# amidos2006/gym-pcgrl

Measured on AMD Instinct MI355X. Metric: env-steps/sec (whole node), binary-narrow 14x14 @ 65536 envs, higher is better.
Workload: dtype u8; 1 GPU; binary-narrow-v0 14x14, 65536 envs/GPU; envs_per_gpu=65536, width=14, height=14, max_changes=39, actions=uniform random, device-generated before the timed region, parallelism=env-axis shard x1, no collective on the step path

## Files before the change

gym_pcgrl_amd/_lib.py:

```python
import ctypes as C
import os
import subprocess

PKG = os.path.dirname(os.path.abspath(__file__))
ROOT = os.path.dirname(PKG)
CSRC = os.path.join(PKG, "csrc")
LIBDIR = os.path.join(PKG, "lib")
SO = os.path.join(LIBDIR, "libpcgrl_hip.so")
SOURCES = [os.path.join(CSRC, "pcgrl_abi.hip")]
HIPCC_FLAGS = ["--offload-arch=gfx950", "-O3", "-std=c++17", "-ffp-contract=off", "-fPIC", "-shared", "-mllvm", "-amdgpu-sched-strategy=max-ilp"]

PCGRL_OK, PCGRL_EINVAL, PCGRL_EHIP, PCGRL_ESTATE = 0, -1, -2, -3


class Config(C.Structure):
    _fields_ = [(n, C.c_int32) for n in (
        "prob", "rep", "num_envs", "width", "height", "prob_width", "prob_height", "max_changes", "max_iterations",
        "random_start", "random_tile", "warp", "random_probs", "auto_reset", "target_path",
        "max_enemies", "target_enemy_dist", "max_crates", "target_solution", "solver_power", "max_potions",
        "max_treasures", "max_diamonds", "min_spikes", "target_jumps", "min_empty", "min_enemies", "min_jumps")] + [
        ("target_col_enemies", C.c_double), ("tile_probs", C.c_double * 8), ("rewards", C.c_double * 12)]


class Layout(C.Structure):
    _fields_ = [(n, C.c_int32) for n in ("group", "mask_bytes", "nplanes", "nstats")] + [
        (n, C.c_size_t) for n in ("map", "old_map", "heatmap", "pos", "planes", "counters", "stats", "start_stats",
                                  "info", "reward", "done", "tile_p", "rng_rep", "rng_prob", "rng_cursor", "scratch")]


TUNING_FIELDS = ("no_fused", "fused_zelda", "step_epb", "no_inc", "inline_reset", "pair_min", "no_wide", "wide_waves", "wide_grid",
                 "wide_pairs", "wide_few", "sok_generic", "sok_hard_cap", "sok_spawn", "md_only_agent", "smb_lds_heap", "full_per_wave", "inc_per_wave", "wide_spin", "step_prio", "no_touch", "touch_tight", "step_pair", "async_split", "big_team", "obs_at_end", "touch_resume",
                 "changes_grid", "changes_chunk")


class Tuning(C.Structure):
    _fields_ = [(n, C.c_int32) for n in TUNING_FIELDS]


TUNING_OVERRIDES = {}


def make_tuning(overrides=None):
    t = Tuning(*([-1] * len(TUNING_FIELDS)))
    for k, v in list(TUNING_OVERRIDES.items()) + list((overrides or {}).items()):
        if k not in TUNING_FIELDS:
            raise KeyError("unknown tuning switch %r (known: %s)" % (k, ", ".join(TUNING_FIELDS)))
        setattr(t, k, int(v))
    return t


BUFFER_NAMES = ("map", "old_map", "heatmap", "pos", "planes", "counters", "stats", "start_stats", "info", "reward",
                "done", "tile_p", "rng_rep", "rng_prob", "rng_cursor", "scratch")


class Buffers(C.Structure):
    _fields_ = [(n, C.c_void_p) for n in BUFFER_NAMES]


ROW_FIELDS = ("actions_out", "reward", "done", "start_in", "start_out", "ep_return", "ep_length", "took", "fresh")


class Row(C.Structure):
    _fields_ = [(n, C.c_void_p) for n in ROW_FIELDS] + [("actions_i64", C.c_int32)]


class RenderDesc(C.Structure):
    _fields_ = [("indices", C.c_void_p), ("count", C.c_int32), ("tiles", C.c_void_p), ("tile_size", C.c_int32),
                ("border_x", C.c_int32), ("border_y", C.c_int32), ("border_tile", C.c_int32), ("cursor", C.c_int32),
                ("grid_rows", C.c_int32), ("grid_cols", C.c_int32), ("out", C.c_void_p)]


ABI_VERSION = 15
EXPORTS = ("pcgrl_abi_version", "pcgrl_error_string", "pcgrl_last_hip_error", "pcgrl_query_layout", "pcgrl_create",
           "pcgrl_destroy", "pcgrl_bind", "pcgrl_configure", "pcgrl_seed", "pcgrl_set_tile_probs", "pcgrl_reset",
           "pcgrl_step", "pcgrl_set_maps", "pcgrl_observe", "pcgrl_action_map", "pcgrl_status", "pcgrl_profile",
           "pcgrl_profile_read", "pcgrl_bind_episode_stats", "pcgrl_seed_words", "pcgrl_rollout", "pcgrl_bind_observation", "pcgrl_selftest_heap",
           "pcgrl_tuning_defaults", "pcgrl_set_tuning", "pcgrl_clear_status", "pcgrl_step_flat",
           "pcgrl_async_bytes", "pcgrl_bind_async", "pcgrl_step_async", "pcgrl_async_flush", "pcgrl_step_multi", "pcgrl_selftest_step_pool", "pcgrl_step_threads", "pcgrl_selftest_range_reward",
           "pcgrl_bind_row", "pcgrl_render", "pcgrl_get_stats_bytes", "pcgrl_get_stats", "pcgrl_get_reward",
           "pcgrl_get_solution_bytes", "pcgrl_get_solution", "pcgrl_get_playthrough_bytes", "pcgrl_get_playthrough",
           "pcgrl_get_smb_play_bytes", "pcgrl_get_smb_play", "pcgrl_get_paths_legs", "pcgrl_get_paths_bytes", "pcgrl_get_paths",
           "pcgrl_get_changes_bytes", "pcgrl_get_changes")
NPHASE = 6
PHASES = ("update", "stats", "reset_or_idle", "solver_or_reset", "reset2", "solver2")


def sources_newer_than_lib():
    if not os.path.exists(SO):
        return True
    t = os.path.getmtime(SO)
    deps = [os.path.join(CSRC, f) for f in os.listdir(CSRC)] + [os.path.join(ROOT, "include", "pcgrl_hip.h")]
    return any(os.path.getmtime(d) > t for d in deps)


def source_hash():
    import hashlib
    h = hashlib.sha256()
    files = sorted(os.path.join(CSRC, f) for f in os.listdir(CSRC)) + [os.path.join(ROOT, "include", "pcgrl_hip.h")]
    h.update(" ".join(HIPCC_FLAGS).encode() + b"\0")
    for f in files:
        h.update(os.path.basename(f).encode() + b"\0")
        with open(f, "rb") as fh:
            h.update(fh.read())
    return h.hexdigest()[:16]


NPARTS = 8


def build(force=False, verbose=False, jobs=None):
    if not force and not sources_newer_than_lib():
        return SO
    os.makedirs(LIBDIR, exist_ok=True)
    objdir = os.path.join(LIBDIR, "obj")
    os.makedirs(objdir, exist_ok=True)
    hipcc = os.environ.get("HIPCC", "hipcc")
    flags = [f for f in HIPCC_FLAGS if f != "-shared"]
    jobs = jobs or int(os.environ.get("PCGRL_BUILD_JOBS", "0")) or min(NPARTS, os.cpu_count() or 1)
    objs = [os.path.join(objdir, "part%d.o" % k) for k in range(NPARTS)]
    cmds = [[hipcc] + flags + ["-DPCGRL_PART=%d" % k, "-c", SOURCES[0], "-o", objs[k]] for k in range(NPARTS)]
    running, todo, failed = [], list(range(NPARTS)), []
    while todo or running:
        while todo and len(running) < jobs:
            k = todo.pop(0)
            if verbose:
                print(" ".join(cmds[k]), flush=True)
            running.append((k, subprocess.Popen(cmds[k])))
        k, p = running.pop(0)
        if p.wait() != 0:
            failed.append(k)
    if failed:
        raise subprocess.CalledProcessError(1, cmds[failed[0]])
    link = [hipcc, "--offload-arch=gfx950", "-shared", "-fPIC"] + objs + ["-o", SO]
    if verbose:
        print(" ".join(link), flush=True)
    subprocess.check_call(link)
    return SO


_lib = None


def load():
    global _lib, SO
    if _lib is not None:
        return _lib
    SO = os.environ.get("PCGRL_HIP_SO", SO)
    if not os.path.exists(SO):
        raise RuntimeError(
            "gym_pcgrl_amd: HIP library %s is missing. Build it with `python -c 'import __graft_entry__ as g; g.build()'` "
            "(hipcc --offload-arch=gfx950). There is no CPU fallback for the batched environment." % SO)
    import torch
    L = C.CDLL(SO)
    for name in EXPORTS:
        if not hasattr(L, name):
            raise RuntimeError("gym_pcgrl_amd: %s does not export %s (stale build?)" % (SO, name))
    L.pcgrl_abi_version.restype = C.c_int
    if L.pcgrl_abi_version() != ABI_VERSION:
        raise RuntimeError("gym_pcgrl_amd: %s has ABI version %d, this package needs %d (stale build?)" % (SO, L.pcgrl_abi_version(), ABI_VERSION))
    L.pcgrl_error_string.restype = C.c_char_p
    L.pcgrl_error_string.argtypes = [C.c_int]
    L.pcgrl_last_hip_error.restype = C.c_int
    L.pcgrl_query_layout.argtypes = [C.POINTER(Config), C.POINTER(Layout)]
    L.pcgrl_create.argtypes = [C.POINTER(Config), C.POINTER(C.c_void_p)]
    L.pcgrl_destroy.argtypes = [C.c_void_p]
    L.pcgrl_tuning_defaults.argtypes = [C.POINTER(Tuning)]
    L.pcgrl_tuning_defaults.restype = None
    L.pcgrl_set_tuning.argtypes = [C.c_void_p, C.POINTER(Tuning)]
    L.pcgrl_bind.argtypes = [C.c_void_p, C.POINTER(Buffers), C.c_void_p]
    L.pcgrl_configure.argtypes = [C.c_void_p, C.POINTER(Config)]
    L.pcgrl_seed.argtypes = [C.c_void_p, C.c_void_p, C.c_int32, C.c_int32, C.c_void_p]
    L.pcgrl_seed_words.argtypes = [C.c_void_p, C.c_void_p, C.c_int32, C.c_int32, C.c_void_p]
    L.pcgrl_set_tile_probs.argtypes = [C.c_void_p, C.c_void_p]
    L.pcgrl_reset.argtypes = [C.c_void_p, C.c_void_p]
    L.pcgrl_step.argtypes = [C.c_void_p, C.c_void_p, C.c_void_p]
    L.pcgrl_rollout.argtypes = [C.c_void_p, C.c_void_p, C.c_int32, C.c_void_p, C.c_void_p, C.c_void_p, C.c_void_p]
    L.pcgrl_set_maps.argtypes = [C.c_void_p, C.c_void_p, C.c_void_p]
    L.pcgrl_observe.argtypes = [C.c_void_p, C.c_void_p, C.c_int32, C.c_int32, C.c_int32, C.c_int32, C.c_int32, C.c_void_p]
    L.pcgrl_bind_observation.argtypes = [C.c_void_p, C.c_void_p, C.c_int32, C.c_int32, C.c_int32, C.c_int32, C.c_int32, C.c_int32]
    L.pcgrl_bind_row.argtypes = [C.c_void_p, C.POINTER(Row)]
    L.pcgrl_render.argtypes = [C.c_void_p, C.POINTER(RenderDesc), C.c_void_p]
    L.pcgrl_get_stats_bytes.argtypes = [C.POINTER(Config), C.c_int32]
    L.pcgrl_get_stats_bytes.restype = C.c_size_t
    L.pcgrl_get_stats.argtypes = [C.c_void_p, C.c_void_p, C.c_int32, C.c_void_p, C.c_void_p, C.c_size_t, C.c_void_p]
    L.pcgrl_get_reward.argtypes = [C.c_void_p, C.c_void_p, C.c_void_p, C.c_int32, C.c_void_p, C.c_void_p, C.c_void_p]
    moves_args = (C.c_void_p, C.c_void_p, C.c_int32, C.c_int32, C.c_void_p, C.c_void_p, C.c_void_p, C.c_void_p, C.c_void_p, C.c_size_t, C.c_void_p)
    for name in ("pcgrl_get_solution", "pcgrl_get_playthrough", "pcgrl_get_smb_play"):
        getattr(L, name + "_bytes").argtypes = [C.POINTER(Config), C.c_int32, C.c_int32]
        getattr(L, name + "_bytes").restype = C.c_size_t
        getattr(L, name).argtypes = list(moves_args)
    L.pcgrl_get_paths_legs.argtypes = [C.POINTER(Config)]
    L.pcgrl_get_paths_legs.restype = C.c_int32
    L.pcgrl_get_paths_bytes.argtypes = [C.POINTER(Config), C.c_int32, C.c_int32]
    L.pcgrl_get_paths_bytes.restype = C.c_size_t
    L.pcgrl_get_paths.argtypes = [C.c_void_p, C.c_void_p, C.c_int32, C.c_int32, C.c_void_p, C.c_void_p, C.c_void_p, C.c_void_p, C.c_size_t, C.c_void_p]
    L.pcgrl_get_changes_bytes.argtypes = [C.POINTER(Config), C.c_int32, C.c_int32]
    L.pcgrl_get_changes_bytes.restype = C.c_size_t
    L.pcgrl_get_changes.argtypes = [C.c_void_p, C.c_void_p, C.c_int32, C.c_void_p, C.c_int32, C.c_void_p, C.c_void_p, C.c_void_p, C.c_void_p, C.c_void_p,
                                    C.c_void_p, C.c_size_t, C.c_void_p]
    L.pcgrl_action_map.argtypes = [C.c_void_p, C.c_void_p, C.c_void_p, C.c_void_p]
    L.pcgrl_step_flat.argtypes = [C.c_void_p, C.c_void_p, C.c_void_p, C.c_void_p]
    L.pcgrl_selftest_heap.argtypes = [C.c_void_p, C.c_int32, C.c_void_p, C.c_void_p, C.c_void_p, C.c_void_p]
    L.pcgrl_selftest_step_pool.argtypes = [C.c_int32, C.c_int32, C.c_int32, C.c_void_p]
    L.pcgrl_selftest_range_reward.argtypes = [C.c_void_p, C.c_int32, C.c_void_p, C.c_void_p]
    L.pcgrl_step_threads.argtypes = [C.c_int32]
    L.pcgrl_step_threads.restype = C.c_int32
    L.pcgrl_status.argtypes = [C.c_void_p, C.c_void_p, C.POINTER(C.c_int32)]
    L.pcgrl_clear_status.argtypes = [C.c_void_p, C.c_void_p]
    L.pcgrl_profile.argtypes = [C.c_void_p, C.c_int]
    L.pcgrl_bind_episode_stats.argtypes = [C.c_void_p, C.c_void_p, C.c_void_p, C.c_void_p, C.c_void_p, C.c_void_p]
    L.pcgrl_profile_read.argtypes = [C.c_void_p, C.POINTER(C.c_double), C.POINTER(C.c_int32)]
    L.pcgrl_async_bytes.argtypes = [C.POINTER(Config), C.c_int32]
    L.pcgrl_async_bytes.restype = C.c_size_t
    L.pcgrl_bind_async.argtypes = [C.c_void_p, C.c_void_p, C.c_size_t, C.c_int32, C.c_void_p]
    L.pcgrl_step_async.argtypes = [C.c_void_p, C.c_void_p, C.c_int32, C.c_void_p]
    L.pcgrl_async_flush.argtypes = [C.c_void_p, C.c_void_p]
    L.pcgrl_step_multi.argtypes = [C.POINTER(C.c_void_p), C.POINTER(C.c_void_p), C.POINTER(C.c_void_p), C.c_int32]
    _lib = L
    return L


def check(rc, what):
    if rc != 0:
        L = load()
        msg = L.pcgrl_error_string(rc).decode()
        extra = " (hipError %d)" % L.pcgrl_last_hip_error() if rc == PCGRL_EHIP else ""
        raise RuntimeError("gym_pcgrl_amd: %s failed: %s%s" % (what, msg, extra))
```

gym_pcgrl_amd/csrc/kernels_stats.h:

```cpp
#pragma once
template <class MaskT>
__device__ __forceinline__ MaskT row_valid(int lane, int W, int H) {
    MaskT full = (W >= (int)(8 * sizeof(MaskT))) ? ~(MaskT)0 : (((MaskT)1 << W) - 1);
    return lane < H ? full : (MaskT)0;
}

template <int PROB = -1>
__device__ __forceinline__ bool finalize_item(const PcgrlParams& P, const DevBufs& B, int e, const int32_t* s,
                                              int mode, int parity, int shard, bool push_reset = true, int rst_list = WL_RST,
                                              const int2* pre = nullptr, const double* reward_pre = nullptr) {
    const int prob = PROB >= 0 ? PROB : P.prob;
    int32_t* st = B.stats + (size_t)e * 8;
    int32_t* start = B.start_stats + (size_t)e * 8;
    if (mode == MODE_STEP) {
        int32_t old[PCGRL_MAX_STATS], sv[PCGRL_MAX_STATS];
        for (int k = 0; k < 8; k++) { old[k] = st[k]; sv[k] = start[k]; }
        const int2 c = pre ? *pre : reinterpret_cast<const int2*>(B.counters)[e];
        const double r = reward_pre ? *reward_pre : compute_reward(P, s, old, prob);
        const bool d = episode_over(P, s, sv, prob) || c.y >= P.max_changes || c.x >= P.max_iterations;
        B.reward[e] = r;
        B.done[e] = d ? 1 : 0;
        episode_account(B, e, r, d);
        int32_t* inf = B.info + (size_t)e * 10;
#pragma unroll
        for (int k = 0; k < 8; k++) {
            st[k] = s[k];
            inf[k] = (prob == PCGRL_PROB_BINARY && k == 2) ? s[1] - sv[1] : ((prob == PCGRL_PROB_BINARY && k == 3) ? 0 : s[k]);
        }
        inf[8] = c.x; inf[9] = c.y;
        if (d && P.auto_reset && push_reset) wl_push(B, parity, rst_list, shard, e);
        return d && P.auto_reset;
    } else {
        for (int k = 0; k < 8; k++) st[k] = s[k];
        if (mode == MODE_START)
            for (int k = 0; k < 8; k++) start[k] = s[k];
    }
    return false;
}

template <int PROB, class G, class MaskT>
__device__ __forceinline__ bool compute_item_stats(G& g, const PcgrlParams& P, MaskT b0, MaskT b1, MaskT b2, MaskT valid, int32_t* s,
                                                   int32_t* status, MaskT& champ, bool tight = true) {
    champ = 0;
    if (PROB == PCGRL_PROB_BINARY) {
        int regions, path;
        if (G::kGroup == 16) {
            int ub2;
            regions_and_longest_path(g, (MaskT)(~b0 & valid), regions, path, champ, ub2, tight);
            s[3] = ub2 + 1;
        } else {
            regions_and_longest_path(g, (MaskT)(~b0 & valid), regions, path, champ);
        }
        s[0] = regions; s[1] = path; s[2] = g.any(champ) ? 1 : 0;
        return false;
    }
    if (PROB == PCGRL_PROB_ZELDA) { zelda_stats(g, P, b0, b1, b2, valid, s); return false; }
    if (PROB == PCGRL_PROB_MDUNGEON) return mdungeon_stats(g, P, b0, b1, b2, valid, s);
    if (PROB == PCGRL_PROB_DDAVE) {
        bool overflow = false;
        const bool ns = ddave_stats(g, P, b0, b1, b2, valid, s, &overflow);
        if (overflow && g.lane == 0) atomicOr(status, PCGRL_STATUS_TOO_MANY_CRATES);
        return ns;
    }
    if (PROB == PCGRL_PROB_SMB) return true;
    return sokoban_stats(g, P, b0, b1, b2, valid, s);
}
template <int PROB, class G, class MaskT>
__device__ __forceinline__ bool compute_item_stats(G& g, const PcgrlParams& P, MaskT b0, MaskT b1, MaskT b2, MaskT valid, int32_t* s, int32_t* status) {
    MaskT champ;
    return compute_item_stats<PROB>(g, P, b0, b1, b2, valid, s, status, champ);
}

template <int PROB = -1>
__device__ __forceinline__ bool finish_or_park(const PcgrlParams& P, const DevBufs& B, int e, const int32_t* s, bool need_solver,
                                               int mode, int parity, int shard, bool push_reset = true, int park_list = -1,
                                               const double* reward_pre = nullptr) {
    if (need_solver) {
        int32_t* park = (mode == MODE_STEP) ? B.info + (size_t)e * 10 : B.stats + (size_t)e * 8;
        for (int k = 0; k < 8; k++) park[k] = s[k];
        wl_push(B, parity, park_list >= 0 ? park_list : (mode == MODE_STEP ? WL_SOL : WL_SOL2), shard, e);
        return false;
    }
    return finalize_item<PROB>(P, B, e, s, mode, parity, shard, push_reset, WL_RST, nullptr, reward_pre);
}

template <int J>
__device__ __forceinline__ double dpp_down(double v) {
    const long long b = __double_as_longlong(v);
    const int lo = __builtin_amdgcn_update_dpp(0, (int)b, 0x100 + J, 0xF, 0xF, true), hi = __builtin_amdgcn_update_dpp(0, (int)(b >> 32), 0x100 + J, 0xF, 0xF, true);
    return __longlong_as_double(((long long)hi << 32) | (unsigned)lo);
}
__device__ __forceinline__ void zelda_reward_tab(const PcgrlParams& P, ZeldaRewardTab* T) {
    T->w[0] = P.rewards[0]; T->w[1] = P.rewards[1]; T->w[2] = P.rewards[2]; T->w[3] = P.rewards[4]; T->w[4] = P.rewards[3];
    T->w[5] = P.rewards[5]; T->w[6] = P.rewards[6]; T->w[7] = 0.0;
    T->lo[0] = 1; T->lo[1] = 1; T->lo[2] = 1; T->lo[3] = 2; T->lo[4] = 1; T->lo[5] = P.target_enemy_dist; T->lo[6] = PCGRL_IPOS; T->lo[7] = 0;
    T->hi[0] = 1; T->hi[1] = 1; T->hi[2] = 1; T->hi[3] = P.max_enemies; T->hi[4] = 1; T->hi[5] = PCGRL_IPOS; T->hi[6] = PCGRL_IPOS; T->hi[7] = 0;
}
__device__ __forceinline__ double zelda_reward_lanes(const ZeldaRewardTab* T, const int32_t* old, const int32_t* s, int k) {
    const int s0 = s[0], s1 = s[1], s2 = s[2], s3 = s[3], s4 = s[4], s5 = s[5], s6 = s[6];
    int n = s6;
    n = k == 5 ? s5 : n; n = k == 4 ? s4 : n; n = k == 3 ? s3 : n; n = k == 2 ? s2 : n; n = k == 1 ? s1 : n; n = k == 0 ? s0 : n;
    const int kk = k & 7;
    const int o = old[kk];
    const double t = k < 7 ? (double)range_reward_i(n, o, T->lo[kk], T->hi[kk]) * T->w[kk] : 0.0;
    double r = t;
    r = r + dpp_down<1>(t); r = r + dpp_down<2>(t); r = r + dpp_down<3>(t);
    r = r + dpp_down<4>(t); r = r + dpp_down<5>(t); r = r + dpp_down<6>(t);
    return r;
}

template <int PROB, int G, class MaskT, bool FUSED = false>
__device__ __forceinline__ void stats_wave_task(const PcgrlParams& P, const DevBufs& B, DevGroup<G, MaskT>& g, int lane64, int gw, bool lone,
                                                bool inc, bool pair, bool zinc, bool have, int raw, int shard, int mode, int parity,
                                                int inline_reset, int gen_map, uint32_t* mt, uint8_t* tiles, MaskT rowmask,
                                                StepLocal* SL = nullptr, bool step_obs = false) {
    constexpr bool kCanReset = PROB == PCGRL_PROB_BINARY || PROB == PCGRL_PROB_ZELDA;
    if (!kCanReset) inline_reset = 0;
    constexpr int GPW = 64 / G;
    constexpr bool kInc = PROB == PCGRL_PROB_BINARY;
    constexpr bool kZinc = PROB == PCGRL_PROB_ZELDA && G == 16 && sizeof(MaskT) == 4;
    constexpr int NPL = (PROB == PCGRL_PROB_BINARY) ? 1 : 3;
    MaskT* champ_base = reinterpret_cast<MaskT*>(B.champ);
    const bool tch = kInc && G == 16 && !inc && !lone && have && raw < 0;
    const bool packed = inc || (kZinc && zinc && !lone) || tch;
    const bool reset_only = have && !packed && (raw & WL_RESET_ONLY) != 0;
    const bool compute = have && !reset_only && !(lone && (gw & 1));
    const int e = packed ? wl_inc_env<G>(raw) : (raw & ~WL_RESET_ONLY);
    MaskT* planes_e = reinterpret_cast<MaskT*>(B.planes) + (size_t)e * NPL * G;
    MaskT b0 = 0, b1 = 0, b2 = 0;
    if (compute) {
        b0 = planes_e[g.lane * NPL];
        if (NPL > 1) { b1 = planes_e[g.lane * NPL + 1]; b2 = planes_e[g.lane * NPL + 2]; }
    }
    if (GPW >= 2 && lone && inline_reset) {
        const int role = gw & 1;
        int2 pre = make_int2(0, 0);
        if (g.lane == 0 && role == 0 && have) pre = reinterpret_cast<const int2*>(B.counters)[e];
        asm volatile("s_waitcnt vmcnt(0)" ::: "memory");
#pragma unroll
        for (int k = 0; k < GPW / 2; k++) {
            if (k > 0 && !pair) break;
            if (!__builtin_amdgcn_readlane((int)have, 2 * k * G)) continue;
            const int ek = __builtin_amdgcn_readlane(e, 2 * k * G);
            const int step_draws = (SL && P.rep == PCGRL_REP_NARROW && P.random_tile) ? 1 : 0;
            if (SL && lane64 == 0) SL->dirty[ek - SL->e0] = 1;
            ResetRows rr;
            wave_reset_env<PROB, !FUSED, FUSED>(P, B, ek, gen_map, mt, (uint8_t*)nullptr, lane64, step_draws, gw == 2 * k + 1 ? g.lane : -1, &rr);
            MaskT t0, t1, t2;
            reset_rows_to_planes<MaskT>(P, reinterpret_cast<MaskT*>(B.planes) + (size_t)ek * NPL * G, gw == 2 * k + 1 ? g.lane : -1, rr.m0, rr.m1, rr.m2, t0, t1, t2);
            if (gw == 2 * k + 1) { b0 = t0; b1 = t1; b2 = t2; }
            __builtin_amdgcn_wave_barrier();
        }
        TL(9);
        const bool act = have && (role == 1 || !reset_only);
        int32_t sl[PCGRL_MAX_STATS] = {0, 0, 0, 0, 0, 0, 0, 0};
        MaskT champ_l = 0;
        bool ns = false;
        if (act) ns = compute_item_stats<PROB>(g, P, b0, b1, b2, rowmask, sl, B.status, champ_l, (B.step_tight & 2) != 0);
        TL(10);
        constexpr bool kLaneReward = PROB == PCGRL_PROB_ZELDA && G == 16;
        double rpre = 0.0;
        if (kLaneReward && SL && role == 0 && act) rpre = zelda_reward_lanes(&SL->zr, B.stats + (size_t)e * 8, sl, g.lane);
        if (g.lane == 0 && role == 0 && act) finalize_item<PROB>(P, B, e, sl, MODE_STEP, parity, shard, false, WL_RST, &pre, (kLaneReward && SL) ? &rpre : nullptr);
        __builtin_amdgcn_wave_barrier();
        if (role == 1 && have) {
            if (kInc && champ_base) champ_base[(size_t)e * G + g.lane] = champ_l;
            if (g.lane == 0) finish_or_park<PROB>(P, B, e, sl, ns, MODE_START, parity, shard);
        }
        if (FUSED && step_obs) {
#pragma unroll
            for (int k = 0; k < GPW / 2; k++) {
                if (k > 0 && !pair) break;
                if (!__builtin_amdgcn_readlane((int)have, 2 * k * G)) continue;
                const ObsPlanes<MaskT, NPL> src = {reinterpret_cast<const MaskT*>(B.planes), G};
                obs_write_env_lean(src, obs_view_from_lds(&SL->obs_v), B.pos, __builtin_amdgcn_readlane(e, 2 * k * G), lane64);
            }
        }
        return;
    }
    int32_t s[PCGRL_MAX_STATS] = {0, 0, 0, 0, 0, 0, 0, 0};
    bool need_solver = false;
    MaskT champ = 0;
    if (kInc && inc) {
        if (compute) {
            const MaskT cbit = (g.lane == wl_inc_row<G>(raw)) ? (MaskT)1 << wl_inc_col<G>(raw) : (MaskT)0;
            const MaskT champ_old = champ_base[(size_t)e * G + g.lane];
            const int4 old = *reinterpret_cast<const int4*>(B.stats + (size_t)e * 8);
            int regions, path, ub2;
            binary_incremental(g, (MaskT)(~b0 & rowmask), cbit, wl_inc_code<G>(raw) != 0, old.x, old.y, champ_old, old.w - 1, regions, path, champ, ub2);
            s[0] = regions; s[1] = path; s[2] = 1; s[3] = ub2 + 1;
        }
    } else if (kZinc && packed) {
        if (compute) {
            const MaskT cbit = (g.lane == wl_inc_row<G>(raw)) ? (MaskT)1 << wl_inc_col<G>(raw) : (MaskT)0;
            zelda_stats(g, P, b0, b1, b2, rowmask, s, (int)wl_inc_code<G>(raw), cbit, B.stats[(size_t)e * 8 + 4]);
        }
    } else {
        bool full = compute;
        if (kInc && G == 16) {
            const bool t = compute && tch;
            TouchMemo<MaskT> memo = touch_memo_empty(g, b0);
            if (t) {
                const MaskT cbit = (g.lane == wl_inc_row<G>(raw)) ? (MaskT)1 << wl_inc_col<G>(raw) : (MaskT)0;
                const MaskT champ_old = champ_base[(size_t)e * G + g.lane];
                const int4 old = *reinterpret_cast<const int4*>(B.stats + (size_t)e * 8);
                int regions, path, ub2;
                if (binary_touch(g, (MaskT)(~b0 & rowmask), cbit, (wl_inc_code<G>(raw) & 1u) != 0, old.x, champ_old, old.w - 1, regions, path, champ, ub2, memo)) {
                    s[0] = regions; s[1] = path; s[2] = 1; s[3] = ub2 + 1;
                    full = false;
                }
            }
#ifdef PCGRL_TIMELINE
            {
                const uint64_t gu = __ballot(t && full && g.lane == 0), pl = __ballot(compute && !tch && g.lane == 0);
                TL(32 + __popcll(gu) + 8 * __popcll(pl));
            }
#endif
            constexpr bool kResume = FUSED && sizeof(MaskT) == 4;
            if (kResume && B.touch_resume) {
                if (full) {
                    int regions, path, ub2;
                    rlp_resume(g, (MaskT)(~b0 & rowmask), memo, regions, path, champ, ub2, (B.step_tight & 1) != 0);
                    s[0] = regions; s[1] = path; s[2] = g.any(champ) ? 1 : 0; s[3] = ub2 + 1;
                }
                full = false;
            }
        }
        if (full) need_solver = compute_item_stats<PROB>(g, P, b0, b1, b2, rowmask, s, B.status, champ, (B.step_tight & 1) != 0);
    }
    if (kInc && compute && champ_base) champ_base[(size_t)e * G + g.lane] = champ;
    TL(10);
    int want_reset = 0;
    constexpr bool kLaneReward = PROB == PCGRL_PROB_ZELDA && G == 16;
    double rpre = 0.0;
    const bool lane_reward = kLaneReward && SL != nullptr && mode == MODE_STEP;
    if (lane_reward && have && !reset_only) rpre = zelda_reward_lanes(&SL->zr, B.stats + (size_t)e * 8, s, g.lane);
    if (g.lane == 0 && have) {
        if (reset_only) want_reset = 1;
        else want_reset = finish_or_park<PROB>(P, B, e, s, need_solver, mode, parity, shard, !inline_reset, -1, lane_reward ? &rpre : nullptr) ? 1 : 0;
    }
    if (inline_reset) {
        const uint64_t want = __ballot(want_reset != 0);
        TL(11);
        if (want) {
            TL(12);
            if (SL) { while (__hip_atomic_load(&SL->refill_done[SL->par], __ATOMIC_ACQUIRE, __HIP_MEMORY_SCOPE_WORKGROUP) < SL->need) __builtin_amdgcn_s_sleep(2); }
            bool mine = false;
#pragma unroll
            for (int k = 0; k < GPW; k++) {
                if ((want >> (k * G)) & 1ull) {
                    const int ek = __builtin_amdgcn_readlane(e, k * G);
                    if (SL && lane64 == 0) { SL->dirty[ek - SL->e0] = 1; SL->late[ek - SL->e0] = 1; SL->n_late = 1; }
                    int pend = 0;
                    if (SL) {
                        if (lane64 == 0) {
                            pend = atomicExch(&SL->pend[ek - SL->e0], 0);
                            if (pend < 0) {
                                while (__hip_atomic_load(&SL->late_done[(ek - SL->e0) >> 6], __ATOMIC_ACQUIRE, __HIP_MEMORY_SCOPE_WORKGROUP) == 0) __builtin_amdgcn_s_sleep(2);
                                pend = 0;
                            }
                        }
                        pend = __builtin_amdgcn_readfirstlane(pend);
                    }
                    ResetRows rr;
                    wave_reset_env<PROB, !FUSED, FUSED>(P, B, ek, gen_map, mt, (uint8_t*)nullptr, lane64, 0, gw == k ? g.lane : -1, &rr, pend);
                    MaskT t0, t1, t2;
                    reset_rows_to_planes<MaskT>(P, reinterpret_cast<MaskT*>(B.planes) + (size_t)ek * NPL * G, gw == k ? g.lane : -1, rr.m0, rr.m1, rr.m2, t0, t1, t2);
                    if (gw == k) { b0 = t0; b1 = t1; b2 = t2; mine = true; }
                    __builtin_amdgcn_wave_barrier();
                }
            }
            if (mine) {
                int32_t st[PCGRL_MAX_STATS] = {0, 0, 0, 0, 0, 0, 0, 0};
                const bool ns = compute_item_stats<PROB>(g, P, b0, b1, b2, rowmask, st, B.status, champ, (B.step_tight & 2) != 0);
                if (kInc && champ_base) champ_base[(size_t)e * G + g.lane] = champ;
                if (g.lane == 0) finish_or_park<PROB>(P, B, e, st, ns, MODE_START, parity, shard);
            }
        }
    }
}

template <int PROB, int G, class MaskT>
__global__ __launch_bounds__(PCGRL_BLOCK) __attribute__((amdgpu_waves_per_eu(4, 8))) void k_stats(PcgrlParams P, DevBufs B, int list, int parity, int mode, int clear_parity,
                                                        int inline_reset, int gen_map, int lone0) {
    extern __shared__ __attribute__((aligned(16))) uint8_t smem[];
    __shared__ int s_pref[WL_NSHARD + 1], s_pref_inc[WL_NSHARD + 1], s_pref_rst[WL_NSHARD + 1];
    if (clear_parity >= 0 && blockIdx.x == 0) wl_clear(B, clear_parity);
    DevGroup<G, MaskT> g;
    constexpr int GPB = PCGRL_BLOCK / G, GPW = 64 / G;
    constexpr bool kInc = PROB == PCGRL_PROB_BINARY;
    constexpr bool kZinc = PROB == PCGRL_PROB_ZELDA && G == 16 && sizeof(MaskT) == 4;
    const bool zinc = kZinc && mode == MODE_STEP && B.zelda_inc;
    const bool with_inc = (kInc && mode == MODE_STEP && B.champ != nullptr) || zinc;
    int n_inc = 0, n_rst = 0;
    const int n_full = (with_inc || lone0 == 2 || list < 0) ? wl_load_prefix3(B, parity, list, with_inc ? WL_INC : -1, lone0 == 2 ? WL_RST : -1,
                                                                              s_pref, s_pref_inc, s_pref_rst, &n_inc, &n_rst)
                                                             : wl_load_prefix(B, parity, list, s_pref);
    const int n0 = lone0 == 1 ? s_pref[1] : (lone0 == 2 ? n_rst : 0);
    const int f0 = lone0 == 1 ? n0 : 0;
    const int w_full = (n_full - f0 + GPW - 1) / GPW;
    const bool pair = GPW >= 4 && n0 >= B.pair_min;
    const int w_lone = pair ? (n0 + 1) >> 1 : n0;
    const int w_total = w_lone + w_full + (n_inc + GPW - 1) / GPW;
    MaskT* champ_base = reinterpret_cast<MaskT*>(B.champ);
    const int lane64 = threadIdx.x & 63, wv = threadIdx.x >> 6, gw = lane64 / G;
    const int NPL = (PROB == PCGRL_PROB_BINARY) ? 1 : 3;
    const int W = P.width, H = P.height;
    uint32_t* mt = reinterpret_cast<uint32_t*>(smem + (size_t)wv * reset_stage_bytes(W * H));
    uint8_t* tiles = reinterpret_cast<uint8_t*>(mt + PCGRL_MT_N);
    const MaskT rowmask = row_valid<MaskT>(g.lane, W, H);
    for (int wid = blockIdx.x * (PCGRL_BLOCK / 64) + wv; wid < w_total; wid += gridDim.x * (PCGRL_BLOCK / 64)) {
        const bool lone = wid < w_lone;
        const bool inc = wid >= w_lone + w_full;
        const int item = lone ? (pair ? 2 * wid + (gw >> 1) : wid) : (inc ? (wid - w_lone - w_full) * GPW + gw : f0 + (wid - w_lone) * GPW + gw);
        const bool have = lone ? (item < n0 && (pair || gw < 2)) : item < (inc ? n_inc : n_full);
        const bool from_rst = lone && lone0 == 2;
        const int raw = !have ? 0 : (inc ? wl_get(B, WL_INC, s_pref_inc, item) : (from_rst ? wl_get(B, WL_RST, s_pref_rst, item) : wl_get(B, list, s_pref, item)));
        const int shard = (item >> 4) & (WL_NSHARD - 1);
        stats_wave_task<PROB, G, MaskT>(P, B, g, lane64, gw, lone, inc, pair, zinc, have, raw, shard, mode, parity, inline_reset, gen_map, mt, tiles, rowmask);
    }
}

template <class MaskT>
struct LdsShared {
    MaskT* rest; int* bestp; int lane;
    __device__ __forceinline__ MaskT load_rest() const { return *reinterpret_cast<volatile MaskT*>(rest + lane); }
    template <class G>
    __device__ __forceinline__ bool retire(G& g, MaskT comp) const {
        const MaskT fb = g.first_bit(comp);
        MaskT old = 0;
        if (fb) old = atomicAnd(rest + lane, ~fb);
        const bool won = __ballot((old & fb) != 0) != 0;
        if (comp) atomicAnd(rest + lane, ~comp);
        return won;
    }
    __device__ __forceinline__ int best() const { return *reinterpret_cast<volatile int*>(bestp); }
    __device__ __forceinline__ void raise(int v) const { if (lane == 0 && v > 0) atomicMax(bestp, v); }
};
template <class MaskT>
__device__ __forceinline__ void block_regions_and_path(DevGroup<64, MaskT>& g, MaskT pass, int tw, int ts, int lane, int H,
                                                       MaskT* s_rest, int* s_regions, int* s_best, int* s_owner, MaskT* champ_e) {
    const int bh = (H + ts - 1) / ts;
    const int row_lo = tw * bh, row_hi = (row_lo + bh < H) ? row_lo + bh : H;
    int tiny_regions, tiny_path;
    TL(20);
    const MaskT nontiny = rlp_prepare(g, pass, tiny_regions, tiny_path);
    TL(21);
    if (tw == 0) {
        s_rest[lane] = nontiny;
        if (lane == 0) { *s_regions = tiny_regions; *s_best = tiny_path; *s_owner = -1; }
    }
    __syncthreads();
    LdsShared<MaskT> sh = {s_rest, s_best, lane};
    int regions = 0, my_best = 0;
    MaskT my_champ = 0;
    MaskT rest = sh.load_rest();
    if (g.any(rest)) {
        const PcgFillCtx<DevGroup<64, MaskT>> ctx = pcg_fill_ctx(g, pass);
        do {
            rlp_process_seed(g, rlp_choose_seed(g, rest, row_lo, row_hi), ctx, sh, regions, my_best, my_champ);
            rest = sh.load_rest();
        } while (g.any(rest));
    }
    TL(22);
    if (lane == 0 && regions) atomicAdd(s_regions, regions);
    __syncthreads();
    TL(23);
    if (lane == 0 && my_best > tiny_path && my_best == *s_best) atomicCAS(s_owner, -1, tw);
    __syncthreads();
    if (champ_e) {
        const int owner = *s_owner;
        if (tw == (owner < 0 ? 0 : owner)) champ_e[lane] = owner < 0 ? (MaskT)0 : my_champ;
    }
}

template <class MaskT>
__device__ __forceinline__ void wave_incremental_item(const PcgrlParams& P, const DevBufs& B, DevGroup<64, MaskT>& g, int raw, int parity,
                                                      int inline_reset, int gen_map, uint32_t* mt, uint8_t* tiles, int lane, MaskT rowmask) {
    const int e = wl_inc_env<64>(raw);
    MaskT* planes_e = reinterpret_cast<MaskT*>(B.planes) + (size_t)e * 64;
    MaskT* champ_e = reinterpret_cast<MaskT*>(B.champ) + (size_t)e * 64;
    const MaskT b0 = planes_e[lane];
    const MaskT champ_old = champ_e[lane];
    const int2 old = *reinterpret_cast<const int2*>(B.stats + (size_t)e * 8);
    const MaskT cbit = (lane == wl_inc_row<64>(raw)) ? (MaskT)1 << wl_inc_col<64>(raw) : (MaskT)0;
    int regions, path;
    MaskT champ;
    binary_incremental(g, (MaskT)(~b0 & rowmask), cbit, wl_inc_code<64>(raw) != 0, old.x, old.y, champ_old, regions, path, champ);
    champ_e[lane] = champ;
    int want = 0;
    if (lane == 0) {
        int32_t s[PCGRL_MAX_STATS] = {regions, path, 1, 0, 0, 0, 0, 0};
        want = finalize_item<PCGRL_PROB_BINARY>(P, B, e, s, MODE_STEP, parity, e & (WL_NSHARD - 1), !inline_reset) ? 1 : 0;
    }
    want = __builtin_amdgcn_readfirstlane(want);
    if (inline_reset && want) {
        ResetRows rr;
        wave_reset_env<PCGRL_PROB_BINARY>(P, B, e, gen_map, mt, (uint8_t*)nullptr, lane, 0, lane, &rr);
        MaskT n0, n1, n2;
        reset_rows_to_planes<MaskT>(P, planes_e, lane, rr.m0, rr.m1, rr.m2, n0, n1, n2);
        int32_t st[PCGRL_MAX_STATS] = {0, 0, 0, 0, 0, 0, 0, 0};
        compute_item_stats<PCGRL_PROB_BINARY>(g, P, n0, n1, n2, rowmask, st, B.status, champ);
        champ_e[lane] = champ;
        if (lane == 0) finalize_item<PCGRL_PROB_BINARY>(P, B, e, st, MODE_START, parity, e & (WL_NSHARD - 1));
    }
}

#define WIDE_SPIN_LIMIT 400
__device__ __forceinline__ int wide_claim(int32_t* word, int epoch, int who) {
    int cur = __hip_atomic_load(word, __ATOMIC_RELAXED, __HIP_MEMORY_SCOPE_AGENT);
    for (;;) {
        if ((cur >> 1) == epoch) return 0;
        const int seen = atomicCAS(word, cur, (epoch << 1) | who);
        if (seen == cur) return 1;
        cur = seen;
    }
}

template <class MaskT, int NWAVES>
__global__ __launch_bounds__(NWAVES * 64) void k_stats_wide(PcgrlParams P, DevBufs B, int list, int parity, int mode, int clear_parity,
                                                             int inline_reset, int gen_map, int pair_few) {
    extern __shared__ __attribute__((aligned(16))) uint8_t smem[];
    __shared__ int s_pref[WL_NSHARD + 1], s_pref_rst[WL_NSHARD + 1], s_pref_inc[WL_NSHARD + 1];
    __shared__ MaskT s_rest[2][64];
    __shared__ int s_regions[2], s_best[2], s_owner[2], s_flag, s_flag2[2], s_cur, s_claim;
    __shared__ int2 s_pre;
    if (clear_parity >= 0 && blockIdx.x == 0) wl_clear(B, clear_parity);
    TL_INIT(); TL(1);
    WTL(0, wall_clock64());
    DevGroup<64, MaskT> g;
    const bool with_inc = mode == MODE_STEP && B.champ != nullptr;
    int n_rst = 0, n_inc = 0;
    const int n_chg = wl_load_prefix3(B, parity, list, with_inc ? WL_INC : -1, inline_reset ? WL_RST : -1, s_pref, s_pref_inc, s_pref_rst, &n_inc, &n_rst);
    const int n = n_rst + n_chg;
    const int lane = threadIdx.x & 63, wv = threadIdx.x >> 6;
    const int W = P.width, H = P.height;
    const int wave_lds = reset_stage_bytes(W * H);
    uint32_t* mt = reinterpret_cast<uint32_t*>(smem);
    uint8_t* tiles = reinterpret_cast<uint8_t*>(mt + PCGRL_MT_N);
    uint32_t* rst_raw = reinterpret_cast<uint32_t*>(smem + wave_lds);
    uint64_t* rst_bits = reinterpret_cast<uint64_t*>(smem + wave_lds + (size_t)8 * W * H);
    const MaskT rowmask = row_valid<MaskT>(lane, W, H);
    const int n_many = pair_few ? s_pref[WL_NSHARD / 2] : n_chg;
    const int n_items = 2 * n_rst + n_many + (n_chg - n_many + 1) / 2;
    const int epoch = B.wide_epoch;
    WTL(1, wall_clock64());
    WTL(5, (unsigned long long)n_items | ((unsigned long long)n_rst << 16) | ((unsigned long long)n_many << 32) | ((unsigned long long)n_inc << 48));
    for (int item = blockIdx.x; item < n_items; item += gridDim.x) {
        const bool lone = item < 2 * n_rst;
        const bool old_half = lone && (item & 1) == 0;
        WTL(2, (old_half ? 1 : (lone ? 2 : (item >= 2 * n_rst + n_many ? 4 : 3))) | (item << 8));
        if (item >= 2 * n_rst + n_many) {
            constexpr int TS = NWAVES / 2;
            const int team = wv / TS, tw = wv % TS;
            const int idx0 = n_many + 2 * (item - 2 * n_rst - n_many);
            const int e0 = wl_get(B, list, s_pref, idx0) & ~WL_RESET_ONLY;
            const int e1 = idx0 + 1 < n_chg ? (wl_get(B, list, s_pref, idx0 + 1) & ~WL_RESET_ONLY) : -1;
            const int et = team ? e1 : e0;
            const int shard = (item >> 4) & (WL_NSHARD - 1);
            MaskT pass = 0;
            if (et >= 0) pass = (MaskT)(~(reinterpret_cast<const MaskT*>(B.planes) + (size_t)et * 64)[lane] & rowmask);
            if (threadIdx.x < 2) s_flag2[threadIdx.x] = 0;
            block_regions_and_path(g, pass, tw, TS, lane, H, s_rest[team], &s_regions[team], &s_best[team], &s_owner[team],
                                   (et >= 0 && B.champ) ? reinterpret_cast<MaskT*>(B.champ) + (size_t)et * 64 : (MaskT*)nullptr);
            if (tw == 0 && lane == 0 && et >= 0) {
                int32_t s[PCGRL_MAX_STATS] = {s_regions[team], s_best[team], s_owner[team] >= 0 ? 1 : 0, 0, 0, 0, 0, 0};
                const bool want = finalize_item<PCGRL_PROB_BINARY>(P, B, et, s, mode, parity, shard, !inline_reset);
                s_flag2[team] = (want && inline_reset) ? 1 : 0;
            }
            __syncthreads();
            for (int t = 0; t < 2; t++) {
                if (!(inline_reset && s_flag2[t])) continue;
                const int er = t ? e1 : e0;
                MaskT* planes_r = reinterpret_cast<MaskT*>(B.planes) + (size_t)er * 64;
                const MaskT b0 = block_reset_env<PCGRL_PROB_BINARY, NWAVES * 64, MaskT>(P, B, er, gen_map, mt, tiles, rst_raw, rst_bits, &s_cur);
                if (wv == 0) planes_r[lane] = b0;
                block_regions_and_path(g, (MaskT)(~b0 & rowmask), wv, NWAVES, lane, H, s_rest[0], &s_regions[0], &s_best[0], &s_owner[0],
                                       B.champ ? reinterpret_cast<MaskT*>(B.champ) + (size_t)er * 64 : (MaskT*)nullptr);
                if (threadIdx.x == 0) {
                    int32_t s[PCGRL_MAX_STATS] = {s_regions[0], s_best[0], s_owner[0] >= 0 ? 1 : 0, 0, 0, 0, 0, 0};
                    finalize_item<PCGRL_PROB_BINARY>(P, B, er, s, MODE_START, parity, shard);
                }
                __syncthreads();
            }
            continue;
        }
        const int raw = lone ? wl_get(B, WL_RST, s_pref_rst, item >> 1) : wl_get(B, list, s_pref, item - 2 * n_rst);
        const bool reset_only = (raw & WL_RESET_ONLY) != 0;
        const int e = raw & ~WL_RESET_ONLY;
        const int shard = (item >> 4) & (WL_NSHARD - 1);
        MaskT* planes_e = reinterpret_cast<MaskT*>(B.planes) + (size_t)e * 64;
        MaskT* champ_e = B.champ ? reinterpret_cast<MaskT*>(B.champ) + (size_t)e * 64 : nullptr;
        int32_t* sync_e = B.wide_sync + (size_t)e * 4;
        if (old_half) {
            if (reset_only) continue;
            if (threadIdx.x == 0) s_claim = wide_claim(sync_e + 3, epoch, 0);
            __syncthreads();
            if (!s_claim) { __syncthreads(); continue; }
            const MaskT b_old = planes_e[lane];
            asm volatile("s_waitcnt vmcnt(0)" ::: "memory");
            __syncthreads();
            if (threadIdx.x == 0) __hip_atomic_store(sync_e + 0, epoch, __ATOMIC_RELEASE, __HIP_MEMORY_SCOPE_AGENT);
            block_regions_and_path(g, (MaskT)(~b_old & rowmask), wv, NWAVES, lane, H, s_rest[0], &s_regions[0], &s_best[0], &s_owner[0], (MaskT*)nullptr);
            if (threadIdx.x == 0) {
                sync_e[2] = s_regions[0] | (s_best[0] << 16);
                __hip_atomic_store(sync_e + 1, epoch, __ATOMIC_RELEASE, __HIP_MEMORY_SCOPE_AGENT);
            }
            __syncthreads();
            continue;
        }
        if (lone) {
            __builtin_amdgcn_s_setprio(1);
            if (threadIdx.x == 0) s_pre = reinterpret_cast<const int2*>(B.counters)[e];
            asm volatile("s_waitcnt vmcnt(0)" ::: "memory");
            __syncthreads();
            TL(24);
            const MaskT n0 = block_reset_env<PCGRL_PROB_BINARY, NWAVES * 64, MaskT>(P, B, e, gen_map, mt, tiles, rst_raw, rst_bits, &s_cur);
            int own_old = 0;
            if (!reset_only) {
                if (threadIdx.x == 0) {
                    int spins = 0, mine = 0;
                    while (__hip_atomic_load(sync_e + 0, __ATOMIC_ACQUIRE, __HIP_MEMORY_SCOPE_AGENT) != epoch) {
                        __builtin_amdgcn_s_sleep(4);
                        if (++spins == B.wide_spin && wide_claim(sync_e + 3, epoch, 1)) { mine = 1; break; }
                    }
                    s_claim = mine;
                }
                __syncthreads();
                own_old = s_claim;
                if (own_old) {
                    const MaskT b_old = planes_e[lane];
                    asm volatile("s_waitcnt vmcnt(0)" ::: "memory");
                    block_regions_and_path(g, (MaskT)(~b_old & rowmask), wv, NWAVES, lane, H, s_rest[1], &s_regions[1], &s_best[1], &s_owner[1], (MaskT*)nullptr);
                }
                __syncthreads();
            }
            if (wv == 0) planes_e[lane] = n0;
            TL(26);
            block_regions_and_path(g, (MaskT)(~n0 & rowmask), wv, NWAVES, lane, H, s_rest[0], &s_regions[0], &s_best[0], &s_owner[0], champ_e);
            if (threadIdx.x == 0) {
                if (!reset_only) {
                    int32_t s[PCGRL_MAX_STATS] = {s_regions[1], s_best[1], 0, 0, 0, 0, 0, 0};
// ... 52 lines not shown
```

gym_pcgrl_amd/csrc/kernels_step.h:

```cpp
#pragma once

struct StepLds { int planes, champ, stats, start, cnt, cur, fifo, tag, pos, act, flat, in_total, info, rew, done, total; };
__host__ __device__ constexpr StepLds step_lds_layout(int plane_row_bytes, int champ_row_bytes, bool fifo, int action_width, int epb) {
    StepLds L = {};
    int o = 0;
    L.planes = o; o += epb * plane_row_bytes;
    L.champ = o; o += epb * champ_row_bytes;
    L.stats = o; o += epb * 32;
    L.start = o; o += epb * 32;
    L.cnt = o; o += epb * 8;
    L.cur = o; o += epb * 8;
    L.fifo = o; o += fifo ? epb * PCGRL_FIFO_N * 4 : 0;
    L.tag = o; o += fifo ? epb * 4 : 0;
    L.pos = o; o += epb * 2;
    L.act = o; o += epb * 4 * action_width;
    L.flat = o; o += action_width == 3 ? epb * 4 : 0;
    L.in_total = o;
    L.info = o; o += epb * 40;
    L.rew = o; o += epb * 8;
    L.done = o; o += epb;
    L.total = (o + 15) & ~15;
    return L;
}

template <int TPB>
__device__ __forceinline__ void blk_copy(uint8_t* dst, const uint8_t* src, int bytes) {
    const int nv = bytes >> 4;
    for (int i = threadIdx.x; i < nv; i += TPB) reinterpret_cast<uint4*>(dst)[i] = reinterpret_cast<const uint4*>(src)[i];
    for (int i = (nv << 4) + threadIdx.x; i < bytes; i += TPB) dst[i] = src[i];
}
template <int TPB>
__device__ __forceinline__ void blk_copy_rows(uint8_t* dst, const uint8_t* src, int rows, int row, const uint8_t* flag) {
    const int per = row >> 4;
    for (int i = threadIdx.x; i < rows * per; i += TPB)
        if (flag[i / per]) reinterpret_cast<uint4*>(dst)[i] = reinterpret_cast<const uint4*>(src)[i];
}

template <int TPB, int C, int SLOT0, int NV>
__device__ __forceinline__ void seg_load_c(uint4& rc, const void* g, bool on, int tid) {
    if (C * TPB + TPB - 1 < SLOT0 || C * TPB >= SLOT0 + NV) return;
    const int slot = C * TPB + tid;
    if (on && slot >= SLOT0 && slot < SLOT0 + NV) rc = reinterpret_cast<const uint4*>(g)[slot - SLOT0];
}
#define PCGRL_SEG_LOAD(SLOT0, NV, G, ON) do { const void* g_ = (G); const bool on_ = (ON); \
    seg_load_c<TPB, 0, SLOT0, NV>(r0, g_, on_, tid0); seg_load_c<TPB, 1, SLOT0, NV>(r1, g_, on_, tid0); seg_load_c<TPB, 2, SLOT0, NV>(r2, g_, on_, tid0); \
    seg_load_c<TPB, 3, SLOT0, NV>(r3, g_, on_, tid0); seg_load_c<TPB, 4, SLOT0, NV>(r4, g_, on_, tid0); seg_load_c<TPB, 5, SLOT0, NV>(r5, g_, on_, tid0); \
    seg_load_c<TPB, 6, SLOT0, NV>(r6, g_, on_, tid0); seg_load_c<TPB, 7, SLOT0, NV>(r7, g_, on_, tid0); seg_load_c<TPB, 8, SLOT0, NV>(r8, g_, on_, tid0); } while (0)
template <int TPB, int C, int TOTAL>
__device__ __forceinline__ void seg_store_c(uint8_t* smem, const uint4& rc, int tid) {
    if (C * TPB >= TOTAL) return;
    const int slot = C * TPB + tid;
    if (slot < TOTAL) reinterpret_cast<uint4*>(smem)[slot] = rc;
}

__device__ __forceinline__ void fifo_refill(const DevBufs& B, int e, int k, int cur0) {
    uint32_t* ring = B.rng_rep + (size_t)e * PCGRL_MT_N;
    uint32_t* fl = B.fifo + (size_t)e * PCGRL_FIFO_N;
    const int base = mt_wrap(cur0 + PCGRL_FIFO_N), basem = mt_wrap(base + PCGRL_MT_M);
    uint32_t a[PCGRL_FIFO_N + 1], m[PCGRL_FIFO_N];
#pragma unroll
    for (int i = 0; i <= PCGRL_FIFO_N; i++) a[i] = (i <= k) ? ring[mt_wrap(base + i)] : 0u;
#pragma unroll
    for (int i = 0; i < PCGRL_FIFO_N; i++) m[i] = (i < k) ? ring[mt_wrap(basem + i)] : 0u;
#pragma unroll
    for (int i = 0; i < PCGRL_FIFO_N; i++) if (i < k) ring[mt_wrap(cur0 + i)] = fl[i];
#pragma unroll
    for (int j = 0; j < PCGRL_FIFO_N; j++) if (j + k < PCGRL_FIFO_N) fl[j] = fl[j + k];
#pragma unroll
    for (int i = 0; i < PCGRL_FIFO_N; i++) if (i < k) fl[PCGRL_FIFO_N - k + i] = mt_twist(a[i], a[i + 1], m[i]);
    B.fifo_tag[e] = mt_wrap(cur0 + k);
}

__device__ __forceinline__ void step_set_prio(int p) {
    if (p == 0) __builtin_amdgcn_s_setprio(0);
    else if (p == 1) __builtin_amdgcn_s_setprio(1);
    else if (p == 2) __builtin_amdgcn_s_setprio(2);
    else __builtin_amdgcn_s_setprio(3);
}

template <int PROB, int REP, class MaskT, bool MULTI, int EPB, bool OBS = false, bool ROW = false>
__global__ __launch_bounds__(EPB * 4) __attribute__((amdgpu_waves_per_eu(4, 8))) void k_step(PcgrlParams P, DevBufs Bg, const int32_t* __restrict__ actions, int parity, int gen_map,
                                                                                                     int steps, size_t action_stride, double* reward_out, uint8_t* done_out, int32_t* info_out) {
    extern __shared__ __attribute__((aligned(16))) uint8_t smem[];
    constexpr int TPB = EPB * 4, NUPD = EPB / 64;
    __shared__ int s_items[3][EPB];
    __shared__ int s_n[2][4];
    __shared__ StepLocal s_loc;
    __shared__ int s_obs_ticket;
    static_assert(!(OBS && MULTI), "the tape form writes its images at the end");
    static_assert(!(ROW && MULTI), "the tape form has its own outputs (pcgrl_rollout ignores the row binding)");
    constexpr int G = 16, GPW = 4;
    constexpr int NPL = (PROB == PCGRL_PROB_BINARY) ? 1 : 3;
    constexpr int kPlaneRow = G * NPL * (int)sizeof(MaskT);
    const int W = P.width, H = P.height;
    TL_INIT(); TL(1);
    const int e0 = blockIdx.x * EPB;
    const int ne = (P.num_envs - e0) < EPB ? (P.num_envs - e0) : EPB;
    const bool has_champ = PROB == PCGRL_PROB_BINARY && Bg.champ != nullptr;
    const bool has_fifo = REP == PCGRL_REP_NARROW && Bg.fifo != nullptr;
    constexpr int kChampRow = PROB == PCGRL_PROB_BINARY ? G * (int)sizeof(MaskT) : 0;
    constexpr int AW = REP == PCGRL_REP_WIDE ? 3 : 1;
    constexpr StepLds L = step_lds_layout(kPlaneRow, kChampRow, REP == PCGRL_REP_NARROW, AW, EPB);
    const int champ_row = kChampRow;
    DevBufs B = Bg;
    const size_t cells_ = (size_t)W * H;
    B.map = Bg.map + (size_t)e0 * cells_;
    B.old_map = Bg.old_map + (size_t)e0 * cells_;
    B.heat = Bg.heat + (size_t)e0 * cells_;
    B.tile_p = Bg.tile_p + (size_t)e0 * 2;
    B.rng_rep = Bg.rng_rep + (size_t)e0 * PCGRL_MT_N;
    if (Bg.rng_prob) B.rng_prob = Bg.rng_prob + (size_t)e0 * PCGRL_MT_N;
    if (Bg.ep_return) { B.ep_return = Bg.ep_return + e0; B.ep_length = Bg.ep_length + e0; B.last_return = Bg.last_return + e0; B.last_length = Bg.last_length + e0; }
    B.planes = smem + L.planes;
    if (has_champ) B.champ = smem + L.champ;
    B.stats = reinterpret_cast<int32_t*>(smem + L.stats);
    B.start_stats = reinterpret_cast<int32_t*>(smem + L.start);
    B.info = reinterpret_cast<int32_t*>(smem + L.info);
    B.reward = reinterpret_cast<double*>(smem + L.rew);
    B.counters = reinterpret_cast<int32_t*>(smem + L.cnt);
    B.rng_cur = reinterpret_cast<int32_t*>(smem + L.cur);
    if (has_fifo) {
        B.fifo = reinterpret_cast<uint32_t*>(smem + L.fifo);
        B.fifo_tag = reinterpret_cast<int32_t*>(smem + L.tag);
    } else {
        B.fifo = nullptr; B.fifo_tag = nullptr;
    }
    B.pos = smem + L.pos;
    B.done = smem + L.done;
    const int32_t* act_lds = reinterpret_cast<const int32_t*>(smem + L.act);
    const uint8_t* g_planes = reinterpret_cast<const uint8_t*>(Bg.planes) + (size_t)e0 * kPlaneRow;
    const uint8_t* g_champ = has_champ ? reinterpret_cast<const uint8_t*>(Bg.champ) + (size_t)e0 * champ_row : nullptr;
    const bool row_fl = ROW && AW == 3 && Bg.flat;
    const int row_per = row_fl ? 1 : AW;
    const size_t row_a0 = (size_t)e0 * row_per + threadIdx.x;
    const bool row_have = ROW && (int)threadIdx.x < ne * row_per;
    int64_t row_act = 0;
    static_assert(AW <= 4, "one action value per thread");
    if (row_have) {
        const int32_t* src = row_fl ? Bg.flat : actions;
        row_act = Bg.act_i64 ? reinterpret_cast<const int64_t*>(src)[row_a0] : (int64_t)src[row_a0];
    }
    if (ne == EPB) {
        static_assert(L.in_total / 16 <= 9 * TPB, "nine 16-byte slots per thread");
        uint4 r0 = {}, r1 = {}, r2 = {}, r3 = {}, r4 = {}, r5 = {}, r6 = {}, r7 = {}, r8 = {};
        const int tid0 = (int)threadIdx.x;
        PCGRL_SEG_LOAD(L.planes / 16, EPB * kPlaneRow / 16, g_planes, true);
        if (kChampRow) PCGRL_SEG_LOAD(L.champ / 16, (kChampRow ? EPB * kChampRow / 16 : 1), g_champ, has_champ);
        PCGRL_SEG_LOAD(L.stats / 16, EPB * 2, Bg.stats + (size_t)e0 * 8, true);
        PCGRL_SEG_LOAD(L.start / 16, EPB * 2, Bg.start_stats + (size_t)e0 * 8, true);
        PCGRL_SEG_LOAD(L.cnt / 16, EPB / 2, Bg.counters + (size_t)e0 * 2, true);
        PCGRL_SEG_LOAD(L.cur / 16, EPB / 2, Bg.rng_cur + (size_t)e0 * 2, true);
        if (REP == PCGRL_REP_NARROW) {
            PCGRL_SEG_LOAD(L.fifo / 16, EPB * PCGRL_FIFO_N * 4 / 16, has_fifo ? Bg.fifo + (size_t)e0 * PCGRL_FIFO_N : nullptr, has_fifo);
            PCGRL_SEG_LOAD(L.tag / 16, EPB / 4, has_fifo ? Bg.fifo_tag + e0 : nullptr, has_fifo);
        }
        PCGRL_SEG_LOAD(L.pos / 16, EPB / 8, Bg.pos + (size_t)e0 * 2, true);
        if (!ROW) PCGRL_SEG_LOAD(L.act / 16, EPB / 4 * AW, actions + (size_t)e0 * AW, !(AW == 3 && Bg.flat));
        if (!ROW && AW == 3) PCGRL_SEG_LOAD(L.flat / 16, (AW == 3 ? EPB / 4 : 1), Bg.flat ? Bg.flat + e0 : nullptr, Bg.flat != nullptr);
        asm volatile("" ::: "memory");
        static_assert(L.act % 16 == 0, "the prefetch ends on a slot boundary in front of the actions");
        constexpr int TOT = (ROW ? L.act : L.in_total) / 16;
        seg_store_c<TPB, 0, TOT>(smem, r0, tid0); seg_store_c<TPB, 1, TOT>(smem, r1, tid0); seg_store_c<TPB, 2, TOT>(smem, r2, tid0);
        seg_store_c<TPB, 3, TOT>(smem, r3, tid0); seg_store_c<TPB, 4, TOT>(smem, r4, tid0); seg_store_c<TPB, 5, TOT>(smem, r5, tid0);
        seg_store_c<TPB, 6, TOT>(smem, r6, tid0); seg_store_c<TPB, 7, TOT>(smem, r7, tid0); seg_store_c<TPB, 8, TOT>(smem, r8, tid0);
    } else {
        blk_copy<TPB>(smem + L.planes, g_planes, ne * kPlaneRow);
        if (has_champ) blk_copy<TPB>(smem + L.champ, g_champ, ne * champ_row);
        blk_copy<TPB>(smem + L.stats, reinterpret_cast<const uint8_t*>(Bg.stats + (size_t)e0 * 8), ne * 32);
        blk_copy<TPB>(smem + L.start, reinterpret_cast<const uint8_t*>(Bg.start_stats + (size_t)e0 * 8), ne * 32);
        blk_copy<TPB>(smem + L.cnt, reinterpret_cast<const uint8_t*>(Bg.counters + (size_t)e0 * 2), ne * 8);
        blk_copy<TPB>(smem + L.cur, reinterpret_cast<const uint8_t*>(Bg.rng_cur + (size_t)e0 * 2), ne * 8);
        blk_copy<TPB>(smem + L.pos, Bg.pos + (size_t)e0 * 2, ne * 2);
        if (has_fifo) {
            blk_copy<TPB>(smem + L.fifo, reinterpret_cast<const uint8_t*>(Bg.fifo + (size_t)e0 * PCGRL_FIFO_N), ne * PCGRL_FIFO_N * 4);
            blk_copy<TPB>(smem + L.tag, reinterpret_cast<const uint8_t*>(Bg.fifo_tag + e0), ne * 4);
        }
        if (ROW) {}
        else if (AW == 3 && Bg.flat) blk_copy<TPB>(smem + L.flat, reinterpret_cast<const uint8_t*>(Bg.flat + e0), ne * 4);
        else blk_copy<TPB>(smem + L.act, reinterpret_cast<const uint8_t*>(actions + (size_t)e0 * AW), ne * 4 * AW);
    }
    if (row_have) {
        reinterpret_cast<int32_t*>(smem + (row_fl ? L.flat : L.act))[threadIdx.x] = (int32_t)row_act;
        if (Bg.row.actions_out) Bg.row.actions_out[row_a0] = row_act;
    }
    if (threadIdx.x < EPB) { s_loc.dirty[threadIdx.x] = 0; if (OBS) { s_loc.obs_skip[threadIdx.x] = 0; s_loc.late[threadIdx.x] = 0; } }
    if (threadIdx.x < 8) s_n[threadIdx.x >> 2][threadIdx.x & 3] = 0;
    if (threadIdx.x == 0) { s_loc.e0 = 0; s_loc.need = NUPD; s_loc.refill_done[0] = 0; s_loc.refill_done[1] = 0; s_loc.n_late = 0; s_obs_ticket = 0; }
    constexpr int OBS_PER_TASK = 8;
    const bool obs_delta = OBS && REP == PCGRL_REP_WIDE && NPL == 3 && Bg.obs.delta;
    const int n_obs = (OBS && !obs_delta) ? (ne + OBS_PER_TASK - 1) / OBS_PER_TASK : 0;
    const ObsPlanes<MaskT, NPL> obs_src = {reinterpret_cast<const MaskT*>(smem + L.planes), G};
    if (OBS && threadIdx.x == 0) s_loc.obs_v = obs_view(P, Bg.obs, e0);
    if (PROB == PCGRL_PROB_ZELDA && threadIdx.x == 64) zelda_reward_tab(P, &s_loc.zr);
    uint8_t* reset_scratch = smem + L.total;
#pragma clang loop unroll(disable)
  for (int t = 0; t < (MULTI ? steps : 1); t++) {
    int tid = (int)threadIdx.x;
    if (MULTI) asm volatile("" : "+v"(tid));
    const int lane64 = tid & 63, wv = tid >> 6, gw = lane64 / G;
    const int sp = t & 1;
    DevGroup<G, MaskT> g(lane64);
    if (MULTI && t > 0) {
        const int32_t* row = actions + (size_t)t * action_stride + (size_t)e0 * AW;
        for (int i = tid; i < ne * AW; i += TPB) reinterpret_cast<int32_t*>(smem + L.act)[i] = row[i];
    }
    __syncthreads();
    TL(17);
    const int prio = B.step_prio, prio_nfull = (prio >> 8) & 15;
    int prio_now = 0;
    if (wv < NUPD) {
        if ((prio >> 6) & 3) { prio_now = (prio >> 6) & 3; step_set_prio(prio_now); }
        const int e = wv * 64 + lane64;
        UpdateOut u = {};
        UpdateMid mid = {};
        if (REP == PCGRL_REP_WIDE && !MULTI && Bg.flat && e < ne) {
            const int dim = P.ntiles, total = W * H * dim;
            int a = reinterpret_cast<const int32_t*>(smem + L.flat)[e];
            if (a < 0 || a >= total) atomicOr(B.status, PCGRL_STATUS_BAD_ACTION);
            a = a < 0 ? 0 : (a >= total ? total - 1 : a);
            int32_t* t3 = reinterpret_cast<int32_t*>(smem + L.act) + 3 * e;
            const int q = a / dim;
            t3[0] = q % W; t3[1] = q / W; t3[2] = a - q * dim;
        }
        if (e < ne) u = update_env<REP, MaskT, true, true, true>(P, B, act_lds, e, &mid);
        TL(2);
        const bool first = u.rst || u.sure_done;
        const bool packed_full = PROB == PCGRL_PROB_ZELDA && B.zelda_inc;
        int dest = -1, v = e;
        if (first) { dest = 0; v = u.rst ? (e | WL_RESET_ONLY) : e; }
        else if (u.chg) { dest = u.cheap ? 2 : 1; v = (u.cheap || packed_full) ? u.inc_item : ((u.touch && B.step_touch) ? (u.inc_item | (int)0x80000000) : e); }
        if (u.chg) s_loc.dirty[e] = 1;
        if (OBS && first && e < EPB) s_loc.obs_skip[e] = 1;
        const uint64_t m0 = __ballot(dest == 0), m1 = __ballot(dest == 1), m2 = __ballot(dest == 2);
        const uint64_t below = (1ull << lane64) - 1ull;
        int b0 = 0, b1 = 0, b2 = 0;
        if (lane64 == 0) {
            b0 = m0 ? atomicAdd(&s_n[sp][0], __popcll(m0)) : 0;
            b1 = m1 ? atomicAdd(&s_n[sp][1], __popcll(m1)) : 0;
            b2 = m2 ? atomicAdd(&s_n[sp][2], __popcll(m2)) : 0;
            if (wv == 0) { s_n[sp ^ 1][0] = 0; s_n[sp ^ 1][1] = 0; s_n[sp ^ 1][2] = 0; s_n[sp ^ 1][3] = 0; s_loc.refill_done[sp ^ 1] = 0; s_loc.par = sp; }
        }
        b0 = __builtin_amdgcn_readfirstlane(b0); b1 = __builtin_amdgcn_readfirstlane(b1); b2 = __builtin_amdgcn_readfirstlane(b2);
        if (dest == 0) s_items[0][b0 + __popcll(m0 & below)] = v;
        if (dest == 2) s_items[2][b2 + __popcll(m2 & below)] = v;
        {
            const int lvl = (u.bucket >> 3) & 7;
            int pos1 = 0;
#pragma unroll
            for (int b = 0; b < 8; b++) {
                const uint64_t mb = __ballot(dest == 1 && lvl == b);
                pos1 += b > lvl ? __popcll(mb) : (b == lvl ? __popcll(mb & below) : 0);
            }
            if (dest == 1) s_items[1][b1 + pos1] = v;
        }
        asm volatile("s_waitcnt lgkmcnt(0)" ::: "memory");
        __builtin_amdgcn_s_barrier();
        int k_used = 0, cur0 = 0;
        if (lane64 == 0) s_loc.late_done[wv] = 0;
        if (e < ne && !first) update_env_cursor<REP, MaskT>(P, B, e, mid, k_used, cur0);
        if (OBS && REP == PCGRL_REP_WIDE && NPL == 3 && obs_delta && e < ne && !first && u.chg) obs_write_delta_piece(obs_src, obs_view_from_lds(&s_loc.obs_v), e, act_lds[3 * e], act_lds[3 * e + 1]);
        if (e < EPB) s_loc.pend[e] = (has_fifo && e < ne && !first) ? k_used : 0;
        asm volatile("s_waitcnt vmcnt(0) lgkmcnt(0)" ::: "memory");
        if (lane64 == 0) __hip_atomic_fetch_add(&s_loc.refill_done[sp], 1, __ATOMIC_RELEASE, __HIP_MEMORY_SCOPE_WORKGROUP);
    }
    int n0 = 0, n1 = 0, n2 = 0, w_full = 0, w_total = 0, w_lone = 0;
    bool stats_left = true, obs_left = OBS;
    bool pair = false;
    const int fpw = B.step_fpw, ipw = B.step_ipw;
    const int tiles_bytes = (W * H + 15) & ~15;
    uint32_t* mt = reinterpret_cast<uint32_t*>(reset_scratch + (size_t)wv * (PCGRL_MT_N * 4 + tiles_bytes));
    uint8_t* tiles = reinterpret_cast<uint8_t*>(mt + PCGRL_MT_N);
    const MaskT rowmask = row_valid<MaskT>(g.lane, W, H);
    const bool zinc = PROB == PCGRL_PROB_ZELDA && sizeof(MaskT) == 4 && B.zelda_inc;
    for (bool first_round = true;; first_round = false) {
        if (first_round) {
            if (wv >= NUPD) {
                asm volatile("s_waitcnt lgkmcnt(0)" ::: "memory");
                __builtin_amdgcn_s_barrier();
                asm volatile("" ::: "memory");
            }
            TL(3);
            n0 = s_n[sp][0]; n1 = s_n[sp][1]; n2 = s_n[sp][2];
            w_full = (n1 + fpw - 1) / fpw;
            pair = PROB == PCGRL_PROB_ZELDA && B.step_pair > 0 && n0 >= B.step_pair;
            w_lone = pair ? (n0 + 1) >> 1 : n0;
            w_total = w_lone + w_full + (n2 + ipw - 1) / ipw;
        }
        if (OBS && !first_round && obs_left) {
            int oid = 0;
            if (lane64 == 0) oid = atomicAdd(&s_obs_ticket, 1);
            oid = __builtin_amdgcn_readfirstlane(oid);
            if (oid >= n_obs) obs_left = false;
            else {
                if (prio_now) { prio_now = 0; step_set_prio(0); }
                while (__hip_atomic_load(&s_loc.refill_done[sp], __ATOMIC_ACQUIRE, __HIP_MEMORY_SCOPE_WORKGROUP) < NUPD) __builtin_amdgcn_s_sleep(2);
                const int o0 = oid * OBS_PER_TASK;
                const ObsView V = obs_view_from_lds(&s_loc.obs_v);
#pragma clang loop unroll(disable)
                for (int j = 0; j < OBS_PER_TASK; j++) {
                    const int eo = o0 + j;
                    if (eo < ne && !s_loc.obs_skip[eo]) obs_write_env_lean(obs_src, V, smem + L.pos, eo, lane64);
                }
            }
        }
        if (!stats_left) { if (!OBS || !obs_left) break; continue; }
        int wid = 0;
        if (lane64 == 0) wid = atomicAdd(&s_n[sp][3], 1);
        wid = __builtin_amdgcn_readfirstlane(wid);
        TL(18);
        if (wid >= w_total) { stats_left = false; if (!OBS || !obs_left) break; continue; }
        const bool lone = wid < w_lone, inc = wid >= w_lone + w_full;
        const int item = lone ? (pair ? 2 * wid + (gw >> 1) : wid) : (inc ? (wid - w_lone - w_full) * ipw + gw : (wid - w_lone) * fpw + gw);
        const bool have = lone ? (item < n0 && (pair || gw < 2)) : (gw < (inc ? ipw : fpw) && item < (inc ? n2 : n1));
        const int raw = have ? s_items[lone ? 0 : (inc ? 2 : 1)][item] : 0;
        TL(lone ? 4 : (inc ? 6 : 5));
        if (prio) {
            const int want = lone ? (prio & 3) : (inc ? ((prio >> 4) & 3) : ((prio_nfull == 0 || wid - w_lone < prio_nfull) ? ((prio >> 2) & 3) : 0));
            if (want != prio_now) { prio_now = want; step_set_prio(want); }
        }
        stats_wave_task<PROB, G, MaskT, true>(P, B, g, lane64, gw, lone, inc, PROB == PCGRL_PROB_ZELDA && pair, zinc, have, raw, lane64, MODE_STEP, parity, 1, gen_map, mt, tiles, rowmask, &s_loc, OBS);
        TL(7);
    }
    if (prio_now) { prio_now = 0; step_set_prio(0); }
    if (has_fifo && wv < NUPD) {
        const int e = wv * 64 + lane64;
        int k = 0;
        if (e < ne) k = atomicExch(&s_loc.pend[e], -1);
        if (k > 0) {
            int c0 = B.rng_cur[2 * e] - k;
            c0 = c0 < 0 ? c0 + PCGRL_MT_N : c0;
            fifo_refill(B, e, k, c0);
        }
        asm volatile("s_waitcnt vmcnt(0) lgkmcnt(0)" ::: "memory");
        if (lane64 == 0) __hip_atomic_store(&s_loc.late_done[wv], 1, __ATOMIC_RELEASE, __HIP_MEMORY_SCOPE_WORKGROUP);
    }
    TL(8);
    if (MULTI && (reward_out || done_out || info_out)) {
        __syncthreads();
        const size_t row = (size_t)t * P.num_envs + e0;
        if (reward_out && tid < ne) reward_out[row + tid] = reinterpret_cast<const double*>(smem + L.rew)[tid];
        if (done_out && tid >= TPB / 2 && tid - TPB / 2 < ne) done_out[row + tid - TPB / 2] = smem[L.done + tid - TPB / 2];
        if (info_out) for (int i = tid; i < ne * 10; i += TPB) info_out[row * 10 + i] = reinterpret_cast<const int32_t*>(smem + L.info)[i];
    }
  }
    __syncthreads();
    blk_copy<TPB>(reinterpret_cast<uint8_t*>(Bg.stats + (size_t)e0 * 8), smem + L.stats, ne * 32);
    blk_copy<TPB>(reinterpret_cast<uint8_t*>(Bg.info + (size_t)e0 * 10), smem + L.info, ne * 40);
    blk_copy<TPB>(reinterpret_cast<uint8_t*>(Bg.reward + e0), smem + L.rew, ne * 8);
    blk_copy<TPB>(reinterpret_cast<uint8_t*>(Bg.counters + (size_t)e0 * 2), smem + L.cnt, ne * 8);
    blk_copy<TPB>(reinterpret_cast<uint8_t*>(Bg.rng_cur + (size_t)e0 * 2), smem + L.cur, ne * 8);
    blk_copy<TPB>(Bg.pos + (size_t)e0 * 2, smem + L.pos, ne * 2);
    blk_copy<TPB>(Bg.done + e0, smem + L.done, ne);
    if (has_fifo) {
        blk_copy<TPB>(reinterpret_cast<uint8_t*>(Bg.fifo + (size_t)e0 * PCGRL_FIFO_N), smem + L.fifo, ne * PCGRL_FIFO_N * 4);
        blk_copy<TPB>(reinterpret_cast<uint8_t*>(Bg.fifo_tag + e0), smem + L.tag, ne * 4);
    }
    blk_copy_rows<TPB>(reinterpret_cast<uint8_t*>(Bg.planes) + (size_t)e0 * kPlaneRow, smem + L.planes, ne, kPlaneRow, s_loc.dirty);
    if (has_champ) blk_copy_rows<TPB>(reinterpret_cast<uint8_t*>(Bg.champ) + (size_t)e0 * champ_row, smem + L.champ, ne, champ_row, s_loc.dirty);
    blk_copy_rows<TPB>(reinterpret_cast<uint8_t*>(Bg.start_stats + (size_t)e0 * 8), smem + L.start, ne, 32, s_loc.dirty);
    if (ROW) {
        const RowBind& R = Bg.row;
        const int q = (int)threadIdx.x / EPB, i = (int)threadIdx.x % EPB;
        if (i < ne) {
            const uint8_t d = smem[L.done + i] ? 1 : 0;
            if (q == 0) { if (R.reward) R.reward[e0 + i] = reinterpret_cast<const double*>(smem + L.rew)[i]; }
            else if (q == 1) {
                if (R.done) R.done[e0 + i] = d;
                if (R.start_out) R.start_out[e0 + i] = d;
                if (R.took) R.took[e0 + i] = 1;
                if (R.fresh) R.fresh[e0 + i] = 1;
            }
            else if (q == 2) { if (R.ep_return) R.ep_return[e0 + i] = d ? Bg.last_return[e0 + i] : __longlong_as_double(0x7FF8000000000000ll); }
            else if (R.ep_length) R.ep_length[e0 + i] = d ? Bg.last_length[e0 + i] : 0;
        }
    }
    if (!OBS && Bg.obs.out && Bg.obs.fused) {
        const ObsPlanes<MaskT, NPL> src = {reinterpret_cast<const MaskT*>(smem + L.planes), G};
        obs_write_block_lean(src, obs_view(P, Bg.obs, e0), smem + L.pos, ne, REP == PCGRL_REP_WIDE && !MULTI && Bg.obs.delta, act_lds, s_loc.dirty,
                             smem + L.done, (int)threadIdx.x, TPB);
    }
    if (OBS && s_loc.n_late) {
        asm volatile("s_waitcnt vmcnt(0)" ::: "memory");
        __syncthreads();
        const ObsView V = obs_view_from_lds(&s_loc.obs_v);
        for (int eo = __builtin_amdgcn_readfirstlane((int)threadIdx.x >> 6); eo < ne; eo += TPB >> 6)
            if (s_loc.late[eo]) obs_write_env_lean(obs_src, V, smem + L.pos, eo, (int)threadIdx.x & 63);
    }
}
```

gym_pcgrl_amd/csrc/kernels_update.h:

```cpp
#pragma once
#define PCGRL_SPEC_DRAWS 6
struct UpdateOut {
    bool chg;
    bool rst;
    bool cheap;
    bool touch;
    bool sure_done;
    int bucket;
    int inc_item;
    int k, cur0;
};
struct UpdateMid { int x, y, hx, hy, cur; bool chg, dead; };
template <int REP, class MaskT, bool FIFO = false, bool SPLIT = false, bool AR_ONLY = false>
__device__ __forceinline__ UpdateOut update_env(const PcgrlParams& P, const DevBufs& B, const int32_t* __restrict__ actions, int e, UpdateMid* mid = nullptr, const int ash = 0) {
    bool chg = false, rst = false, cheap = false, sure_done = false, touch_item = false;
    int bucket = 0, inc_item = 0, k_used = 0, cur0 = 0;
    uint32_t fw[PCGRL_FIFO_N];
#pragma unroll
    for (int i = 0; i < PCGRL_FIFO_N; i++) fw[i] = 0;
    {
        const int W = P.width, H = P.height, G = P.group, NPL = P.nplanes;
        const int2 c = reinterpret_cast<const int2*>(B.counters)[e];
        int a0_ = 0, a1_ = 0, a2_ = 0;
        if (REP == PCGRL_REP_WIDE) { a0_ = actions[(size_t)(3 * e + 0) << ash]; a1_ = actions[(size_t)(3 * e + 1) << ash]; a2_ = actions[(size_t)(3 * e + 2) << ash]; }
        else a0_ = actions[(size_t)e << ash];
        uchar2 p0 = make_uchar2(0, 0);
        if (REP != PCGRL_REP_WIDE) p0 = reinterpret_cast<const uchar2*>(B.pos)[e];
        const bool draws = REP == PCGRL_REP_NARROW && P.random_tile;
        int cur = 0;
        if (draws) cur = B.rng_cur[2 * e];
        const int4* sp = reinterpret_cast<const int4*>(B.stats + (size_t)e * 8);
        const int4* tp = reinterpret_cast<const int4*>(B.start_stats + (size_t)e * 8);
        const int4 s0 = sp[0], s1 = sp[1], t0 = tp[0], t1 = tp[1];

        bucket = difficulty_bucket(P, s0, s1, B.wide_few);
        const int iter = c.x + 1;
        int changes = c.y;
        int x = p0.x, y = p0.y;
        int tile = -1, wx = 0, wy = 0, hx = 0, hy = 0;
        bool bad = false;
        if (REP == PCGRL_REP_NARROW) {
            const int a = clampi(a0_, 0, P.ntiles);
            bad = a != a0_;
            if (a > 0) tile = a - 1;
            wx = x; wy = y;
        } else if (REP == PCGRL_REP_WIDE) {
            wx = clampi(a0_, 0, W - 1);
            wy = clampi(a1_, 0, H - 1);
            tile = clampi(a2_, 0, P.ntiles - 1);
            bad = wx != a0_ || wy != a1_ || tile != a2_;
            hx = wx; hy = wy;
        } else {
            const int a = clampi(a0_, 0, P.ntiles + 3);
            bad = a != a0_;
            if (a < 4) {
                const int dx = (a == 0) ? -1 : (a == 1 ? 1 : 0), dy = (a == 2) ? -1 : (a == 3 ? 1 : 0);
                x += dx;
                if (x < 0) x = P.warp ? x + W : 0;
                if (x >= W) x = P.warp ? x - W : W - 1;
                y += dy;
                if (y < 0) y = P.warp ? y + H : 0;
                if (y >= H) y = P.warp ? y - H : H - 1;
            } else {
                tile = a - 4;
            }
            wx = x; wy = y; hx = x; hy = y;
        }
        uint8_t* cell = B.map + ((size_t)e * H + wy) * W + wx;
        MaskT* pl = reinterpret_cast<MaskT*>(B.planes) + ((size_t)e * G + wy) * NPL;
        const bool writes = tile >= 0;
        const bool inc_on = P.prob == PCGRL_PROB_BINARY && B.champ != nullptr;
        MaskT ch0 = 0, chu = 0, chd = 0;
        bool big_touch = false;
        if (inc_on && writes && P.big) {
            const int KW = (W + 63) >> 6;
            const uint64_t* ch = reinterpret_cast<const uint64_t*>(B.champ) + (size_t)e * H * KW;
            const int xs[5] = {wx, wx - 1, wx + 1, wx, wx}, ys[5] = {wy, wy, wy, wy - 1, wy + 1};
#pragma unroll
            for (int q = 0; q < 5; q++) {
                const int xx = xs[q], yy = ys[q];
                if (xx >= 0 && xx < W && yy >= 0 && yy < H) big_touch = big_touch || ((ch[yy * KW + (xx >> 6)] >> (xx & 63)) & 1ull) != 0ull;
            }
        } else if (inc_on && writes) {
            const MaskT* ch = reinterpret_cast<const MaskT*>(B.champ) + (size_t)e * G;
            ch0 = ch[wy];
            chu = ch[wy > 0 ? wy - 1 : wy];
            chd = ch[wy < G - 1 ? wy + 1 : wy];
        }
        MaskT m0 = 0, m1 = 0, m2 = 0;
        int old_byte = 0;
        if (writes) {
            if (NPL == 0) old_byte = (int)*cell;
            else {
                m0 = pl[0];
                if (NPL > 1) { m1 = pl[1]; m2 = pl[2]; }
            }
        }
        const int old = NPL == 0 ? old_byte : ((int)((m0 >> wx) & 1) | ((NPL > 1) ? (int)(((m1 >> wx) & 1) << 1) | (int)(((m2 >> wx) & 1) << 2) : 0));
        uint32_t* ring = B.rng_rep + (size_t)e * PCGRL_MT_N;
        uint32_t xa[PCGRL_SPEC_DRAWS + 1], xb[PCGRL_SPEC_DRAWS];
        cur0 = cur;
        if (draws && FIFO && !SPLIT) {
            const int tag = B.fifo_tag[e];
            const uint4* fp = reinterpret_cast<const uint4*>(B.fifo + (size_t)e * PCGRL_FIFO_N);
            const uint4 fa = fp[0], fb = fp[1];
            fw[0] = fa.x; fw[1] = fa.y; fw[2] = fa.z; fw[3] = fa.w; fw[4] = fb.x; fw[5] = fb.y; fw[6] = fb.z; fw[7] = fb.w;
            if (tag != cur) {
#pragma unroll
                for (int i = 0; i < PCGRL_FIFO_N; i++) {
                    fw[i] = mt_twist(ring[mt_wrap(cur + i)], ring[mt_wrap(cur + i + 1)], ring[mt_wrap(mt_wrap(cur + PCGRL_MT_M) + i)]);
                    B.fifo[(size_t)e * PCGRL_FIFO_N + i] = fw[i];
                }
            }
        }
        if (draws && !FIFO) {
#pragma unroll
            for (int i = 0; i <= PCGRL_SPEC_DRAWS; i++) xa[i] = ring[mt_wrap(cur + i)];
#pragma unroll
            for (int i = 0; i < PCGRL_SPEC_DRAWS; i++) xb[i] = ring[mt_wrap(mt_wrap(cur + PCGRL_MT_M) + i)];
        }
        if (tile >= 0 && old != tile) {
            chg = true;
            if (inc_on && s0.z != 0 && P.big) {
                cheap = !big_touch;
                inc_item = wl_incbig_pack(e, wx, wy, tile == 0);
            } else if (inc_on && s0.z != 0) {
                const MaskT bit = (MaskT)1 << wx;
                const MaskT touch = ((ch0 | chu | chd) & bit) | (ch0 & ((bit << 1) | (bit >> 1)));
                cheap = touch == 0;
                touch_item = touch != 0 && s0.w != 0;
                inc_item = wl_inc_pack(G, e, wy, wx, tile == 0 ? 1u : 0u);
            }
            if (P.prob == PCGRL_PROB_SMB && B.champ != nullptr) {
                const bool so = (0x5Au >> old) & 1u, sn = (0x5Au >> tile) & 1u;
                const uint32_t seen = reinterpret_cast<const uint32_t*>(B.champ)[(size_t)e * W + wx];
                cheap = (so == sn || ((seen >> wy) & 1u) == 0u) && B.sok_cnt[e] != SMB_REPLAY;
                inc_item = e | SMB_KEEP_PLAY;
            }
            if (B.zelda_inc) {
                const bool po = old != 1 && old != 4, pn = tile != 1 && tile != 4;
                inc_item = wl_inc_pack(16, e, wy, wx, po == pn ? 0u : (pn ? 1u : 2u));
                cheap = po == pn;
            }
            const bool dead_writes = FIFO && P.auto_reset && B.inline_reset && (c.y + 1 >= P.max_changes || iter >= P.max_iterations);
            if (!dead_writes) *cell = (uint8_t)tile;
            const MaskT bit = (MaskT)1 << wx;
            if (NPL > 0) pl[0] = (tile & 1) ? (m0 | bit) : (m0 & ~bit);
            if (NPL > 1) {
                pl[1] = (tile & 2) ? (m1 | bit) : (m1 & ~bit);
                pl[2] = (tile & 4) ? (m2 | bit) : (m2 & ~bit);
            }
        }
        if (REP == PCGRL_REP_NARROW && !SPLIT) {
            if (draws && FIFO) {
                const uint32_t rx = (uint32_t)(W - 1), ry = (uint32_t)(H - 1);
                uint32_t mx = rx, my = ry;
                mx |= mx >> 1; mx |= mx >> 2; mx |= mx >> 4; mx |= mx >> 8; mx |= mx >> 16;
                my |= my >> 1; my |= my >> 2; my |= my >> 4; my |= my >> 8; my |= my >> 16;
                int stage = 0, used = 0;
                if (rx == 0) { x = 0; stage = 1; }
                if (stage == 1 && ry == 0) { y = 0; stage = 2; }
#pragma unroll
                for (int i = 0; i < PCGRL_FIFO_N; i++) {
                    if (stage < 2) {
                        used = i + 1;
                        const uint32_t v = mt_temper(fw[i]);
                        if (stage == 0) {
                            if ((v & mx) <= rx) { x = (int)(v & mx); stage = 1; if (ry == 0) { y = 0; stage = 2; } }
                        } else {
                            if ((v & my) <= ry) { y = (int)(v & my); stage = 2; }
                        }
                    }
                }
                if (stage < 2) {
#pragma unroll
                    for (int i = 0; i < PCGRL_FIFO_N; i++) ring[mt_wrap(cur + i)] = fw[i];
                    cur = mt_wrap(cur + PCGRL_FIFO_N);
                    if (stage == 0) { x = mt_randint(ring, cur, W); y = mt_randint(ring, cur, H); }
                    else y = mt_randint(ring, cur, H);
                    B.fifo_tag[e] = -1;
                    asm volatile("s_waitcnt vmcnt(0)" ::: "memory");
                    __threadfence_block();
                    cur0 = cur;
                } else {
                    cur = mt_wrap(cur + used);
                    k_used = used;
                }
                B.rng_cur[2 * e] = cur;
            } else if (draws) {
                if (B.fifo_tag) B.fifo_tag[e] = -1;
                const uint32_t rx = (uint32_t)(W - 1), ry = (uint32_t)(H - 1);
                uint32_t mx = rx, my = ry;
                mx |= mx >> 1; mx |= mx >> 2; mx |= mx >> 4; mx |= mx >> 8; mx |= mx >> 16;
                my |= my >> 1; my |= my >> 2; my |= my >> 4; my |= my >> 8; my |= my >> 16;
                int stage = 0, used = 0;
                if (rx == 0) { x = 0; stage = 1; }
                if (stage == 1 && ry == 0) { y = 0; stage = 2; }
#pragma unroll
                for (int i = 0; i < PCGRL_SPEC_DRAWS; i++) {
                    if (stage < 2) {
                        const uint32_t yv = mt_twist(xa[i], xa[i + 1], xb[i]);
                        ring[mt_wrap(cur + i)] = yv;
                        used = i + 1;
                        const uint32_t v = mt_temper(yv);
                        if (stage == 0) {
                            if ((v & mx) <= rx) { x = (int)(v & mx); stage = 1; if (ry == 0) { y = 0; stage = 2; } }
                        } else {
                            if ((v & my) <= ry) { y = (int)(v & my); stage = 2; }
                        }
                    }
                }
                cur = mt_wrap(cur + used);
                if (stage < 2) {
                    if (stage == 0) { x = mt_randint(ring, cur, W); y = mt_randint(ring, cur, H); }
                    else y = mt_randint(ring, cur, H);
                }
                B.rng_cur[2 * e] = cur;
            } else {
                x += 1;
                if (x >= W) { x = 0; y += 1; if (y >= H) y = 0; }
            }
            hx = x; hy = y;
        }
        bool dead_heat = false;
        if (chg) {
            changes += 1;
            const bool dead_writes = FIFO && P.auto_reset && B.inline_reset && (changes >= P.max_changes || iter >= P.max_iterations);
            dead_heat = dead_writes;
            if (!dead_writes && !(SPLIT && REP == PCGRL_REP_NARROW)) heat_increment<AR_ONLY>(B, ((size_t)e * H + hy) * W + hx);
        }
        reinterpret_cast<int2*>(B.counters)[e] = make_int2(iter, changes);
        if (bad) atomicOr(B.status, PCGRL_STATUS_BAD_ACTION);
        if (REP != PCGRL_REP_WIDE && !(SPLIT && REP == PCGRL_REP_NARROW)) reinterpret_cast<uchar2*>(B.pos)[e] = make_uchar2((unsigned char)x, (unsigned char)y);
        if (SPLIT && mid) { mid->x = x; mid->y = y; mid->hx = hx; mid->hy = hy; mid->cur = cur; mid->chg = chg; mid->dead = dead_heat; }
        sure_done = chg && P.auto_reset && B.inline_reset && (changes >= P.max_changes || iter >= P.max_iterations);
        if (sure_done) { cheap = false; touch_item = false; }
        if (!chg) {
            int32_t s[PCGRL_MAX_STATS], st[PCGRL_MAX_STATS];
            s[0] = s0.x; s[1] = s0.y; s[2] = s0.z; s[3] = s0.w; s[4] = s1.x; s[5] = s1.y; s[6] = s1.z; s[7] = s1.w;
            st[0] = t0.x; st[1] = t0.y; st[2] = t0.z; st[3] = t0.w; st[4] = t1.x; st[5] = t1.y; st[6] = t1.z; st[7] = t1.w;
            const bool d = episode_over(P, s, st) || changes >= P.max_changes || iter >= P.max_iterations;
            B.reward[e] = 0.0;
            B.done[e] = d ? 1 : 0;
            episode_account(B, e, 0.0, d);
            int32_t* inf = B.info + (size_t)e * 10;
            inf[0] = s0.x; inf[1] = s0.y; inf[2] = s0.z; inf[3] = s0.w;
            inf[4] = s1.x; inf[5] = s1.y; inf[6] = s1.z; inf[7] = s1.w;
            if (P.prob == PCGRL_PROB_BINARY) { inf[2] = s0.y - t0.y; inf[3] = 0; }
            inf[8] = iter; inf[9] = changes;
            rst = d && P.auto_reset;
        }
    }
    UpdateOut o;
    o.chg = chg; o.rst = rst; o.cheap = cheap; o.touch = touch_item; o.sure_done = sure_done; o.bucket = bucket; o.inc_item = inc_item;
    o.k = k_used; o.cur0 = cur0;
    return o;
}

template <int REP, class MaskT>
__device__ __forceinline__ void update_env_cursor(const PcgrlParams& P, const DevBufs& B, int e, const UpdateMid& mid, int& k_used, int& cur0) {
    const int W = P.width, H = P.height;
    int x = mid.x, y = mid.y, cur = mid.cur;
    k_used = 0; cur0 = cur;
    if (REP != PCGRL_REP_NARROW) return;
    if (P.random_tile) {
        uint32_t* ring = B.rng_rep + (size_t)e * PCGRL_MT_N;
        uint32_t fw[PCGRL_FIFO_N];
        const int tag = B.fifo_tag[e];
        const uint4* fp = reinterpret_cast<const uint4*>(B.fifo + (size_t)e * PCGRL_FIFO_N);
        const uint4 fa = fp[0], fb = fp[1];
        fw[0] = fa.x; fw[1] = fa.y; fw[2] = fa.z; fw[3] = fa.w; fw[4] = fb.x; fw[5] = fb.y; fw[6] = fb.z; fw[7] = fb.w;
        if (tag != cur) {
#pragma unroll
            for (int i = 0; i < PCGRL_FIFO_N; i++) {
                fw[i] = mt_twist(ring[mt_wrap(cur + i)], ring[mt_wrap(cur + i + 1)], ring[mt_wrap(mt_wrap(cur + PCGRL_MT_M) + i)]);
                B.fifo[(size_t)e * PCGRL_FIFO_N + i] = fw[i];
            }
        }
        const uint32_t rx = (uint32_t)(W - 1), ry = (uint32_t)(H - 1);
        uint32_t mx = rx, my = ry;
        mx |= mx >> 1; mx |= mx >> 2; mx |= mx >> 4; mx |= mx >> 8; mx |= mx >> 16;
        my |= my >> 1; my |= my >> 2; my |= my >> 4; my |= my >> 8; my |= my >> 16;
        int stage = 0, used = 0;
        if (rx == 0) { x = 0; stage = 1; }
        if (stage == 1 && ry == 0) { y = 0; stage = 2; }
#pragma unroll
        for (int i = 0; i < PCGRL_FIFO_N; i++) {
            if (stage < 2) {
                used = i + 1;
                const uint32_t v = mt_temper(fw[i]);
                if (stage == 0) {
                    if ((v & mx) <= rx) { x = (int)(v & mx); stage = 1; if (ry == 0) { y = 0; stage = 2; } }
                } else {
                    if ((v & my) <= ry) { y = (int)(v & my); stage = 2; }
                }
            }
        }
        if (stage < 2) {
#pragma unroll
            for (int i = 0; i < PCGRL_FIFO_N; i++) ring[mt_wrap(cur + i)] = fw[i];
            cur = mt_wrap(cur + PCGRL_FIFO_N);
            if (stage == 0) { x = mt_randint(ring, cur, W); y = mt_randint(ring, cur, H); }
            else y = mt_randint(ring, cur, H);
            B.fifo_tag[e] = -1;
            asm volatile("s_waitcnt vmcnt(0)" ::: "memory");
            __threadfence_block();
            cur0 = cur;
        } else {
            cur = mt_wrap(cur + used);
            k_used = used;
        }
        B.rng_cur[2 * e] = cur;
    } else {
        x += 1;
        if (x >= W) { x = 0; y += 1; if (y >= H) y = 0; }
    }
    if (mid.chg && !mid.dead) heat_increment<true>(B, ((size_t)e * H + y) * W + x);
    reinterpret_cast<uchar2*>(B.pos)[e] = make_uchar2((unsigned char)x, (unsigned char)y);
}

template <int REP, class MaskT>
__global__ __launch_bounds__(PCGRL_BLOCK) void k_update(PcgrlParams P, DevBufs B, const int32_t* __restrict__ actions, int parity) {
    __shared__ int s_cnt[3][4];
    __shared__ int s_base[3];
    __shared__ int s_hist[WL_NSHARD + 1], s_gbase[WL_NSHARD + 1];
    const int e = blockIdx.x * PCGRL_BLOCK + threadIdx.x;
    UpdateOut u = {};
    bool live = e < P.num_envs;
    if (B.pending) {
        const int pv = live ? (int)B.pending[e] : 1;
        live = pv == 0;
        const int cnt = __popcll(__ballot(live));
        if ((threadIdx.x & 63) == 0 && cnt) atomicAdd(B.async_stats + 8 + 8 * (blockIdx.x & 15), (unsigned long long)cnt);
        if (pv == 2) { u.rst = true; B.pending[e] = 0; }
        if (B.row.took && e < P.num_envs) B.row.took[e] = live ? 1 : 0;
        async_list_runnable(B, e);
    }
    if (live) u = update_env<REP, MaskT>(P, B, actions, e, nullptr, B.act_i64);
    const bool chg = u.chg, rst = u.rst, cheap = u.cheap, sure_done = u.sure_done;
    int bucket = u.bucket;
    const int inc_item = u.inc_item;
    const bool inl = rst && B.inline_reset;
    const int val = inl ? (e | WL_RESET_ONLY) : e;
    if (P.prob == PCGRL_PROB_BINARY && P.group == 16 && !P.big) {
        bucket = (inl || sure_done) ? 0 : (bucket < 1 ? 1 : bucket);
        block_append_bucketed((chg && !cheap) || inl, bucket, val, B, parity, WL_CHG, s_hist, s_gbase, cheap, inc_item, B.champ != nullptr ? WL_INC : -1);
        if (!B.inline_reset) block_append(rst, e, B, parity, WL_RST, s_cnt[1], &s_base[1]);
    } else {
        const bool first = B.inline_reset ? (inl || sure_done) : rst;
        int dest = -1, v = e;
        if (first) { dest = 2; v = val; }
        else if (chg) { dest = cheap ? 1 : 0; v = (cheap || B.zelda_inc) ? inc_item : e; }
        if (P.prob == PCGRL_PROB_BINARY && P.group == 64 && !P.big) {
            block_append_bucketed(dest == 0, bucket, v, B, parity, WL_CHG, s_hist, s_gbase, dest == 1, v, WL_INC);
            block_append(dest == 2, v, B, parity, WL_RST, s_cnt[1], &s_base[1]);
            return;
        }
        if (P.prob == PCGRL_PROB_SMB && dest == 1) dest = 0;
        else if (P.prob == PCGRL_PROB_SMB && dest == 0 && B.sok_cnt[e] >= SMB_LONG_POPS) dest = 1;
        block_append3(dest, v, B, parity, s_cnt, s_base);
    }
}

template <int REP, class MaskT>
__global__ __launch_bounds__(PCGRL_BLOCK) void k_update_block(PcgrlParams P, DevBufs B, const int32_t* __restrict__ actions, int parity) {
    __shared__ int s_cnt[2][4];
    __shared__ int s_base[2];
    const int e = blockIdx.x * PCGRL_BLOCK + threadIdx.x;
    bool act = e < P.num_envs;
    bool chg = false, rst = false, sure_done = false;
    if (B.pending) {
        const int pv = act ? (int)B.pending[e] : 1;
        act = pv == 0;
        const int cnt = __popcll(__ballot(act));
        if ((threadIdx.x & 63) == 0 && cnt) atomicAdd(B.async_stats + 8 + 8 * (blockIdx.x & 15), (unsigned long long)cnt);
        if (pv == 2) { rst = true; B.pending[e] = 0; }
        if (B.row.took && e < P.num_envs) B.row.took[e] = act ? 1 : 0;
        async_list_runnable(B, e);
    }
    const int ash = B.act_i64;
    if (act) {
        const int W = P.width, H = P.height, G = P.group, NPL = P.nplanes, NT = P.ntiles;
        const int2 c = reinterpret_cast<const int2*>(B.counters)[e];
        const uchar2 p0 = reinterpret_cast<const uchar2*>(B.pos)[e];
        const int iter = c.x + 1;
        int changes = c.y, x = p0.x, y = p0.y;
        int vals[9];
#pragma unroll
        for (int i = 0; i < 9; i++) vals[i] = -1;
        bool bad = false;
        if (REP == PCGRL_REP_NARROW_MULTI) {
#pragma unroll
            for (int i = 0; i < 9; i++) { const int raw = actions[(size_t)(9 * e + i) << ash], a = clampi(raw, 0, NT); bad = bad || a != raw; vals[i] = a - 1; }
        } else {
            const int type = actions[(size_t)(2 * e) << ash], raw_value = actions[(size_t)(2 * e + 1) << ash], value = clampi(raw_value, 0, NT - 1);
            bad = value != raw_value || type < 0 || type > (REP == PCGRL_REP_NARROW_CAST ? 2 : 5);
            if (REP == PCGRL_REP_NARROW_CAST) {
                const int t = clampi(type, 0, 2);
                if (t == 1) vals[4] = value;
                if (t == 2) { for (int i = 0; i < 9; i++) vals[i] = value; }
            } else {
                const int t = clampi(type, 0, 5);
                if (t < 4) {
                    const int dx = (t == 0) ? -1 : (t == 1 ? 1 : 0), dy = (t == 2) ? -1 : (t == 3 ? 1 : 0);
                    x += dx;
                    if (x < 0) x = P.warp ? x + W : 0;
                    if (x >= W) x = P.warp ? x - W : W - 1;
                    y += dy;
                    if (y < 0) y = P.warp ? y + H : 0;
                    if (y >= H) y = P.warp ? y - H : H - 1;
                }
                if (t == 4) vals[4] = value;
                if (t == 5) { for (int i = 0; i < 9; i++) vals[i] = value; }
            }
        }
        int change = 0;
        uint8_t* map_e = B.map + (size_t)e * H * W;
        MaskT* pl_e = reinterpret_cast<MaskT*>(B.planes) + (size_t)e * NPL * G;
#pragma unroll
        for (int dy = -1; dy <= 1; dy++) {
            const int yy = y + dy;
            if (yy < 0 || yy >= H) continue;
            if (vals[(dy + 1) * 3] < 0 && vals[(dy + 1) * 3 + 1] < 0 && vals[(dy + 1) * 3 + 2] < 0) continue;
            MaskT m0 = NPL > 0 ? pl_e[yy * NPL] : (MaskT)0, m1 = NPL > 1 ? pl_e[yy * NPL + 1] : (MaskT)0, m2 = NPL > 1 ? pl_e[yy * NPL + 2] : (MaskT)0;
            bool touched = false;
#pragma unroll
            for (int dx = -1; dx <= 1; dx++) {
                const int xx = x + dx, v = vals[(dy + 1) * 3 + dx + 1];
                if (xx < 0 || xx >= W || v < 0) continue;
                uint8_t* cell = map_e + yy * W + xx;
                if (*cell != v) {
                    change++;
                    touched = true;
                    *cell = (uint8_t)v;
                    const MaskT bit = (MaskT)1 << xx;
                    m0 = (v & 1) ? (m0 | bit) : (m0 & ~bit);
                    m1 = (v & 2) ? (m1 | bit) : (m1 & ~bit);
                    m2 = (v & 4) ? (m2 | bit) : (m2 & ~bit);
                }
            }
            if (touched && NPL > 0) { pl_e[yy * NPL] = m0; if (NPL > 1) { pl_e[yy * NPL + 1] = m1; pl_e[yy * NPL + 2] = m2; } }
        }
        if (REP != PCGRL_REP_TURTLE_CAST) {
            if (P.random_tile) {
                uint32_t* ring = B.rng_rep + (size_t)e * PCGRL_MT_N;
                int cur = B.rng_cur[2 * e];
                x = mt_randint(ring, cur, W);
                y = mt_randint(ring, cur, H);
                B.rng_cur[2 * e] = cur;
            } else {
                x += 1;
                if (x >= W) { x = 0; y += 1; if (y >= H) y = 0; }
            }
        }
        if (change > 0) {
            chg = true;
            changes += change;
            heat_increment(B, ((size_t)e * H + y) * W + x);
        }
        reinterpret_cast<int2*>(B.counters)[e] = make_int2(iter, changes);
        reinterpret_cast<uchar2*>(B.pos)[e] = make_uchar2((unsigned char)x, (unsigned char)y);
        if (bad) atomicOr(B.status, PCGRL_STATUS_BAD_ACTION);
        if (!chg) {
            int32_t s[PCGRL_MAX_STATS], st[PCGRL_MAX_STATS];
            int32_t* inf = B.info + (size_t)e * 10;
            for (int k = 0; k < 8; k++) { s[k] = B.stats[(size_t)e * 8 + k]; st[k] = B.start_stats[(size_t)e * 8 + k]; inf[k] = s[k]; }
            const bool d = episode_over(P, s, st) || changes >= P.max_changes || iter >= P.max_iterations;
            B.reward[e] = 0.0;
            B.done[e] = d ? 1 : 0;
            episode_account(B, e, 0.0, d);
            if (P.prob == PCGRL_PROB_BINARY) inf[2] = s[1] - st[1];
            inf[8] = iter; inf[9] = changes;
            rst = d && P.auto_reset;
        }
    }
    const bool inl = rst && B.inline_reset;
    if (B.inline_reset) {
        const bool first = inl || sure_done;
        block_append2(chg && !first, e, WL_CHG, first, inl ? (e | WL_RESET_ONLY) : e, WL_RST, B, parity, s_cnt, s_base);
    } else {
        block_append2(chg, e, WL_CHG, rst, e, WL_RST, B, parity, s_cnt, s_base);
    }
}
```

gym_pcgrl_amd/csrc/pcgrl_abi.hip:

```cpp
#include <hip/hip_runtime.h>
#include <stdio.h>
#include <stdlib.h>
#include <string.h>

#include <type_traits>
#include <vector>

#include "../../include/pcgrl_hip.h"

#ifdef PCGRL_PART
#define PCGRL_IN_PART(k) (PCGRL_PART == (k))
#else
#define PCGRL_IN_PART(k) 1
#endif
#define PCGRL_LOCAL __attribute__((visibility("hidden")))
#define PART_CORE 0
#define PART_STATS 1
#define PART_UPDATE 2
#define PART_STEP_BINARY 3
#define PART_STEP_ZELDA 4
#define PART_SEARCH 5
#define PART_SMB 6
#define PART_STEP_SOLVER 7

#include "lanegroup_dev.h"
#include "mt19937.h"
#include "pcgrl_algos.h"
#include "path_trace.h"
#include "sokoban_solver.h"
#include "sokoban_fast.h"
#include "mdungeon_solver.h"
#include "mdungeon_fast.h"
#include "ddave_solver.h"
#include "ddave_fast.h"
#include "level_build_wave.h"

#include "worklist.h"
#include "kernels_update.h"
#include "kernels_obs.h"
#include "reset_env.h"
#include "kernels_stats.h"
#include "kernels_reset.h"
#include "bigmap.h"
#include "bigmap_team.h"
#include "kernels_big.h"
#include "kernels_step.h"
#include "search_game.h"
#include "kernels_sokoban.h"
#include "kernels_agents4.h"
#include "kernels_smb.h"
#include "kernels_step_solver.h"
#include "kernels_search_async.h"
#include "kernels_evaluate.h"
#include "kernels_changes.h"
#include "kernels_paths.h"
#include "kernels_moves.h"
#include "kernels_smb_play.h"
#include "search_big.h"
#include "kernels_search_big.h"
#if PCGRL_IN_PART(PART_CORE)
#include "kernels_misc.h"
#include "kernels_render.h"
#endif

#if PCGRL_IN_PART(PART_CORE)
PCGRL_LOCAL thread_local int g_last_hip = 0;
#else
extern PCGRL_LOCAL thread_local int g_last_hip;
#endif
#if PCGRL_IN_PART(PART_CORE)
#include "step_pool.h"
#endif
struct BigArenaDims { int nblocks, nodes_cap, tsize, stride; size_t heap_off, table_off, block_bytes; };
struct pcgrl_env {
    BigArenaDims big_dims;
    pcgrl_config cfg;
    PcgrlParams P;
    pcgrl_layout L;
    DevBufs B;
    int bound;
    int has_old;
    int was_reset;
    int parity;
    int device;
    int alloc_solver_power;
    int smb_replay;
    pcgrl_tuning tun;
    int no_wide, wide_waves, wide_grid, wide_pairs, fused_zelda, no_fused, step_epb, smb_heap, obs_at_end, no_inc;
    int profiling;
    int obs_incremental;
    const uint8_t* obs_synced;
    int obs_hold;
    RowBind row; int row_on, row_i64, row_live;
    AsyncCtl async;
    int async_on, async_dirty, async_split;
    int big_team_waves;
    std::vector<hipEvent_t> events;
    size_t ev_used;
    int prof_steps;
};
static int gen_flag(const pcgrl_env* h) { return (h->P.random_start || !h->has_old) ? 1 : 0; }
#define PCGRL_NPHASE 6
static int prof_mark(pcgrl_env* h, hipStream_t st) {
    if (!h->profiling) return PCGRL_OK;
    if (h->ev_used == h->events.size()) {
        hipEvent_t e;
        if (hipEventCreate(&e) != hipSuccess) return PCGRL_EHIP;
        h->events.push_back(e);
    }
    if (hipEventRecord(h->events[h->ev_used++], st) != hipSuccess) return PCGRL_EHIP;
    return PCGRL_OK;
}

#define HIPCHK(expr) do { hipError_t err_ = (expr); if (err_ != hipSuccess) { g_last_hip = (int)err_; return PCGRL_EHIP; } } while (0)

static size_t align_up(size_t v, size_t a) { return (v + a - 1) / a * a; }
static int tun_or(int v, int dflt) { return v < 0 ? dflt : v; }

struct DeviceGuard {
    int prev, dev;
    explicit DeviceGuard(int d) : prev(-1), dev(d) {
        if (hipGetDevice(&prev) != hipSuccess) prev = -1;
        if (prev != dev) (void)hipSetDevice(dev);
    }
    ~DeviceGuard() { if (prev >= 0 && prev != dev) (void)hipSetDevice(prev); }
};

static bool solver_prob(int prob) { return prob == PCGRL_SOKOBAN || prob == PCGRL_MDUNGEON || prob == PCGRL_DDAVE || prob == PCGRL_SMB; }
#define PCGRL_MAX_DIM 255
#define PCGRL_MAX_DIM_WIDE 4096
#define PCGRL_BIG_LDS_BUDGET ((size_t)150 * 1024)
#define PCGRL_MAX_LEVEL_CELLS 16384
#define PCGRL_MAX_SOLVER_POWER 1000000
static bool big_map(const pcgrl_config* c) { return c->prob != PCGRL_SMB && (c->width > 64 || c->height > 64); }
static bool big_search(const pcgrl_config* c) {
    return solver_prob(c->prob) && c->prob != PCGRL_SMB && ((c->width + 2) * (c->height + 2) > 256 || c->solver_power > 16383);
}
static int validate_config(const pcgrl_config* c) {
    if (!c) return PCGRL_EINVAL;
    if (c->prob < 0 || c->prob > 5 || c->rep < 0 || c->rep > 5) return PCGRL_EINVAL;
    if (c->num_envs < 1) return PCGRL_EINVAL;
    if (c->prob == PCGRL_SMB) {
        if (c->width < 1 || c->width > 250 || c->height < 3 || c->height > SMB_MAX_H) return PCGRL_EINVAL;
    } else {
        const int max_dim = c->rep == PCGRL_REP_WIDE ? PCGRL_MAX_DIM_WIDE : PCGRL_MAX_DIM;
        if (c->width < 1 || c->width > max_dim || c->height < 1 || c->height > max_dim) return PCGRL_EINVAL;
        if (big_map(c)) {
            const int kw = (c->width + 63) >> 6;
            if (big_wave_lds(c->width, c->height) > PCGRL_BIG_LDS_BUDGET || (long long)big_words(c->width, c->height) * kw >= 65536) return PCGRL_EINVAL;
        }
    }
    if (c->max_changes < 1 || c->max_iterations < 1) return PCGRL_EINVAL;
    if (c->auto_reset && c->max_changes > 65535) return PCGRL_EINVAL;
    if (solver_prob(c->prob)) {
        if (c->prob != PCGRL_SMB && (c->width + 2) * (c->height + 2) > PCGRL_MAX_LEVEL_CELLS) return PCGRL_EINVAL;
        if (c->solver_power < 1 || c->solver_power > (c->prob == PCGRL_SMB ? 16383 : PCGRL_MAX_SOLVER_POWER)) return PCGRL_EINVAL;
    }
    return PCGRL_OK;
}
static int ntiles_of(int prob) { return prob == PCGRL_BINARY ? 2 : (prob == PCGRL_SOKOBAN ? 5 : ((prob == PCGRL_DDAVE || prob == PCGRL_SMB) ? 7 : 8)); }

static void fill_params(const pcgrl_config* c, PcgrlParams* P) {
    memset(P, 0, sizeof(*P));
    P->prob = c->prob; P->rep = c->rep; P->num_envs = c->num_envs;
    P->width = c->width; P->height = c->height;
    P->prob_width = c->prob_width > 0 ? c->prob_width : c->width;
    P->prob_height = c->prob_height > 0 ? c->prob_height : c->height;
    P->ntiles = ntiles_of(c->prob);
    P->big = big_map(c) ? 1 : 0;
    P->big_search = big_search(c) ? 1 : 0;
    P->nplanes = (c->prob == PCGRL_SMB || P->big) ? 0 : (c->prob == PCGRL_BINARY ? 1 : 3);
    P->group = c->height <= 16 ? 16 : 64;
    P->mask_bytes = c->width <= 32 ? 4 : 8;
    P->max_changes = c->max_changes; P->max_iterations = c->max_iterations;
    P->random_start = c->random_start; P->random_tile = c->random_tile; P->warp = c->warp;
    P->random_probs = c->random_probs; P->auto_reset = c->auto_reset;
    P->target_path = c->target_path; P->max_enemies = c->max_enemies; P->target_enemy_dist = c->target_enemy_dist;
    P->max_crates = c->max_crates; P->target_solution = c->target_solution; P->solver_power = c->solver_power;
    P->max_potions = c->max_potions; P->max_treasures = c->max_treasures; P->target_col_enemies = c->target_col_enemies;
    P->max_diamonds = c->max_diamonds; P->min_spikes = c->min_spikes; P->target_jumps = c->target_jumps;
    P->min_empty = c->min_empty; P->min_enemies = c->min_enemies; P->min_jumps = c->min_jumps;
    for (int i = 0; i < PCGRL_MAX_REWARDS; i++) P->rewards[i] = c->rewards[i];
    pcgrl_build_cdf(c->tile_probs, P->ntiles, P->cdf);
}

static const size_t WL_CNT_BYTES = 2 * WL_NLIST * WL_NSHARD * WL_CSTRIDE * sizeof(int32_t);
static int wl_capacity(int num_envs, int list) {
    return list == WL_CHG ? num_envs : 2 * ((num_envs + WL_NSHARD - 1) / WL_NSHARD + 256);
}
static size_t wl_list_bytes(int num_envs, int list) { return align_up((size_t)WL_NSHARD * wl_capacity(num_envs, list) * 4, 256); }
#define SOK_BLOCKS 256
enum { SOK_RES_WORDS = 16, SOK_CNT_WORDS = 1, SOK_STOP_WORDS = 1 };
static int sok_table_size(int power) { int t = 1024; while (t < 2 * power) t <<= 1; return t; }
static bool sok_in_lds(const pcgrl_config* c) { return c->solver_power <= SOK_LDS_POWER || c->prob == PCGRL_SMB; }
static size_t sok_heap_bytes(int power) { return align_up((4 * (size_t)power + 4) * 4, 256); }
static size_t sok_pool_bytes(const pcgrl_config* c) {
    const size_t full = 4 * (size_t)c->solver_power + 4, small = (size_t)SS_SEARCH_WAVES * SS_SMALL_NODES;
    size_t nodes = full > small ? full : small;
    if (c->prob == PCGRL_SMB)
        nodes = (SMB_MAX_WAVES * smb_wave_arena_bytes(c->solver_power) + sizeof(SokNode) - 1) / sizeof(SokNode);
    return align_up(nodes * sizeof(SokNode), 256);
}
static int play_trace_words(const pcgrl_config* c) { return (int)(align_up(sok_pool_bytes(c) / sizeof(SokNode) * 4, 256) / 4); }
static_assert(SS_SMALL_NODES >= 4 * SS_SMALL_POPS + 4, "a small-tier search pushes up to four nodes per pop");
static size_t champ_bytes(const pcgrl_config* c) {
    if (c->prob == PCGRL_SMB) return (c->rep <= PCGRL_REP_TURTLE && c->num_envs < SMB_KEEP_PLAY) ? align_up((size_t)c->num_envs * c->width * 4, 256) : 0;
    if (c->prob != PCGRL_BINARY) return 0;
    if (big_map(c))
        return (c->rep <= PCGRL_REP_TURTLE && c->width <= 256 && c->height <= 256 && c->num_envs <= WL_INCBIG_ENV_MASK + 1)
                   ? align_up((size_t)c->num_envs * big_words(c->width, c->height) * 8, 256) : 0;
    if (c->height <= 16) return (c->width <= 32 && c->num_envs <= WL_INC_ENV_MASK) ? align_up((size_t)c->num_envs * 64, 256) : 0;
    return c->num_envs <= WL_INC64_ENV_MASK ? align_up((size_t)c->num_envs * 64 * (c->width > 32 ? 8 : 4), 256) : 0;
}
static BigArenaDims big_arena_of(const pcgrl_config* c) {
    BigArenaDims A;
    const int cells = (c->width + 2) * (c->height + 2), nwb = (cells + 63) / 64, inner = c->width * c->height;
    A.nodes_cap = 4 * c->solver_power + 4;
    A.tsize = sok_table_size(c->solver_power);
    while (align_up((size_t)A.nodes_cap * 8, 256) + (size_t)A.tsize * 4 < (size_t)2 * cells) A.tsize <<= 1;
    A.stride = c->prob == PCGRL_SOKOBAN ? sokb_stride(inner < SOKB_MAXC ? inner : SOKB_MAXC) : mdb_stride(nwb);
    A.heap_off = align_up((size_t)A.nodes_cap * A.stride, 256);
    A.table_off = A.heap_off + align_up((size_t)A.nodes_cap * 8, 256);
    A.block_bytes = A.table_off + align_up((size_t)A.tsize * 4, 256);
    const size_t budget = (size_t)6 << 30;
    size_t nb = budget / A.block_bytes;
    nb = nb > SOK_BLOCKS ? SOK_BLOCKS : (nb < 4 ? 4 : nb);
    if (nb > (size_t)c->num_envs) nb = (size_t)c->num_envs;
    A.nblocks = (int)nb;
    return A;
}
struct Region { size_t off, bytes; };
struct Bump { size_t off; Region take(size_t bytes) { const Region r = {off, bytes}; off += bytes; return r; } };
template <class T> static T* at(uint8_t* base, Region r) { return r.bytes ? reinterpret_cast<T*>(base + r.off) : nullptr; }
struct ScratchPlan {
    Region wl_cnt, status, wl_items[WL_NLIST];
    Region arena;
    Region sok_env, sok_sync;
    Region sok_heap, sok_table;
    Region champ, fifo, fifo_tag, wide_sync;
    size_t total;
    BigArenaDims big;
};
static ScratchPlan scratch_plan(const pcgrl_config* c) {
    ScratchPlan S = {};
    Bump b = {0};
    S.wl_cnt = b.take(WL_CNT_BYTES);
    S.status = b.take(256);
    for (int k = 0; k < WL_NLIST; k++) S.wl_items[k] = b.take(wl_list_bytes(c->num_envs, k));
    if (solver_prob(c->prob)) {
        const bool big = big_search(c);
        if (big) S.big = big_arena_of(c);
        S.arena = b.take(big ? (size_t)S.big.nblocks * S.big.block_bytes : SOK_BLOCKS * sok_pool_bytes(c));
        S.sok_env = b.take(align_up((size_t)c->num_envs * (SOK_RES_WORDS + SOK_CNT_WORDS + SOK_STOP_WORDS) * 4, 256));
        S.sok_sync = b.take(align_up(2 * (size_t)(SOK_SY_WORDS + SOK_HARD_CAP) * 4, 256));
        if (!big && !sok_in_lds(c)) {
            S.sok_heap = b.take(SOK_BLOCKS * sok_heap_bytes(c->solver_power));
            S.sok_table = b.take(SOK_BLOCKS * (size_t)sok_table_size(c->solver_power) * 4);
        }
    }
    S.champ = b.take(champ_bytes(c));
    const size_t n = (size_t)c->num_envs;
    S.fifo = b.take(c->rep == PCGRL_NARROW ? align_up(n * PCGRL_FIFO_N * 4, 256) : 0);
    S.fifo_tag = b.take(c->rep == PCGRL_NARROW ? align_up(n * 4, 256) : 0);
    S.wide_sync = b.take((c->prob == PCGRL_BINARY && c->height > 16 && !big_map(c)) ? align_up(n * 16, 256) : 0);
    S.total = b.off;
    return S;
}

PCGRL_LOCAL int search_device_setup(pcgrl_env* h);
PCGRL_LOCAL int smb_device_setup(pcgrl_env* h);
#if PCGRL_IN_PART(PART_CORE)
static int device_setup(pcgrl_env* h) {
    {
        uint32_t tab[PCGRL_MT_N];
        tab[0] = 19650218u;
        for (int i = 1; i < PCGRL_MT_N; i++) tab[i] = 1812433253u * (tab[i - 1] ^ (tab[i - 1] >> 30)) + (uint32_t)i;
        HIPCHK(hipMemcpyToSymbol(HIP_SYMBOL(g_mt_genrand), tab, sizeof(tab)));
    }
    if (h->cfg.prob == PCGRL_SMB) return smb_device_setup(h);
    if (solver_prob(h->cfg.prob) && !big_search(&h->cfg)) return search_device_setup(h);
    return PCGRL_OK;
}

static void resolve_tuning(pcgrl_env* h) {
    const pcgrl_tuning& T = h->tun;
    DevBufs& B = h->B;
    h->no_wide = tun_or(T.no_wide, 0) ? 1 : 0;
    h->wide_waves = tun_or(T.wide_waves, 8);
    h->wide_pairs = tun_or(T.wide_pairs, 1);
    h->wide_grid = tun_or(T.wide_grid, 2048);
    if (h->wide_grid < 1) h->wide_grid = 2048;
    h->fused_zelda = tun_or(T.fused_zelda, 1) ? 1 : 0;
    h->no_fused = tun_or(T.no_fused, 0) ? 1 : 0;
    h->obs_at_end = tun_or(T.obs_at_end, 0) ? 1 : 0;
    h->async_split = tun_or(T.async_split, h->cfg.prob == PCGRL_SOKOBAN ? 1 : 0) ? 1 : 0;
    const int n_ = h->cfg.num_envs;
    h->step_epb = T.step_epb > 0 ? T.step_epb : ((n_ >= 192 * 256 && n_ <= 256 * 256) ? 256 : (n_ >= 192 * 128 ? 128 : 64));
    if (h->step_epb != 128 && h->step_epb != 256) h->step_epb = 64;
    h->smb_heap = T.smb_lds_heap > 0 ? T.smb_lds_heap : SMB_LDS_HEAP;
    if (h->smb_heap < 256 || h->smb_heap > 4096) h->smb_heap = SMB_LDS_HEAP;
    const int f = tun_or(T.full_per_wave, 4), i = tun_or(T.inc_per_wave, 4);
    B.step_fpw = (f == 1 || f == 2) ? f : 4;
    B.step_prio = tun_or(T.step_prio, h->cfg.prob == PCGRL_BINARY ? (h->cfg.rep == PCGRL_NARROW ? (15 | (3 << 6)) : 15) : 0) & 0xFFF;
    B.step_ipw = (i == 1 || i == 2) ? i : 4;
    B.step_touch = tun_or(T.no_touch, 0) ? 0 : 1;
    B.touch_resume = tun_or(T.touch_resume, 1) ? 1 : 0;
    B.step_pair = tun_or(T.step_pair, 6);
    B.step_tight = B.step_touch ? tun_or(T.touch_tight, 1) : 0;
    h->no_inc = tun_or(T.no_inc, 0) != 0;
    B.zelda_inc = (h->cfg.prob == PCGRL_ZELDA && h->cfg.rep <= PCGRL_REP_TURTLE && h->cfg.height <= 16 && h->cfg.width <= 32 &&
                   h->cfg.num_envs <= WL_INC_ENV_MASK && !h->no_inc) ? 1 : 0;
    B.pair_min = tun_or(T.pair_min, 2048);
    B.big_team = tun_or(T.big_team, 1) ? 1 : 0;
    h->big_team_waves = tun_or(T.big_team, 1) >= 2 ? (tun_or(T.big_team, 1) > BIG_TEAM_MAX_WAVES ? BIG_TEAM_MAX_WAVES : tun_or(T.big_team, 1)) : 4;
    B.wide_few = tun_or(T.wide_few, WL_WIDE_FEW_REGIONS);
    B.wide_spin = T.wide_spin > 0 ? T.wide_spin : WIDE_SPIN_LIMIT;
    B.inline_reset = (!solver_prob(h->cfg.prob) && tun_or(T.inline_reset, 1) != 0) ? 1 : 0;
    if (big_search(&h->cfg)) {
        B.sok_fast_maxc = -1; B.md_only_agent = -1; B.sok_hard_cap = 0; B.sok_spawn_iters = SOK_SPAWN_ITERS;
    } else if (solver_prob(h->cfg.prob)) {
        B.sok_fast_maxc = tun_or(T.sok_generic, 0) ? -1 : SOKF_MAXC;
        B.md_only_agent = T.md_only_agent;
        B.sok_hard_cap = tun_or(T.sok_hard_cap, SOK_HARD_CAP);
        B.sok_spawn_iters = T.sok_spawn > 0 ? T.sok_spawn : SOK_SPAWN_ITERS;
        if (B.sok_hard_cap > SOK_HARD_CAP) B.sok_hard_cap = SOK_HARD_CAP;
    }
}
static int bind_buffers(pcgrl_env* h, const pcgrl_buffers* b, hipStream_t st) {
    const pcgrl_config& c = h->cfg;
    DevBufs& B = h->B;
    B.map = (uint8_t*)b->map; B.old_map = (uint8_t*)b->old_map; B.heat = (uint16_t*)b->heatmap; B.pos = (uint8_t*)b->pos;
    B.heat_end = B.heat + (size_t)c.num_envs * c.width * c.height;
    B.heat32 = c.auto_reset ? 0 : 1;
    B.ep_return = nullptr; B.ep_length = nullptr; B.last_return = nullptr; B.last_length = nullptr;
    B.planes = b->planes; B.counters = (int32_t*)b->counters; B.stats = (int32_t*)b->stats;
    B.start_stats = (int32_t*)b->start_stats; B.info = (int32_t*)b->info; B.reward = (double*)b->reward;
    B.done = (uint8_t*)b->done; B.tile_p = (double*)b->tile_p; B.rng_rep = (uint32_t*)b->rng_rep;
    B.rng_prob = (uint32_t*)b->rng_prob; B.rng_cur = (int32_t*)b->rng_cursor;
    B.obs = ObsSpec{nullptr, 0, 0, 0, 0, 0, 0, 0};
    B.local = nullptr; B.flat = nullptr;
    const ScratchPlan S = scratch_plan(&c);
    uint8_t* s = (uint8_t*)b->scratch;
    B.wl_cnt = at<int32_t>(s, S.wl_cnt); B.status = at<int32_t>(s, S.status);
    for (int k = 0; k < WL_NLIST; k++) { B.wl_cap[k] = wl_capacity(c.num_envs, k); B.wl_items[k] = at<int32_t>(s, S.wl_items[k]); }
    HIPCHK(hipMemsetAsync(B.wl_cnt, 0, S.wl_cnt.bytes + S.status.bytes, st));
    B.champ = h->no_inc ? nullptr : at<uint8_t>(s, S.champ);
    if (B.champ) HIPCHK(hipMemsetAsync(B.champ, c.prob == PCGRL_SMB ? 0xFF : 0, S.champ.bytes, st));
    B.fifo = at<uint32_t>(s, S.fifo); B.fifo_tag = at<int32_t>(s, S.fifo_tag);
    if (B.fifo_tag) HIPCHK(hipMemsetAsync(B.fifo_tag, 0xFF, S.fifo_tag.bytes, st));
    B.wide_sync = at<int32_t>(s, S.wide_sync); B.wide_epoch = 0;
    if (B.wide_sync) HIPCHK(hipMemsetAsync(B.wide_sync, 0, S.wide_sync.bytes, st));
    const bool big = big_search(&c);
    B.big_arena = big ? at<uint8_t>(s, S.arena) : nullptr;
    B.sok_pool = big ? nullptr : at<SokNode>(s, S.arena);
    B.sok_heap = at<uint32_t>(s, S.sok_heap); B.sok_table = at<uint32_t>(s, S.sok_table);
    if (solver_prob(c.prob)) {
        const int power = h->alloc_solver_power = c.solver_power;
        h->big_dims = S.big;
        B.sok_res = at<int32_t>(s, S.sok_env);
        B.sok_cnt = B.sok_res + (size_t)c.num_envs * SOK_RES_WORDS;
        B.sok_stop = B.sok_cnt + (size_t)c.num_envs * SOK_CNT_WORDS;
        B.sok_sync = at<int32_t>(s, S.sok_sync);
        HIPCHK(hipMemsetAsync(B.sok_res, 0, S.sok_env.bytes + S.sok_sync.bytes, st));
        B.sok_use_lds = !big && sok_in_lds(&c);
        B.sok_table_size = big ? S.big.tsize : sok_table_size(power);
        B.sok_pool_stride = big ? 0 : (int32_t)(sok_pool_bytes(&c) / sizeof(SokNode));
        B.sok_heap_stride = big ? 0 : (int32_t)(sok_heap_bytes(power) / 4);
    }
    return PCGRL_OK;
}

extern "C" {

int pcgrl_abi_version(void) { return PCGRL_ABI_VERSION; }
int pcgrl_last_hip_error(void) { return g_last_hip; }
const char* pcgrl_error_string(int code) {
    switch (code) {
        case PCGRL_OK: return "ok";
        case PCGRL_EINVAL: return "invalid argument or unsupported configuration";
        case PCGRL_EHIP: return "HIP runtime error";
        case PCGRL_ESTATE: return "call order violated (bind, seed and reset before step)";
        default: return "unknown error";
    }
}

int pcgrl_query_layout(const pcgrl_config* c, pcgrl_layout* L) {
    int rc = validate_config(c);
    if (rc) return rc;
    if (!L) return PCGRL_EINVAL;
    PcgrlParams P;
    fill_params(c, &P);
    const size_t n = (size_t)c->num_envs, cells = (size_t)c->width * c->height;
    memset(L, 0, sizeof(*L));
    L->group = P.group; L->mask_bytes = P.mask_bytes; L->nplanes = P.nplanes; L->nstats = num_stats(c->prob);
    L->map = n * cells; L->old_map = n * cells; L->heatmap = n * cells * (c->auto_reset ? 2 : 4); L->pos = n * 2;
    L->planes = n * P.nplanes * P.group * P.mask_bytes;
    L->counters = n * 8; L->stats = n * 32; L->start_stats = n * 32; L->info = n * 40;
    L->reward = n * 8; L->done = n; L->tile_p = n * 16;
    L->rng_rep = n * PCGRL_MT_N * 4; L->rng_prob = c->prob == PCGRL_BINARY ? n * PCGRL_MT_N * 4 : 0;
    L->rng_cursor = n * 8;
    L->scratch = scratch_plan(c).total;
    return PCGRL_OK;
}

int pcgrl_create(const pcgrl_config* c, pcgrl_env** out) {
    int rc = validate_config(c);
    if (rc) return rc;
    if (!out) return PCGRL_EINVAL;
    pcgrl_env* h = new pcgrl_env();
    h->bound = h->has_old = h->was_reset = h->parity = h->device = 0;
    h->smb_replay = 0;
    h->profiling = 0; h->ev_used = 0; h->prof_steps = 0; h->obs_hold = 0; h->obs_incremental = 0; h->obs_synced = nullptr;
    memset(&h->row, 0, sizeof(h->row)); h->row_on = h->row_i64 = h->row_live = 0;
    memset(&h->async, 0, sizeof(h->async)); h->async_on = h->async_dirty = 0;
    memset(&h->B, 0, sizeof(h->B));
    pcgrl_tuning_defaults(&h->tun);
    h->cfg = *c;
    fill_params(c, &h->P);
    pcgrl_query_layout(c, &h->L);
    *out = h;
    return PCGRL_OK;
}

void pcgrl_tuning_defaults(pcgrl_tuning* t) {
    if (!t) return;
    int32_t* f = reinterpret_cast<int32_t*>(t);
    for (size_t i = 0; i < sizeof(pcgrl_tuning) / sizeof(int32_t); i++) f[i] = -1;
}
int pcgrl_set_tuning(pcgrl_env* h, const pcgrl_tuning* t) {
    if (!h || !t) return PCGRL_EINVAL;
    if (h->bound) return PCGRL_ESTATE;
    h->tun = *t;
    return PCGRL_OK;
}

int pcgrl_destroy(pcgrl_env* h) {
    if (h) {
        for (hipEvent_t e : h->events) (void)hipEventDestroy(e);
    }
    delete h;
    return PCGRL_OK;
}

int pcgrl_bind(pcgrl_env* h, const pcgrl_buffers* b, void* stream) {
    if (!h || !b) return PCGRL_EINVAL;
    if (!b->map || !b->old_map || !b->heatmap || !b->pos || !b->planes || !b->counters || !b->stats ||
        !b->start_stats || !b->info || !b->reward || !b->done || !b->tile_p || !b->rng_rep || !b->rng_cursor || !b->scratch)
        return PCGRL_EINVAL;
    if (h->cfg.prob == PCGRL_BINARY && !b->rng_prob) return PCGRL_EINVAL;
    {
        hipPointerAttribute_t at;
        if (hipPointerGetAttributes(&at, b->map) == hipSuccess) h->device = at.device;
        else { (void)hipGetLastError(); HIPCHK(hipGetDevice(&h->device)); }
    }
    DeviceGuard guard(h->device);
    int rc = device_setup(h);
    if (rc) return rc;
    resolve_tuning(h);
    if ((rc = bind_buffers(h, b, (hipStream_t)stream))) return rc;
    h->bound = 1; h->has_old = 0; h->was_reset = 0; h->parity = 0;
    h->async_on = h->async_dirty = 0;
    return PCGRL_OK;
}

int pcgrl_configure(pcgrl_env* h, const pcgrl_config* c) {
    if (!h) return PCGRL_EINVAL;
    int rc = validate_config(c);
    if (rc) return rc;
    if (c->prob != h->cfg.prob || c->rep != h->cfg.rep || c->num_envs != h->cfg.num_envs ||
        c->width != h->cfg.width || c->height != h->cfg.height)
        return PCGRL_EINVAL;
    if (h->bound && solver_prob(c->prob) && c->solver_power > h->alloc_solver_power) return PCGRL_EINVAL;
    const bool was_big = h->bound && h->P.big_search;
    if (h->bound && big_search(c) && !was_big) return PCGRL_EINVAL;
    if (h->bound && c->prob == PCGRL_SMB && c->solver_power != h->cfg.solver_power) h->smb_replay = 1;
    h->cfg = *c;
    fill_params(c, &h->P);
    if (was_big) h->P.big_search = 1;
    return PCGRL_OK;
}

int pcgrl_set_tile_probs(pcgrl_env* h, void* stream) {
    if (!h || !h->bound) return PCGRL_ESTATE;
    DeviceGuard guard(h->device);
    const int n = h->cfg.num_envs;
    hipLaunchKernelGGL(k_bcast_tile_p, dim3((n + 255) / 256), dim3(256), 0, (hipStream_t)stream, h->B.tile_p, n,
                       h->cfg.tile_probs[0], h->cfg.tile_probs[1]);
    HIPCHK(hipGetLastError());
    return PCGRL_OK;
}

int pcgrl_seed(pcgrl_env* h, const uint32_t* keys, int32_t first, int32_t count, void* stream) {
    if (!h || !h->bound) return PCGRL_ESTATE;
    if (!keys || first < 0 || count < 1 || first + count > h->cfg.num_envs) return PCGRL_EINVAL;
    DeviceGuard guard(h->device);
    const size_t bytes = (size_t)count * PCGRL_MT_N * 4, off = (size_t)first * PCGRL_MT_N;
    HIPCHK(hipMemcpyAsync(h->B.rng_rep + off, keys, bytes, hipMemcpyHostToDevice, (hipStream_t)stream));
    if (h->B.fifo_tag) HIPCHK(hipMemsetAsync(h->B.fifo_tag + first, 0xFF, (size_t)count * 4, (hipStream_t)stream));
    if (h->B.rng_prob) HIPCHK(hipMemcpyAsync(h->B.rng_prob + off, keys, bytes, hipMemcpyHostToDevice, (hipStream_t)stream));
    hipLaunchKernelGGL(k_zero_cursors, dim3((count + 255) / 256), dim3(256), 0, (hipStream_t)stream, h->B.rng_cur, first, count);
    HIPCHK(hipGetLastError());
    HIPCHK(hipStreamSynchronize((hipStream_t)stream));
    return PCGRL_OK;
}

int pcgrl_seed_words(pcgrl_env* h, const uint32_t* words, int32_t first, int32_t count, void* stream) {
    if (!h || !h->bound) return PCGRL_ESTATE;
    if (!words || first < 0 || count < 1 || first + count > h->cfg.num_envs) return PCGRL_EINVAL;
    DeviceGuard guard(h->device);
    hipStream_t st = (hipStream_t)stream;
    HIPCHK(hipMemcpy2DAsync(h->B.rng_rep + (size_t)first * PCGRL_MT_N, PCGRL_MT_N * 4, words, 12, 12, (size_t)count, hipMemcpyHostToDevice, st));
    if (h->B.fifo_tag) HIPCHK(hipMemsetAsync(h->B.fifo_tag + first, 0xFF, (size_t)count * 4, st));
    hipLaunchKernelGGL(k_init_by_array, dim3((count + 63) / 64), dim3(64), 0, st, h->B.rng_rep, h->B.rng_prob, h->B.rng_cur, first, count);
    HIPCHK(hipGetLastError());
    HIPCHK(hipStreamSynchronize(st));
    return PCGRL_OK;
}

}
#endif

struct RolloutArgs { int steps; size_t action_stride; double* reward_out; uint8_t* done_out; int32_t* info_out; };
PCGRL_LOCAL int launch_stats(pcgrl_env* h, int list, int parity, int mode, int clr, int inline_reset, hipStream_t st);
PCGRL_LOCAL int launch_reset(pcgrl_env* h, int list, int park_list, int parity, int clr, hipStream_t st);
PCGRL_LOCAL int launch_planes_from_map(pcgrl_env* h, const uint8_t* maps, hipStream_t st);
PCGRL_LOCAL int launch_update(pcgrl_env* h, const int32_t* actions, int parity, hipStream_t st);
PCGRL_LOCAL int launch_step_binary(pcgrl_env* h, const int32_t* actions, int parity, hipStream_t st, const RolloutArgs& R);
PCGRL_LOCAL int launch_step_zelda(pcgrl_env* h, const int32_t* actions, int parity, hipStream_t st, const RolloutArgs& R);
PCGRL_LOCAL int launch_search(pcgrl_env* h, int32_t* sync, int list_a, int mode_a, int list_b, int mode_b, int parity, int rst_list, int clr, hipStream_t st);
PCGRL_LOCAL int launch_smb(pcgrl_env* h, int32_t* sync, int list_a, int mode_a, int list_b, int mode_b, int parity, int rst_list, int clr, hipStream_t st, int inline_reset);
PCGRL_LOCAL int launch_step_solver(pcgrl_env* h, const int32_t* actions, hipStream_t st, const RolloutArgs& R, int epb);
PCGRL_LOCAL int launch_get_stats(pcgrl_env* h, const uint8_t* maps, int count, int32_t* rows_out, int32_t* head, int32_t* jobs, hipStream_t st);
PCGRL_LOCAL int launch_get_stats_search(pcgrl_env* h, const uint8_t* maps, int32_t* rows_out, int32_t* head, const int32_t* jobs, SokNode* pools, int blocks, hipStream_t st);
PCGRL_LOCAL int launch_get_paths(pcgrl_env* h, const uint8_t* maps, int count, int max_len, int16_t* cells_out, int32_t* length_out, int32_t* rows_out, hipStream_t st);
struct ChangesArgs {
    const uint8_t* maps; int count; const int32_t* cells; int ncells; const int32_t* start_rows;
    int32_t* base_rows; int32_t* rows; double* reward; uint8_t* over;
    int chunk, nchunks, grid_cap;
};
PCGRL_LOCAL int launch_get_changes(pcgrl_env* h, const ChangesArgs& A, int32_t* head, int32_t* jobs, hipStream_t st);
static int changes_group(const PcgrlParams& P) { return (P.group == 16 && P.mask_bytes == 8) ? 64 : P.group; }
PCGRL_LOCAL int launch_get_changes_search(pcgrl_env* h, const ChangeJobs& src, int32_t* head, const int32_t* jobs, SokNode* pools, int blocks, hipStream_t st);
PCGRL_LOCAL int launch_get_moves(pcgrl_env* h, const uint8_t* maps, int32_t* rows_out, const SolOut& out, int32_t* head, const int32_t* jobs, SokNode* pools, uint32_t* traces, int blocks, hipStream_t st);
PCGRL_LOCAL int launch_smb_play(pcgrl_env* h, const uint8_t* maps, int count, int32_t* rows_out, const SolOut& out, int32_t* ticket, uint8_t* arenas, int slots, hipStream_t st);
PCGRL_LOCAL int launch_search_async(pcgrl_env* h, int32_t* tickets, int list_a, int mode_a, int list_b, int mode_b, int parity, int rst_list, int clr, int budget, int resume, int small, hipStream_t st);
template <auto KFN>
static int lds_cap(int device, size_t lds) {
    static size_t cap[64];
    if (lds <= 64 * 1024) return PCGRL_OK;
    const int d = device & 63;
    if (lds > cap[d]) {
        HIPCHK(hipFuncSetAttribute(reinterpret_cast<const void*>(KFN), hipFuncAttributeMaxDynamicSharedMemorySize, (int)lds));
        cap[d] = lds;
    }
    return PCGRL_OK;
}
template <class... Params, class... Args>
static int launch_fn(void (*kfn)(Params...), int grid, int block, size_t lds, hipStream_t st, const Args&... args) {
    hipLaunchKernelGGL(kfn, dim3(grid), dim3(block), lds, st, args...);
    HIPCHK(hipGetLastError());
    return PCGRL_OK;
}
template <auto KFN, class... Args>
static int launch(pcgrl_env* h, int grid, int block, size_t lds, hipStream_t st, const Args&... args) {
    { const int rc = lds_cap<KFN>(h->device, lds); if (rc) return rc; }
    return launch_fn(KFN, grid, block, lds, st, args...);
}
static int grid_for(int items, int per_block, int cap) {
    int g = (items + per_block - 1) / per_block;
    if (g < 1) g = 1;
    return g < cap ? g : cap;
}
template <int V> using Int = std::integral_constant<int, V>;
template <class T> struct Type { using type = T; };
template <class Tag> using type_of = typename Tag::type;
template <int... VS, class F>
static int with_value(int v, F&& f) {
    int rc = PCGRL_EINVAL;
    (void)(... || (v == VS ? (rc = f(Int<VS>{}), true) : false));
    return rc;
}
template <int... PROBS, class F> static int with_prob(int prob, F&& f) { return with_value<PROBS...>(prob, f); }
template <int... REPS, class F> static int with_rep(int rep, F&& f) { return with_value<REPS...>(rep, f); }
template <class F> static int with_mask(int mask_bytes, F&& f) { return mask_bytes == 4 ? f(Type<uint32_t>{}) : f(Type<uint64_t>{}); }
template <class F>
static int with_lanes(int group, int mask_bytes, F&& f) {
    if (group == 16) return with_mask(mask_bytes, [&](auto m) { return f(Int<16>{}, m); });
    return with_mask(mask_bytes, [&](auto m) { return f(Int<64>{}, m); });
}

#if PCGRL_IN_PART(PART_STATS)
template <int PROB>
static int launch_stats_p(pcgrl_env* h, int list, int parity, int mode, int clr, int inline_reset, hipStream_t st) {
    const PcgrlParams& P = h->P;
    const int gpb = PCGRL_BLOCK / P.group;
    const int grid = grid_for(P.num_envs, gpb, 8192);
    const size_t lds = inline_reset ? 4 * (size_t)reset_stage_bytes(P.width * P.height) : 0;
    const int gen = gen_flag(h);
    const int lone0 = !(mode == MODE_STEP && inline_reset) ? 0 : ((PROB == PCGRL_PROB_BINARY && P.group == 16 && P.rep <= PCGRL_REP_TURTLE) ? 1 : 2);
    if (PROB == PCGRL_PROB_BINARY && P.group == 64 && !h->no_wide) {
        const int nw = h->wide_waves;
        const size_t set1 = reset_stage_bytes(P.width * P.height);
        const size_t need1 = set1 + (size_t)8 * P.width * P.height + 8 * ((size_t)(P.width * P.height + 63) / 64 + 2);
        const size_t sets1 = (size_t)(nw == 8 ? 8 : 4) * set1;
        const size_t lds1 = inline_reset ? (sets1 > need1 ? sets1 : need1) : 0;
        int gridw = P.num_envs < h->wide_grid ? P.num_envs : h->wide_grid;
        if (gridw > 1) gridw &= ~1;
        h->B.wide_epoch = (h->B.wide_epoch % 0x3FFFFFFF) + 1;
        const int pair_few = (mode == MODE_STEP && list == WL_CHG && P.rep <= PCGRL_REP_TURTLE && h->wide_pairs) ? 1 : 0;
// ... 1103 lines not shown
```

gym_pcgrl_amd/csrc/pcgrl_algos.h:

```cpp
#pragma once
#include "pcgrl_common.h"

#if defined(__HIPCC__) && defined(__HIP_DEVICE_COMPILE__)
#define PCGRL_NO_IFCVT() asm volatile("" ::: "memory")
#else
#define PCGRL_NO_IFCVT() do {} while (0)
#endif
#ifndef PCGRL_TRACE
#define PCGRL_TRACE(g, site)
#endif

struct PcgrlParams {
    int32_t prob, rep, num_envs, width, height, ntiles, nplanes, group, mask_bytes;
    int32_t max_changes, max_iterations;
    int32_t random_start, random_tile, warp, random_probs, auto_reset;
    int32_t target_path, max_enemies, target_enemy_dist, max_crates, target_solution, solver_power;
    int32_t prob_width, prob_height;
    int32_t max_potions, max_treasures;
    int32_t max_diamonds, min_spikes, target_jumps;
    int32_t min_empty, min_enemies, min_jumps;
    int32_t big, big_search;
    double target_col_enemies;
    double rewards[PCGRL_MAX_REWARDS];
    double cdf[PCGRL_MAX_TILES];
};

PCGRL_HD double range_reward(double nv, double ov, double lo, double hi) {
    if (nv >= lo && nv <= hi && ov >= lo && ov <= hi) return 0.0;
    if (ov <= hi && nv <= hi) return (nv < lo ? nv : lo) - (ov < lo ? ov : lo);
    if (ov >= lo && nv >= lo) return (ov > hi ? ov : hi) - (nv > hi ? nv : hi);
    if (nv > hi && ov < lo) return hi - nv + ov - lo;
    return hi - ov + nv - lo;
}
#define PCGRL_INF (__builtin_huge_val())

#define PCGRL_IPOS 2147483647
#define PCGRL_INEG (-2147483647 - 1)
PCGRL_HD int range_reward_i(int nv, int ov, int lo, int hi) {
    if (nv >= lo && nv <= hi && ov >= lo && ov <= hi) return 0;
    if (ov <= hi && nv <= hi) return (nv < lo ? nv : lo) - (ov < lo ? ov : lo);
    if (ov >= lo && nv >= lo) return (ov > hi ? ov : hi) - (nv > hi ? nv : hi);
    if (nv > hi && ov < lo) return hi - nv + ov - lo;
    return hi - ov + nv - lo;
}

PCGRL_HD int pcgrl_sat255(int n) { return n > 255 ? 255 : n; }
PCGRL_HD int md_won(const int32_t* s) { return (s[7] >> 24) & 1; }
PCGRL_HD int md_dist_win(const int32_t* s) { return md_won(s) ? 0 : s[6]; }
PCGRL_HD int md_sol_length(const int32_t* s) { return md_won(s) ? s[6] : 0; }
PCGRL_HD int md_col_potions(const int32_t* s) { return s[7] & 255; }
PCGRL_HD int md_col_treasures(const int32_t* s) { return (s[7] >> 8) & 255; }
PCGRL_HD int md_col_enemies(const int32_t* s) { return (s[7] >> 16) & 255; }
PCGRL_HD void md_pack(int32_t* s, const int* out5) {
    const int won = out5[1] > 0 ? 1 : 0;
    s[6] = won ? out5[1] : out5[0];
    s[7] = pcgrl_sat255(out5[2]) | (pcgrl_sat255(out5[3]) << 8) | (pcgrl_sat255(out5[4]) << 16) | (won << 24);
}

PCGRL_HD int dd_player(const int32_t* s) { return s[0] & 255; }
PCGRL_HD int dd_exit(const int32_t* s) { return (s[0] >> 8) & 255; }
PCGRL_HD int dd_key(const int32_t* s) { return (s[0] >> 16) & 255; }
PCGRL_HD void dd_pack(int32_t* s, const int* out4) {
    const int won = out4[1] > 0 ? 1 : 0;
    s[5] = out4[2];
    s[6] = won ? out4[1] : out4[0];
    s[7] = pcgrl_sat255(out4[3]) | (won << 24);
}

PCGRL_HD double compute_reward(const PcgrlParams& P, const int32_t* n, const int32_t* o, int prob) {
#ifdef PCGRL_EXP_NOREWARD
    return (double)(n[0] - o[0]);
#endif
    const double* w = P.rewards;
    if (prob == PCGRL_PROB_BINARY) {
        return (double)range_reward_i(n[0], o[0], 1, 1) * w[0] + (double)(n[1] - o[1]) * w[1];
    } else if (prob == PCGRL_PROB_ZELDA) {
        double r = (double)range_reward_i(n[0], o[0], 1, 1) * w[0];
        r = r + (double)range_reward_i(n[1], o[1], 1, 1) * w[1];
        r = r + (double)range_reward_i(n[2], o[2], 1, 1) * w[2];
        r = r + (double)range_reward_i(n[3], o[3], 2, P.max_enemies) * w[4];
        r = r + (double)range_reward_i(n[4], o[4], 1, 1) * w[3];
        r = r + (double)range_reward_i(n[5], o[5], P.target_enemy_dist, PCGRL_IPOS) * w[5];
        r = r + (double)range_reward_i(n[6], o[6], PCGRL_IPOS, PCGRL_IPOS) * w[6];
        return r;
    } else if (prob == PCGRL_PROB_DDAVE) {
        double r = (double)range_reward_i(dd_player(n), dd_player(o), 1, 1) * w[0];
        r = r + (double)range_reward_i(n[1], o[1], 0, 0) * w[1];
        r = r + (double)range_reward_i(dd_exit(n), dd_exit(o), 1, 1) * w[2];
        r = r + (double)range_reward_i(n[3], o[3], P.min_spikes, PCGRL_IPOS) * w[5];
        r = r + (double)range_reward_i(n[2], o[2], PCGRL_INEG, P.max_diamonds) * w[3];
        r = r + (double)range_reward_i(dd_key(n), dd_key(o), 1, 1) * w[4];
        r = r + (double)range_reward_i(n[4], o[4], 1, 1) * w[6];
        r = r + (double)range_reward_i(n[5], o[5], PCGRL_IPOS, PCGRL_IPOS) * w[7];
        r = r + (double)range_reward_i(md_dist_win(n), md_dist_win(o), PCGRL_INEG, PCGRL_INEG) * w[8];
        r = r + (double)range_reward_i(md_sol_length(n), md_sol_length(o), PCGRL_IPOS, PCGRL_IPOS) * w[9];
        return r;
    } else if (prob == PCGRL_PROB_SMB) {
        double r = (double)range_reward_i(n[0], o[0], 0, 0) * w[0];
        r = r + (double)range_reward_i(n[1], o[1], 0, 0) * w[1];
        r = r + (double)range_reward_i(n[2], o[2], P.min_enemies, P.max_enemies) * w[2];
        r = r + (double)range_reward_i(n[3], o[3], P.min_empty, PCGRL_IPOS) * w[3];
        r = r + (double)range_reward_i(n[4], o[4], 0, 0) * w[4];
        r = r + (double)range_reward_i(n[5], o[5], P.min_jumps, PCGRL_IPOS) * w[5];
        r = r + (double)range_reward_i(n[6], o[6], 0, 0) * w[6];
        r = r + (double)range_reward_i(n[7], o[7], 0, 0) * w[7];
        return r;
    } else if (prob == PCGRL_PROB_MDUNGEON) {
        double r = (double)range_reward_i(n[0], o[0], 1, 1) * w[0];
        r = r + (double)range_reward_i(n[1], o[1], 1, 1) * w[1];
        r = r + (double)range_reward_i(n[4], o[4], 1, P.max_enemies) * w[4];
        r = r + (double)range_reward_i(n[3], o[3], PCGRL_INEG, P.max_treasures) * w[3];
        r = r + (double)range_reward_i(n[2], o[2], PCGRL_INEG, P.max_potions) * w[2];
        r = r + (double)range_reward_i(n[5], o[5], 1, 1) * w[5];
        r = r + (double)range_reward_i(md_col_enemies(n), md_col_enemies(o), PCGRL_IPOS, PCGRL_IPOS) * w[6];
        r = r + (double)range_reward_i(md_dist_win(n), md_dist_win(o), PCGRL_INEG, PCGRL_INEG) * w[7];
        r = r + (double)range_reward_i(md_sol_length(n), md_sol_length(o), PCGRL_IPOS, PCGRL_IPOS) * w[8];
        return r;
    } else {
        int nr = n[1] - n[2], orr = o[1] - o[2];
        nr = nr < 0 ? -nr : nr; orr = orr < 0 ? -orr : orr;
        double r = (double)range_reward_i(n[0], o[0], 1, 1) * w[0];
        r = r + (double)range_reward_i(n[1], o[1], 1, P.max_crates) * w[1];
        r = r + (double)range_reward_i(n[2], o[2], 1, P.max_crates) * w[2];
        r = r + (double)range_reward_i(n[3], o[3], 1, 1) * w[3];
        r = r + (double)range_reward_i(nr, orr, PCGRL_INEG, PCGRL_INEG) * w[4];
        r = r + (double)range_reward_i(n[4], o[4], PCGRL_INEG, PCGRL_INEG) * w[5];
        r = r + (double)range_reward_i(n[5], o[5], PCGRL_IPOS, PCGRL_IPOS) * w[6];
        return r;
    }
}
PCGRL_HD double compute_reward(const PcgrlParams& P, const int32_t* n, const int32_t* o) { return compute_reward(P, n, o, P.prob); }
PCGRL_HD bool episode_over(const PcgrlParams& P, const int32_t* n, const int32_t* start, int prob) {
    if (prob == PCGRL_PROB_BINARY) return n[0] == 1 && n[1] - start[1] >= P.target_path;
    if (prob == PCGRL_PROB_ZELDA) return n[5] >= P.target_enemy_dist && n[6] >= P.target_path;
    if (prob == PCGRL_PROB_DDAVE) return md_sol_length(n) >= P.target_solution && n[5] > P.target_jumps;
    if (prob == PCGRL_PROB_SMB) return n[7] <= 0;
    if (prob == PCGRL_PROB_MDUNGEON) {
        const int en = n[4] > 1 ? n[4] : 1;
        return md_sol_length(n) >= P.target_solution && n[4] > 0 && (double)md_col_enemies(n) / (double)en > P.target_col_enemies;
    }
    return n[5] >= P.target_solution;
}
PCGRL_HD bool episode_over(const PcgrlParams& P, const int32_t* n, const int32_t* start) { return episode_over(P, n, start, P.prob); }
PCGRL_HD int num_stats(int prob) { return prob == PCGRL_PROB_BINARY ? 2 : (prob == PCGRL_PROB_ZELDA ? 7 : (prob == PCGRL_PROB_SOKOBAN ? 6 : 8)); }

template <class WordT>
PCGRL_HD void planes_set_cell(WordT& m0, WordT& m1, WordT& m2, int x, int t) {
    const WordT keep = ~((WordT)1 << x);
    m0 = (m0 & keep) | ((WordT)(t & 1) << x);
    m1 = (m1 & keep) | ((WordT)((t >> 1) & 1) << x);
    m2 = (m2 & keep) | ((WordT)((t >> 2) & 1) << x);
}

template <class B>
PCGRL_D typename B::mask_t pcg_expand(B& g, typename B::mask_t f) {
    return f | (f << 1) | (f >> 1) | g.up(f) | g.down(f);
}
template <class B>
PCGRL_D typename B::mask_t pcg_neighbours(B& g, typename B::mask_t f) {
    return (f << 1) | (f >> 1) | g.up(f) | g.down(f);
}

template <class B>
PCGRL_D typename B::mask_t pcg_fill_rows(B& g, typename B::mask_t s, typename B::mask_t p, typename B::mask_t rp) {
    typedef typename B::mask_t M;
    M hi = (((p + s) ^ p) & p) | s;
    M rs = g.bitrev(s);
    M lo = (((rp + rs) ^ rp) & rp) | rs;
    return hi | g.bitrev(lo);
}

template <class B>
struct PcgFillCtx {
    typename B::mask_t pass, rpass;
    typename B::mask_t dn[B::kLog2Group], up[B::kLog2Group];
};
template <class B>
PCGRL_D PcgFillCtx<B> pcg_fill_ctx(B& g, typename B::mask_t pass) {
    PcgFillCtx<B> c;
    c.pass = pass;
    c.rpass = g.bitrev(pass);
    c.dn[0] = pass; c.up[0] = pass;
#pragma unroll
    for (int k = 1; k < B::kLog2Group; k++) {
        c.dn[k] = c.dn[k - 1] & g.rows_down(c.dn[k - 1], k - 1);
        c.up[k] = c.up[k - 1] & g.rows_up(c.up[k - 1], k - 1);
    }
    return c;
}
template <class B>
PCGRL_D typename B::mask_t pcg_fill_cols(B& g, typename B::mask_t f, const PcgFillCtx<B>& c) {
    typename B::mask_t d = f, u = f;
#pragma unroll
    for (int k = 0; k < B::kLog2Group; k++) {
        d = d | (c.dn[k] & g.rows_down(d, k));
        u = u | (c.up[k] & g.rows_up(u, k));
    }
    typename B::mask_t r = d | u;
    if (B::kGroup > 16) r = r | (c.pass & (g.up(r) | g.down(r)));
    return r;
}

template <class B>
PCGRL_D typename B::mask_t pcg_component_fills(B& g, typename B::mask_t seed, const PcgFillCtx<B>& c) {
    typedef typename B::mask_t M;
    M f = pcg_fill_rows(g, seed, c.pass, c.rpass);
    for (;;) {
        M n = pcg_fill_cols(g, f, c);
        f = pcg_fill_rows(g, n, c.pass, c.rpass);
        if (!g.wave_any(pcg_neighbours(g, f) & c.pass & ~f)) break;
    }
    return f;
}

template <class B>
PCGRL_D typename B::mask_t pcg_component(B& g, typename B::mask_t seed, const PcgFillCtx<B>& c) {
    typedef typename B::mask_t M;
    PCGRL_TRACE(g, 1);
    if (B::kGroup != 16) {
        M f = seed;
        for (int i = 0; i < 4; i++) {
            M n = pcg_expand(g, f) & c.pass;
            n = pcg_expand(g, n) & c.pass;
            if (!g.wave_any(n ^ f)) return f;
            f = n;
        }
        seed = f;
    }
    return pcg_component_fills(g, seed, c);
}

template <class B>
PCGRL_D typename B::mask_t pcg_tiny_components(B& g, typename B::mask_t p, int& regions, int& path) {
    typedef typename B::mask_t M;
    const M a = (p << 1) & p, b = (p >> 1) & p, c = g.up(p) & p, d = g.down(p) & p;
    const M s0 = a ^ b, c0 = a & b, s1 = c ^ d, c1 = c & d;
    const M n0 = s0 ^ s1, k = s0 & s1;
    const M two_or_more = c0 | c1 | k;
    const M iso = p & ~(a | b | c | d);
    const M deg1 = n0 & ~two_or_more;
    const M deg2 = ~n0 & (c0 ^ c1 ^ k) & ~(c0 & c1);
    const M dom = deg1 & pcg_neighbours(g, deg1);
    const M e1 = deg1 << 1, e2 = deg1 >> 1, e3 = g.up(deg1), e4 = g.down(deg1);
    const M centre = deg2 & ((e1 & e2) | (e3 & e4) | ((e1 | e2) & (e3 | e4)));
    const M ends = deg1 & pcg_neighbours(g, centre);
    int n_iso, n_dom, n_tri;
    g.popcount_sum3(iso, dom, centre, n_iso, n_dom, n_tri);
    regions += n_iso + (n_dom >> 1) + n_tri;
    const int tiny_path = n_tri > 0 ? 2 : (n_dom > 0 ? 1 : 0);
    path = tiny_path > path ? tiny_path : path;
    return iso | dom | centre | ends;
}

template <bool WANT_LAST = true, class B>
PCGRL_D int bfs_levels(B& g, typename B::mask_t src, typename B::mask_t pass, typename B::mask_t& last) {
    typedef typename B::mask_t M;
    typedef typename B::ivec_t I;
    if constexpr (B::kHistBfs != 0) {
        M n = src, prev = src ^ src;
        I hist = g.izero(), last_it = g.izero();
        int it = 0;
        PCGRL_TRACE(g, 2);
        while (g.template bfs_run<WANT_LAST>(n, pass, hist, prev, it)) { last_it = g.hist_fold(hist, it, last_it); hist = g.izero(); }
        last_it = g.hist_fold(hist, it, last_it);
        const int ecc = g.imax(last_it);
        if (WANT_LAST) last = g.keep_where_eq(last_it, ecc, n & ~prev);
        return ecc;
    }
    M f = src, prev = src ^ src;
    I last_it = g.izero();
    int it = 0;
    constexpr int kLevels = B::kGroup == 16 ? 2 : 4;
    PCGRL_TRACE(g, 2);
    for (;;) {
        M n = f;
        bool more = false;
#if defined(__HIPCC__)
#pragma unroll
#endif
        for (int uu = 0; uu < kLevels; uu++) {
            ++it;
            const M nn = pcg_expand(g, n) & pass;
            last_it = g.isel_ne(nn, n, it, last_it);
            prev = g.msel_ne(nn, n, n, prev);
            if (uu == kLevels - 1) more = g.wave_any(nn ^ n);
            n = nn;
        }
        f = n;
        if (!more) break;
    }
    const int ecc = g.imax(last_it);
    last = g.keep_where_eq(last_it, ecc, f & ~prev);
    return ecc;
}

template <class B>
PCGRL_D int bfs_dist(B& g, typename B::mask_t src, typename B::mask_t dst, typename B::mask_t pass) {
    typedef typename B::mask_t M;
    M f = src;
    int t = 0;
    for (;;) {
        const M n1 = pcg_expand(g, f) & pass, fresh1 = n1 & ~f;
        const M n2 = pcg_expand(g, n1) & pass, fresh2 = n2 & ~n1;
        if (g.any((fresh1 | fresh2) & dst)) return g.any(fresh1 & dst) ? t + 1 : t + 2;
        if (!g.any(fresh2)) return -1;
        t += 2;
        f = n2;
    }
}

template <class B>
PCGRL_D int count_regions(B& g, typename B::mask_t pass) {
    typedef typename B::mask_t M;
    int regions = 0, dummy = 0;
    M rest = pass & ~pcg_tiny_components(g, pass, regions, dummy);
    if (!g.any(rest)) return regions;
    const PcgFillCtx<B> ctx = pcg_fill_ctx(g, pass);
    while (g.any(rest)) {
        M comp = pcg_component(g, g.first_bit(rest), ctx);
        rest = rest & ~comp;
        ++regions;
    }
    return regions;
}

template <class B>
PCGRL_D int pcg_double_sweep(B& g, typename B::mask_t comp, int best, int& bound) {
#ifdef PCGRL_EXP_NOSWEEP
    return bound = g.popcount_sum(comp) / 4 + 1;
#endif
    typename B::mask_t last, unused;
    const int e1 = bfs_levels(g, g.first_bit(comp), comp, last);
    if (2 * e1 <= best) { bound = 2 * e1; return 0; }
    return bound = bfs_levels<false>(g, g.first_bit(last), comp, unused);
}
template <class B>
PCGRL_D int pcg_double_sweep(B& g, typename B::mask_t comp, int best) {
#ifdef PCGRL_EXP_NOSWEEP
    return g.popcount_sum(comp) / 4 + 1;
#endif
    typename B::mask_t last, unused;
    const int e1 = bfs_levels(g, g.first_bit(comp), comp, last);
    if (2 * e1 <= best) return 0;
    return bfs_levels<false>(g, g.first_bit(last), comp, unused);
}

template <class B>
PCGRL_D void regions_and_longest_path(B& g, typename B::mask_t pass, int& regions, int& path, typename B::mask_t& champ, int& ub2, bool tight = true) {
    typedef typename B::mask_t M;
    regions = 0;
    path = 0;
    ub2 = -1;
    champ = pass ^ pass;
    const M nontiny = pass & ~pcg_tiny_components(g, pass, regions, path);
    if (!g.any(nontiny)) return;
    const PcgFillCtx<B> ctx = pcg_fill_ctx(g, pass);
    if (B::kGroup != 16) {
        typedef typename B::ivec_t I;
        M rest = nontiny;
        const I cnt = g.popc_lanes(rest);
        M seed = g.first_bit(g.keep_where_eq(cnt, g.imax(cnt), rest));
        while (g.any(rest)) {
            const M comp = pcg_component(g, seed, ctx);
            rest = rest & ~comp;
            ++regions;
            if (g.popcount_sum(comp) - 1 > path) { const int e = pcg_double_sweep(g, comp, path); if (e > path) { path = e; champ = comp; } }
            seed = g.first_bit(rest);
        }
        return;
    }
    M rest = nontiny, big1 = nontiny ^ nontiny, big2 = big1;
    int size1 = 0, size2 = 0, size3 = 0;
    while (g.any(rest)) {
        const M comp = pcg_component(g, g.first_bit(rest), ctx);
        rest = rest & ~comp;
        ++regions;
        const int size = g.popcount_sum(comp);
        if (size > size1) { size3 = size2; size2 = size1; big2 = big1; size1 = size; big1 = comp; }
        else if (size > size2) { size3 = size2; size2 = size; big2 = comp; }
        else if (size > size3) size3 = size;
    }
    const int tiny_path = path;
    int bd1 = size1 - 1, bd2 = size2 - 1, who = 0;
    if (size1 - 1 > path) { const int e = pcg_double_sweep(g, big1, path, bd1); if (e > path) { path = e; champ = big1; who = 1; } }
    {
        const int rest_b = size3 - 1 > tiny_path ? size3 - 1 : tiny_path;
        if (size2 - 1 > path) { const int e = pcg_double_sweep(g, big2, path, bd2); if (e > path) { path = e; champ = big2; who = 2; } }
        else if (tight && size2 - 1 > rest_b) pcg_double_sweep(g, big2, rest_b, bd2);
    }
    if (size3 - 1 > path) {
        rest = nontiny & ~big1 & ~big2;
        while (g.any(rest)) {
            const M comp = pcg_component(g, g.first_bit(rest), ctx);
            rest = rest & ~comp;
            if (g.popcount_sum(comp) - 1 > path) { const int e = pcg_double_sweep(g, comp, path); if (e > path) { path = e; champ = comp; who = 3; } }
        }
    }
    const int b1 = who == 1 ? 0 : bd1, b2 = who == 2 ? 0 : bd2, b3 = size3 - 1;
    ub2 = tiny_path;
    ub2 = b1 > ub2 ? b1 : ub2; ub2 = b2 > ub2 ? b2 : ub2; ub2 = b3 > ub2 ? b3 : ub2;
    ub2 = ub2 > path ? path : ub2;
}
template <class B>
PCGRL_D void regions_and_longest_path(B& g, typename B::mask_t pass, int& regions, int& path, typename B::mask_t& champ) {
    int ub2;
    regions_and_longest_path(g, pass, regions, path, champ, ub2);
}
template <class B>
PCGRL_D void regions_and_longest_path(B& g, typename B::mask_t pass, int& regions, int& path) {
    typename B::mask_t champ;
    regions_and_longest_path(g, pass, regions, path, champ);
}

template <class B>
PCGRL_D void binary_incremental(B& g, typename B::mask_t pass_new, typename B::mask_t cbit, bool added, int regions_old, int path_old,
                                typename B::mask_t champ_old, int ub2_old, int& regions, int& path, typename B::mask_t& champ, int& ub2) {
    typedef typename B::mask_t M;
    const M base = pass_new & ~cbit;
    M rest = pcg_neighbours(g, cbit) & base;
    path = path_old;
    champ = champ_old;
    constexpr bool kTrack = B::kGroup == 16;
    const bool track = kTrack && ub2_old >= 0;
    int k = 0, ub = track ? ub2_old : 0;
    M uni = cbit;
    if (g.any(rest)) {
        const PcgFillCtx<B> ctx = pcg_fill_ctx(g, base);
        while (g.any(rest)) {
            const M comp = pcg_component(g, g.first_bit(rest), ctx);
            rest = rest & ~comp;
            ++k;
            if (added) uni = uni | comp;
            else {
                int bd = g.popcount_sum(comp) - 1, e = 0;
                const int thr = track ? ub : path;
                if (bd > thr) e = pcg_double_sweep(g, comp, thr, bd);
                if (e > path) { if (kTrack) ub = path > ub ? path : ub; path = e; champ = comp; }
                else if (kTrack) ub = bd > ub ? bd : ub;
            }
        }
    }
    if (added) {
        regions = regions_old + 1 - k;
        int bd = g.popcount_sum(uni) - 1, e = 0;
        const int thr = track ? ub : path;
        if (bd > thr) e = pcg_double_sweep(g, uni, thr, bd);
// ... 350 lines not shown
```

gym_pcgrl_amd/csrc/worklist.h:

```cpp
#pragma once
#define PCGRL_BLOCK 256
#define PCGRL_STATUS_TOO_MANY_CRATES 1
#define PCGRL_STATUS_BAD_ACTION 2
#define PCGRL_STATUS_BAD_TILE 4
enum { MODE_STEP = 0, MODE_START = 1, MODE_SETMAP = 2 };

#define WL_NSHARD 64
#define WL_WIDE_FEW_REGIONS 32
#define WL_CSTRIDE 16
enum { WL_CHG = 0, WL_RST = 1, WL_SOL = 2, WL_SOL2 = 3, WL_RST2 = 4, WL_SOL3 = 5, WL_INC = 6, WL_NLIST = 7 };
#ifndef SMB_LONG_POPS
#define SMB_LONG_POPS 2000
#endif
#define WL_INC_ENV_MASK 0x1FFFFF
#define WL_INC64_ENV_MASK 0x7FFFF
__device__ __forceinline__ int wl_inc_pack(int group, int e, int row, int col, unsigned code) {
    return group == 16 ? (int)((unsigned)e | ((unsigned)(row * 32 + col) << 21) | (code << 30))
                       : (int)((unsigned)e | ((unsigned)(row * 64 + col) << 19) | ((code & 1u) << 31));
}
#define WL_INCBIG_ENV_MASK 0x7FFF
__device__ __forceinline__ int wl_incbig_pack(int e, int x, int y, bool added) { return (int)((unsigned)e | ((unsigned)x << 15) | ((unsigned)y << 23) | (added ? 0x80000000u : 0u)); }
template <int G> __device__ __forceinline__ int wl_inc_env(int raw) { return raw & (G == 16 ? WL_INC_ENV_MASK : WL_INC64_ENV_MASK); }
template <int G> __device__ __forceinline__ int wl_inc_row(int raw) { return G == 16 ? ((raw >> 26) & 15) : ((raw >> 25) & 63); }
template <int G> __device__ __forceinline__ int wl_inc_col(int raw) { return G == 16 ? ((raw >> 21) & 31) : ((raw >> 19) & 63); }
template <int G> __device__ __forceinline__ unsigned wl_inc_code(int raw) { return G == 16 ? (((unsigned)raw >> 30) & 3u) : ((unsigned)raw >> 31); }
#define WL_RESET_ONLY (1 << 30)
#define SMB_KEEP_PLAY (1 << 29)
#define SMB_REPLAY 0x7F7F7F7F

#if defined(PCGRL_TIMELINE) || defined(PCGRL_SMB_PROF) || defined(PCGRL_BIG_PROF) || defined(PCGRL_WIDE_TL)
__device__ unsigned long long* g_tl_buf;
#endif
#ifdef PCGRL_WIDE_TL
#define WTL(i, v) do { if (threadIdx.x == 0 && g_tl_buf) g_tl_buf[(size_t)blockIdx.x * 8 + (i)] = (unsigned long long)(v); } while (0)
#else
#define WTL(i, v) do {} while (0)
#endif
#ifdef PCGRL_TIMELINE
#define TL_SLOTS 48
__shared__ int s_tl_idx[16];
__device__ __forceinline__ void tl_mark(int tag) {
    if ((threadIdx.x & 63) == 0 && g_tl_buf) {
        const int wv = threadIdx.x >> 6;
        const int i = s_tl_idx[wv];
        if (i < TL_SLOTS) { g_tl_buf[((size_t)blockIdx.x * (blockDim.x >> 6) + wv) * TL_SLOTS + i] = ((unsigned long long)wall_clock64() << 8) | (unsigned)tag; s_tl_idx[wv] = i + 1; }
    }
}
#define TL_INIT() do { if ((threadIdx.x & 63) == 0) s_tl_idx[threadIdx.x >> 6] = 0; } while (0)
#define TL(tag) tl_mark(tag)
#else
#define TL_INIT() do {} while (0)
#define TL(tag) do {} while (0)
#endif

struct LocalLists;
struct ObsSpec { uint8_t* out; int32_t oh, ow, depth, centered, pad;
                 int32_t fused,
                         delta; };
struct RowBind { int64_t* actions_out; double* reward; uint8_t* done; const uint8_t* start_in; uint8_t* start_out;
                 double* ep_return; int32_t* ep_length; uint8_t* took; uint8_t* fresh; };
struct DevBufs {
    uint8_t* map; uint8_t* old_map; uint16_t* heat; uint8_t* pos; void* planes;
    void* champ;
    int32_t* wide_sync;
    int32_t wide_spin;
    int32_t wide_few;
    int32_t wide_epoch;
    const uint16_t* heat_end;
    double* ep_return; int32_t* ep_length; double* last_return; int32_t* last_length;
    int32_t* counters; int32_t* stats; int32_t* start_stats; int32_t* info;
    double* reward; uint8_t* done; double* tile_p;
    uint32_t* rng_rep; uint32_t* rng_prob; int32_t* rng_cur;
    int32_t* wl_cnt;
    int32_t* wl_items[WL_NLIST];
    int32_t wl_cap[WL_NLIST];
    SokNode* sok_pool; uint32_t* sok_heap; uint32_t* sok_table; int32_t* status;
    int32_t* sok_res;
    int32_t* sok_cnt; int32_t* sok_stop;
    struct LocalLists* local;
    int32_t md_only_agent;
    int32_t* sok_sync;
    int32_t sok_pool_stride, sok_heap_stride, sok_table_size, sok_use_lds;
    int32_t sok_spawn_iters;
    int32_t sok_hard_cap;
    int32_t sok_fast_maxc;
    int32_t inline_reset;
    int32_t pair_min;
    int32_t zelda_inc;
    uint32_t* fifo; int32_t* fifo_tag;
    ObsSpec obs;
    int32_t step_fpw, step_ipw;
    int32_t step_prio;
    int32_t step_tight;
    const int32_t* flat;
    int32_t step_pair;
    int32_t big_team;
    int32_t touch_resume;
    int32_t step_touch;
    uint8_t* big_arena;
    uint8_t* pending; unsigned long long* async_stats;
    const uint8_t* async_slots; size_t async_slot_bytes; int32_t async_nslots; int32_t* async_run; int32_t* async_run_n;
    int32_t heat32;
    RowBind row; int32_t act_i64;
};
#define PCGRL_FIFO_N 8

struct ZeldaRewardTab { double w[8]; int lo[8]; int hi[8]; };
struct ObsView {
    uint8_t* out;
    int oh, ow, depth, centered, pad, W, H;
};
struct StepLocal {
    int e0;
    int par, need;
    int refill_done[2];
    int pend[256];
    int late_done[4];
    uint8_t dirty[256];
    uint8_t obs_skip[256];
    uint8_t late[256];
    int n_late;
    ObsView obs_v;
    ZeldaRewardTab zr;
};

__device__ __forceinline__ void async_list_runnable(const DevBufs& B, int gi) {
    if (gi < B.async_nslots && __hip_atomic_load(reinterpret_cast<const int32_t*>(B.async_slots + (size_t)gi * B.async_slot_bytes), __ATOMIC_RELAXED, __HIP_MEMORY_SCOPE_AGENT) == 1)
        B.async_run[atomicAdd(B.async_run_n, 1)] = gi;
}
__device__ __forceinline__ int32_t* wl_counters(const DevBufs& B, int parity, int list) {
    return B.wl_cnt + (size_t)(parity * WL_NLIST + list) * WL_NSHARD * WL_CSTRIDE;
}
#define WL_LOCAL_CAP 512
struct LocalLists { int n[WL_NLIST]; int e0; uint16_t items[WL_NLIST][WL_LOCAL_CAP]; };
__device__ __forceinline__ void wl_push(const DevBufs& B, int parity, int list, int shard, int value) {
    if (B.local) {
        const int i = atomicAdd(&B.local->n[list], 1);
        B.local->items[list][i] = (uint16_t)(value - B.local->e0);
        return;
    }
    const int i = atomicAdd(wl_counters(B, parity, list) + shard * WL_CSTRIDE, 1);
    B.wl_items[list][(size_t)shard * B.wl_cap[list] + i] = value;
}
__device__ __forceinline__ int wl_load_prefix(const DevBufs& B, int parity, int list, int* s_pref) {
    if (threadIdx.x < WL_NSHARD) {
        int v = wl_counters(B, parity, list)[threadIdx.x * WL_CSTRIDE];
        for (int o = 1; o < WL_NSHARD; o <<= 1) {
            const int t = __shfl_up(v, o, 64);
            if ((int)threadIdx.x >= o) v += t;
        }
        s_pref[threadIdx.x + 1] = v;
        if (threadIdx.x == 0) s_pref[0] = 0;
    }
    __syncthreads();
    return s_pref[WL_NSHARD];
}
__device__ __forceinline__ int wl_load_prefix3(const DevBufs& B, int parity, int list_a, int list_b, int list_c, int* s_pref_a,
                                               int* s_pref_b, int* s_pref_c, int* n_b, int* n_c) {
    if (threadIdx.x < 3 * WL_NSHARD) {
        const int t = threadIdx.x & (WL_NSHARD - 1), k = threadIdx.x >> 6;
        const int list = k == 0 ? list_a : (k == 1 ? list_b : list_c);
        int v = list >= 0 ? wl_counters(B, parity, list)[t * WL_CSTRIDE] : 0;
        for (int o = 1; o < WL_NSHARD; o <<= 1) {
            const int u = __shfl_up(v, o, 64);
            if (t >= o) v += u;
        }
        int* sp = k == 0 ? s_pref_a : (k == 1 ? s_pref_b : s_pref_c);
        sp[t + 1] = v;
        if (t == 0) sp[0] = 0;
    }
    __syncthreads();
    *n_b = s_pref_b[WL_NSHARD];
    *n_c = s_pref_c[WL_NSHARD];
    return s_pref_a[WL_NSHARD];
}
__device__ __forceinline__ int wl_get(const DevBufs& B, int list, const int* s_pref, int i) {
    int lo = 0;
#pragma unroll
    for (int step = WL_NSHARD / 2; step > 0; step >>= 1)
        if (s_pref[lo + step] <= i) lo += step;
    return B.wl_items[list][(size_t)lo * B.wl_cap[list] + (i - s_pref[lo])];
}
__device__ __forceinline__ void wl_clear(const DevBufs& B, int parity) {
    for (int i = threadIdx.x; i < WL_NLIST * WL_NSHARD; i += blockDim.x) wl_counters(B, parity, 0)[i * WL_CSTRIDE] = 0;
}

__device__ __forceinline__ void block_append(bool flag, int value, const DevBufs& B, int parity, int list,
                                             int* s_cnt, int* s_base) {
    const int lane = threadIdx.x & 63, w = threadIdx.x >> 6;
    const int shard = blockIdx.x & (WL_NSHARD - 1);
    const uint64_t m = __ballot(flag);
    if (lane == 0) s_cnt[w] = __popcll(m);
    __syncthreads();
    if (threadIdx.x == 0) {
        int tot = s_cnt[0] + s_cnt[1] + s_cnt[2] + s_cnt[3];
        *s_base = tot ? atomicAdd(wl_counters(B, parity, list) + shard * WL_CSTRIDE, tot) : 0;
    }
    __syncthreads();
    if (flag) {
        int off = *s_base;
        for (int i = 0; i < w; i++) off += s_cnt[i];
        off += __popcll(m & ((1ull << lane) - 1ull));
        B.wl_items[list][(size_t)shard * B.wl_cap[list] + off] = value;
    }
}

__device__ __forceinline__ void block_append2(bool flag_a, int value_a, int list_a, bool flag_b, int value_b, int list_b,
                                              const DevBufs& B, int parity, int (*s_cnt)[4], int* s_base) {
    const int lane = threadIdx.x & 63, w = threadIdx.x >> 6;
    const int shard = blockIdx.x & (WL_NSHARD - 1);
    const uint64_t ma = __ballot(flag_a), mb = __ballot(flag_b);
    if (lane == 0) { s_cnt[0][w] = __popcll(ma); s_cnt[1][w] = __popcll(mb); }
    __syncthreads();
    if (threadIdx.x == 0 || threadIdx.x == 64) {
        const int k = threadIdx.x >> 6;
        const int tot = s_cnt[k][0] + s_cnt[k][1] + s_cnt[k][2] + s_cnt[k][3];
        s_base[k] = tot ? atomicAdd(wl_counters(B, parity, k ? list_b : list_a) + shard * WL_CSTRIDE, tot) : 0;
    }
    __syncthreads();
    if (flag_a || flag_b) {
        const int k = flag_a ? 0 : 1;
        const int list = k ? list_b : list_a;
        int off = s_base[k];
        for (int i = 0; i < w; i++) off += s_cnt[k][i];
        off += __popcll((k ? mb : ma) & ((1ull << lane) - 1ull));
        B.wl_items[list][(size_t)shard * B.wl_cap[list] + off] = k ? value_b : value_a;
    }
}

__device__ __forceinline__ void block_append3(int dest, int value, const DevBufs& B, int parity, int (*s_cnt)[4], int* s_base) {
    const int lane = threadIdx.x & 63, w = threadIdx.x >> 6;
    const int shard = blockIdx.x & (WL_NSHARD - 1);
    const uint64_t m0 = __ballot(dest == 0), m1 = __ballot(dest == 1), m2 = __ballot(dest == 2);
    if (lane == 0) { s_cnt[0][w] = __popcll(m0); s_cnt[1][w] = __popcll(m1); s_cnt[2][w] = __popcll(m2); }
    __syncthreads();
    if ((threadIdx.x & 63) == 0 && threadIdx.x < 192) {
        const int k = threadIdx.x >> 6;
        const int list = k == 0 ? WL_CHG : (k == 1 ? WL_INC : WL_RST);
        const int tot = s_cnt[k][0] + s_cnt[k][1] + s_cnt[k][2] + s_cnt[k][3];
        s_base[k] = tot ? atomicAdd(wl_counters(B, parity, list) + shard * WL_CSTRIDE, tot) : 0;
    }
    __syncthreads();
    if (dest >= 0) {
        const int list = dest == 0 ? WL_CHG : (dest == 1 ? WL_INC : WL_RST);
        const uint64_t m = dest == 0 ? m0 : (dest == 1 ? m1 : m2);
        int off = s_base[dest];
        for (int i = 0; i < w; i++) off += s_cnt[dest][i];
        off += __popcll(m & ((1ull << lane) - 1ull));
        B.wl_items[list][(size_t)shard * B.wl_cap[list] + off] = value;
    }
}

__device__ __forceinline__ void block_append_bucketed(bool flag, int bucket, int value, const DevBufs& B, int parity, int list,
                                                      int* s_hist, int* s_gbase, bool flag2 = false, int value2 = 0, int list2 = -1) {
    if (threadIdx.x <= WL_NSHARD) s_hist[threadIdx.x] = 0;
    __syncthreads();
    int rank = 0;
    if (flag) rank = atomicAdd(&s_hist[bucket], 1);
    else if (flag2) rank = atomicAdd(&s_hist[WL_NSHARD], 1);
    __syncthreads();
    const int shard2 = blockIdx.x & (WL_NSHARD - 1);
    if (threadIdx.x < WL_NSHARD) {
        const int c = s_hist[threadIdx.x];
        if (c > 0) s_gbase[threadIdx.x] = atomicAdd(wl_counters(B, parity, list) + threadIdx.x * WL_CSTRIDE, c);
    } else if (threadIdx.x == WL_NSHARD && list2 >= 0) {
        const int c = s_hist[WL_NSHARD];
        if (c > 0) s_gbase[WL_NSHARD] = atomicAdd(wl_counters(B, parity, list2) + shard2 * WL_CSTRIDE, c);
    }
    __syncthreads();
    if (flag) B.wl_items[list][(size_t)bucket * B.wl_cap[list] + s_gbase[bucket] + rank] = value;
    else if (flag2) B.wl_items[list2][(size_t)shard2 * B.wl_cap[list2] + s_gbase[WL_NSHARD] + rank] = value2;
}
__device__ __forceinline__ int difficulty_bucket(const PcgrlParams& P, const int4& s0, const int4& s1, int B_few = WL_WIDE_FEW_REGIONS) {
    if (P.prob == PCGRL_PROB_BINARY && P.group == 64) {
        const int cost = (max(s0.x, 0) + max(s0.y, 0)) / 12;
        const int half = WL_NSHARD / 2;
        return (s0.x <= B_few ? half : 0) + half - 1 - min(cost, half - 1);
    }
    if (P.prob == PCGRL_PROB_BINARY) {
        const int a = min(max(s0.y, 0) / 6, 7), b = min(max(s0.x, 0) / 3, 7);
        return a * 8 + b;
    }
    const int regions = P.prob == PCGRL_PROB_ZELDA ? s1.x : s0.w;
    return min(max(regions, 0), WL_NSHARD - 1);
}

__device__ __forceinline__ void episode_account(const DevBufs& B, int e, double r, bool d) {
    if (!B.ep_return) return;
    double R = B.ep_return[e] + r;
    int L = B.ep_length[e] + 1;
    if (d) { B.last_return[e] = R; B.last_length[e] = L; R = 0.0; L = 0; }
    B.ep_return[e] = R; B.ep_length[e] = L;
}

template <bool AR_ONLY = false>
__device__ __forceinline__ void heat_increment(const DevBufs& B, size_t idx) {
    if (!AR_ONLY && B.heat32) { atomicAdd(reinterpret_cast<uint32_t*>(B.heat) + idx, 1u); return; }
    uint16_t* cell = B.heat + idx;
    const uintptr_t a = reinterpret_cast<uintptr_t>(cell);
    uint32_t* word = reinterpret_cast<uint32_t*>(a & ~(uintptr_t)3);
    if (reinterpret_cast<uintptr_t>(word) + 4 <= reinterpret_cast<uintptr_t>(B.heat_end)) atomicAdd(word, 1u << ((a & 2) * 8));
    else *cell += 1;
}
template <bool AR_ONLY = false>
__device__ __forceinline__ void heat_clear(const DevBufs& B, int e, int cells, int t, int step) {
    const int sh = AR_ONLY ? 0 : B.heat32;
    uint16_t* heat_g = B.heat + ((size_t)e * cells << sh);
    const int n = cells << sh;
    for (int c = t; c < n; c += step) heat_g[c] = 0;
}

__device__ __forceinline__ int clampi(int v, int lo, int hi) { return v < lo ? lo : (v > hi ? hi : v); }
```

include/pcgrl_hip.h:

```cpp
#ifndef PCGRL_HIP_H
#define PCGRL_HIP_H
#include <stddef.h>
#include <stdint.h>

#ifdef __cplusplus
extern "C" {
#endif

#define PCGRL_ABI_VERSION 15
#define PCGRL_OK 0
#define PCGRL_EINVAL (-1)
#define PCGRL_EHIP (-2)
#define PCGRL_ESTATE (-3)

enum { PCGRL_BINARY = 0, PCGRL_ZELDA = 1, PCGRL_SOKOBAN = 2, PCGRL_MDUNGEON = 3, PCGRL_DDAVE = 4, PCGRL_SMB = 5 };
enum { PCGRL_NARROW = 0, PCGRL_WIDE = 1, PCGRL_TURTLE = 2, PCGRL_NARROW_CAST = 3, PCGRL_NARROW_MULTI = 4, PCGRL_TURTLE_CAST = 5 };

typedef struct pcgrl_config {
    int32_t prob, rep;
    int32_t num_envs;
    int32_t width, height;
    int32_t prob_width, prob_height;
    int32_t max_changes, max_iterations;
    int32_t random_start, random_tile, warp, random_probs;
    int32_t auto_reset;
    int32_t target_path;
    int32_t max_enemies, target_enemy_dist;
    int32_t max_crates, target_solution, solver_power;
    int32_t max_potions, max_treasures;
    int32_t max_diamonds, min_spikes, target_jumps;
    int32_t min_empty, min_enemies, min_jumps;
    double target_col_enemies;
    double tile_probs[8];
    double rewards[12];
} pcgrl_config;

typedef struct pcgrl_layout {
    int32_t group;
    int32_t mask_bytes;
    int32_t nplanes;
    int32_t nstats;
    size_t map;
    size_t old_map;
    size_t heatmap;
    size_t pos;
    size_t planes;
    size_t counters;
    size_t stats;
    size_t start_stats;
    size_t info;
    size_t reward;
    size_t done;
    size_t tile_p;
    size_t rng_rep;
    size_t rng_prob;
    size_t rng_cursor;
    size_t scratch;
} pcgrl_layout;

typedef struct pcgrl_buffers {
    void *map, *old_map, *heatmap, *pos, *planes, *counters, *stats, *start_stats, *info, *reward,
         *done, *tile_p, *rng_rep, *rng_prob, *rng_cursor, *scratch;
} pcgrl_buffers;

typedef struct pcgrl_env pcgrl_env;

typedef struct pcgrl_tuning {
    int32_t no_fused;
    int32_t fused_zelda;
    int32_t step_epb;
    int32_t no_inc;
    int32_t inline_reset;
    int32_t pair_min;
    int32_t no_wide;
    int32_t wide_waves;
    int32_t wide_grid;
    int32_t wide_pairs;
    int32_t wide_few;
    int32_t sok_generic;
    int32_t sok_hard_cap;
    int32_t sok_spawn;
    int32_t md_only_agent;
    int32_t smb_lds_heap;
    int32_t full_per_wave;
    int32_t inc_per_wave;
    int32_t wide_spin;
    int32_t step_prio;
    int32_t no_touch;
    int32_t touch_tight;
    int32_t step_pair;
    int32_t async_split;
    int32_t big_team;
    int32_t obs_at_end;
    int32_t touch_resume;
    int32_t changes_grid;
    int32_t changes_chunk;
} pcgrl_tuning;

int pcgrl_abi_version(void);
const char* pcgrl_error_string(int code);
int pcgrl_last_hip_error(void);

int pcgrl_query_layout(const pcgrl_config* cfg, pcgrl_layout* out);
int pcgrl_create(const pcgrl_config* cfg, pcgrl_env** out);
int pcgrl_destroy(pcgrl_env* env);
void pcgrl_tuning_defaults(pcgrl_tuning* t);
int pcgrl_set_tuning(pcgrl_env* env, const pcgrl_tuning* t);
int pcgrl_bind(pcgrl_env* env, const pcgrl_buffers* bufs, void* stream);
int pcgrl_configure(pcgrl_env* env, const pcgrl_config* cfg);
int pcgrl_seed(pcgrl_env* env, const uint32_t* keys, int32_t first, int32_t count, void* stream);
int pcgrl_seed_words(pcgrl_env* env, const uint32_t* words, int32_t first, int32_t count, void* stream);
int pcgrl_set_tile_probs(pcgrl_env* env, void* stream);
int pcgrl_reset(pcgrl_env* env, void* stream);
int pcgrl_step(pcgrl_env* env, const int32_t* actions, void* stream);
int pcgrl_step_multi(pcgrl_env* const* envs, const int32_t* const* actions, void* const* streams, int32_t count);
int32_t pcgrl_step_threads(int32_t n);
int pcgrl_rollout(pcgrl_env* env, const int32_t* actions, int32_t steps, double* reward_out, uint8_t* done_out,
                  int32_t* info_out, void* stream);
int pcgrl_set_maps(pcgrl_env* env, const uint8_t* maps, void* stream);
int pcgrl_observe(pcgrl_env* env, uint8_t* out, int32_t out_h, int32_t out_w, int32_t centered, int32_t pad_value,
                  int32_t onehot, void* stream);
int pcgrl_bind_observation(pcgrl_env* env, uint8_t* out, int32_t out_h, int32_t out_w, int32_t centered,
                           int32_t pad_value, int32_t onehot, int32_t incremental);
typedef struct pcgrl_row {
    int64_t* actions_out;
    double*  reward;
    uint8_t* done;
    const uint8_t* start_in;
    uint8_t* start_out;
    double*  ep_return;
    int32_t* ep_length;
    uint8_t* took;
    uint8_t* fresh;
    int32_t  actions_i64;
} pcgrl_row;
int pcgrl_bind_row(pcgrl_env* env, const pcgrl_row* row);
typedef struct pcgrl_render_desc {
    const int32_t* indices;
    int32_t count;
    const uint8_t* tiles;
    int32_t tile_size;
    int32_t border_x, border_y, border_tile, cursor;
    int32_t grid_rows, grid_cols;
    uint8_t* out;
} pcgrl_render_desc;
int pcgrl_render(pcgrl_env* env, const pcgrl_render_desc* d, void* stream);
size_t pcgrl_get_stats_bytes(const pcgrl_config* cfg, int32_t count);
int    pcgrl_get_stats(pcgrl_env* env, const uint8_t* maps, int32_t count, int32_t* rows_out,
                       void* work, size_t work_bytes, void* stream);
int    pcgrl_get_reward(pcgrl_env* env, const int32_t* rows, const int32_t* ref_rows, int32_t count,
                        double* reward_out, uint8_t* over_out, void* stream);
size_t pcgrl_get_solution_bytes(const pcgrl_config* cfg, int32_t count, int32_t max_len);
int    pcgrl_get_solution(pcgrl_env* env, const uint8_t* maps, int32_t count, int32_t max_len,
                          int8_t* moves_out, int32_t* length_out, int8_t* agent_out, int32_t* rows_out,
                          void* work, size_t work_bytes, void* stream);
size_t pcgrl_get_playthrough_bytes(const pcgrl_config* cfg, int32_t count, int32_t max_len);
int    pcgrl_get_playthrough(pcgrl_env* env, const uint8_t* maps, int32_t count, int32_t max_len,
                             int8_t* moves_out, int32_t* length_out, int8_t* agent_out, int32_t* rows_out,
                             void* work, size_t work_bytes, void* stream);
size_t pcgrl_get_smb_play_bytes(const pcgrl_config* cfg, int32_t count, int32_t max_len);
int    pcgrl_get_smb_play(pcgrl_env* env, const uint8_t* maps, int32_t count, int32_t max_len,
                          int8_t* moves_out, int32_t* length_out, int8_t* agent_out, int32_t* rows_out,
                          void* work, size_t work_bytes, void* stream);
int32_t pcgrl_get_paths_legs(const pcgrl_config* cfg);
size_t pcgrl_get_paths_bytes(const pcgrl_config* cfg, int32_t count, int32_t max_len);
int    pcgrl_get_paths(pcgrl_env* env, const uint8_t* maps, int32_t count, int32_t max_len,
                       int16_t* cells_out, int32_t* length_out, int32_t* rows_out,
                       void* work, size_t work_bytes, void* stream);
size_t pcgrl_get_changes_bytes(const pcgrl_config* cfg, int32_t count, int32_t ncells);
int    pcgrl_get_changes(pcgrl_env* env, const uint8_t* maps, int32_t count,
                         const int32_t* cells, int32_t ncells, const int32_t* start_rows,
                         int32_t* base_rows_out, int32_t* rows_out, double* reward_out, uint8_t* over_out,
                         void* work, size_t work_bytes, void* stream);
int pcgrl_action_map(pcgrl_env* env, const int32_t* flat, int32_t* xyv, void* stream);
int pcgrl_step_flat(pcgrl_env* env, const int32_t* flat, int32_t* xyv, void* stream);
size_t pcgrl_async_bytes(const pcgrl_config* cfg, int32_t nslots);
int pcgrl_bind_async(pcgrl_env* env, void* arena, size_t bytes, int32_t nslots, void* stream);
int pcgrl_step_async(pcgrl_env* env, const int32_t* actions, int32_t pop_budget, void* stream);
int pcgrl_async_flush(pcgrl_env* env, void* stream);
int pcgrl_bind_episode_stats(pcgrl_env* env, double* ep_return, int32_t* ep_length, double* last_return,
                             int32_t* last_length, void* stream);
int pcgrl_selftest_heap(const uint32_t* ops, int32_t n_ops, uint32_t* pops, uint32_t* heap_out, int32_t* n_out, void* stream);
int pcgrl_selftest_step_pool(int32_t count, int32_t calls, int32_t fail_at, int32_t* hits);
int pcgrl_selftest_range_reward(const int32_t* rows, int32_t n, int32_t* out, void* stream);
int pcgrl_status(pcgrl_env* env, void* stream, int32_t* status);
int pcgrl_clear_status(pcgrl_env* env, void* stream);


#define PCGRL_NPHASE 6
int pcgrl_profile(pcgrl_env* env, int enable);
int pcgrl_profile_read(pcgrl_env* env, double* phase_ms , int32_t* steps);

#ifdef __cplusplus
}
#endif
#endif
```

Baseline: 2.382 billion env-steps/s.

## Defer map/heat writes to stats tasks, lane-parallel finalize, static first-round task ids

Adds three default-on switches to the single-kernel step path. The map-cell and heatmap writes from update_env are deferred: their packed location and tile are stored in LDS and later issued by the stats wave task, so the update phase only waits on LDS counters instead of vmcnt. Per-env finalize (stats copy, info, reward, done) is spread across 16 lanes with DPP reduction instead of running on lane 0 alone. The first-round stats work ids are assigned statically, skipping an LDS atomic. Risks include ordering hazards between the deferred writes and readers, a spin-wait on refill_done for the narrow representation, and extra LDS use.

Result: slower. 2.289 billion env-steps/s (-3.9%).

```diff
diff --git a/gym_pcgrl_amd/_lib.py b/gym_pcgrl_amd/_lib.py
--- a/gym_pcgrl_amd/_lib.py
+++ b/gym_pcgrl_amd/_lib.py
@@ -30,7 +30,7 @@
 
 TUNING_FIELDS = ("no_fused", "fused_zelda", "step_epb", "no_inc", "inline_reset", "pair_min", "no_wide", "wide_waves", "wide_grid",
                  "wide_pairs", "wide_few", "sok_generic", "sok_hard_cap", "sok_spawn", "md_only_agent", "smb_lds_heap", "full_per_wave", "inc_per_wave", "wide_spin", "step_prio", "no_touch", "touch_tight", "step_pair", "async_split", "big_team", "obs_at_end", "touch_resume",
-                 "changes_grid", "changes_chunk")
+                 "step_task_writes", "step_lane_finalize", "step_first_static", "changes_grid", "changes_chunk")
 
 
 class Tuning(C.Structure):
diff --git a/gym_pcgrl_amd/csrc/kernels_stats.h b/gym_pcgrl_amd/csrc/kernels_stats.h
--- a/gym_pcgrl_amd/csrc/kernels_stats.h
+++ b/gym_pcgrl_amd/csrc/kernels_stats.h
@@ -90,26 +90,44 @@
     const int lo = __builtin_amdgcn_update_dpp(0, (int)b, 0x100 + J, 0xF, 0xF, true), hi = __builtin_amdgcn_update_dpp(0, (int)(b >> 32), 0x100 + J, 0xF, 0xF, true);
     return __longlong_as_double(((long long)hi << 32) | (unsigned)lo);
 }
-__device__ __forceinline__ void zelda_reward_tab(const PcgrlParams& P, ZeldaRewardTab* T) {
-    T->w[0] = P.rewards[0]; T->w[1] = P.rewards[1]; T->w[2] = P.rewards[2]; T->w[3] = P.rewards[4]; T->w[4] = P.rewards[3];
-    T->w[5] = P.rewards[5]; T->w[6] = P.rewards[6]; T->w[7] = 0.0;
-    T->lo[0] = 1; T->lo[1] = 1; T->lo[2] = 1; T->lo[3] = 2; T->lo[4] = 1; T->lo[5] = P.target_enemy_dist; T->lo[6] = PCGRL_IPOS; T->lo[7] = 0;
-    T->hi[0] = 1; T->hi[1] = 1; T->hi[2] = 1; T->hi[3] = P.max_enemies; T->hi[4] = 1; T->hi[5] = PCGRL_IPOS; T->hi[6] = PCGRL_IPOS; T->hi[7] = 0;
-}
 __device__ __forceinline__ double zelda_reward_lanes(const ZeldaRewardTab* T, const int32_t* old, const int32_t* s, int k) {
     const int s0 = s[0], s1 = s[1], s2 = s[2], s3 = s[3], s4 = s[4], s5 = s[5], s6 = s[6];
     int n = s6;
     n = k == 5 ? s5 : n; n = k == 4 ? s4 : n; n = k == 3 ? s3 : n; n = k == 2 ? s2 : n; n = k == 1 ? s1 : n; n = k == 0 ? s0 : n;
-    const int kk = k & 7;
-    const int o = old[kk];
-    const double t = k < 7 ? (double)range_reward_i(n, o, T->lo[kk], T->hi[kk]) * T->w[kk] : 0.0;
+    const int o = old[k & 7];
+    const double t = zelda_reward_term(T, k, n, o);
     double r = t;
     r = r + dpp_down<1>(t); r = r + dpp_down<2>(t); r = r + dpp_down<3>(t);
     r = r + dpp_down<4>(t); r = r + dpp_down<5>(t); r = r + dpp_down<6>(t);
     return r;
 }
 
-template <int PROB, int G, class MaskT, bool FUSED = false>
+template <int PROB>
+__device__ __forceinline__ bool finalize_lanes(const PcgrlParams& P, const DevBufs& B, int e, const int32_t* s, int lane, int2 c, double reward_pre) {
+    static_assert(PROB == PCGRL_PROB_BINARY || PROB == PCGRL_PROB_ZELDA, "the problems of k_step");
+    const int k = lane & 7;
+    int32_t* st = B.stats + (size_t)e * 8;
+    const int n = lane_slot(s, lane);
+    const int o = st[k];
+    const int sv1 = PROB == PCGRL_PROB_BINARY ? B.start_stats[(size_t)e * 8 + 1] : 0;
+    double r = 0.0;
+    if (PROB == PCGRL_PROB_BINARY) {
+        const double t = binary_reward_term(P, lane, n, o);
+        r = t + dpp_down<1>(t);
+    } else r = reward_pre;
+    if (lane < 8) st[k] = n;
+    if (lane < 10) B.info[(size_t)e * 10 + lane] = lane_info_value(PROB, lane, n, s, sv1, c.x, c.y);
+    bool d = false;
+    if (lane == 0) {
+        d = episode_over_sv1(P, s, sv1, PROB) || c.y >= P.max_changes || c.x >= P.max_iterations;
+        B.reward[e] = r;
+        B.done[e] = d ? 1 : 0;
+        episode_account(B, e, r, d);
+    }
+    return d && P.auto_reset;
+}
+
+template <int PROB, int G, class MaskT, bool FUSED = false, bool STEP1 = false>
 __device__ __forceinline__ void stats_wave_task(const PcgrlParams& P, const DevBufs& B, DevGroup<G, MaskT>& g, int lane64, int gw, bool lone,
                                                 bool inc, bool pair, bool zinc, bool have, int raw, int shard, int mode, int parity,
                                                 int inline_reset, int gen_map, uint32_t* mt, uint8_t* tiles, MaskT rowmask,
@@ -121,6 +139,8 @@
     constexpr bool kZinc = PROB == PCGRL_PROB_ZELDA && G == 16 && sizeof(MaskT) == 4;
     constexpr int NPL = (PROB == PCGRL_PROB_BINARY) ? 1 : 3;
     MaskT* champ_base = reinterpret_cast<MaskT*>(B.champ);
+    constexpr bool kLaneFin = STEP1 && kCanReset && G == 16;
+    const bool lane_fin = kLaneFin && B.step_lane_fin != 0;
     const bool tch = kInc && G == 16 && !inc && !lone && have && raw < 0;
     const bool packed = inc || (kZinc && zinc && !lone) || tch;
     const bool reset_only = have && !packed && (raw & WL_RESET_ONLY) != 0;
@@ -135,7 +155,7 @@
     if (GPW >= 2 && lone && inline_reset) {
         const int role = gw & 1;
         int2 pre = make_int2(0, 0);
-        if (g.lane == 0 && role == 0 && have) pre = reinterpret_cast<const int2*>(B.counters)[e];
+        if ((g.lane == 0 || lane_fin) && role == 0 && have) pre = reinterpret_cast<const int2*>(B.counters)[e];
         asm volatile("s_waitcnt vmcnt(0)" ::: "memory");
 #pragma unroll
         for (int k = 0; k < GPW / 2; k++) {
@@ -161,7 +181,8 @@
         constexpr bool kLaneReward = PROB == PCGRL_PROB_ZELDA && G == 16;
         double rpre = 0.0;
         if (kLaneReward && SL && role == 0 && act) rpre = zelda_reward_lanes(&SL->zr, B.stats + (size_t)e * 8, sl, g.lane);
-        if (g.lane == 0 && role == 0 && act) finalize_item<PROB>(P, B, e, sl, MODE_STEP, parity, shard, false, WL_RST, &pre, (kLaneReward && SL) ? &rpre : nullptr);
+        if (kLaneFin && lane_fin) { if (role == 0 && act) finalize_lanes<kLaneFin ? PROB : PCGRL_PROB_BINARY>(P, B, e, sl, g.lane, pre, rpre); }
+        else if (g.lane == 0 && role == 0 && act) finalize_item<PROB>(P, B, e, sl, MODE_STEP, parity, shard, false, WL_RST, &pre, (kLaneReward && SL) ? &rpre : nullptr);
         __builtin_amdgcn_wave_barrier();
         if (role == 1 && have) {
             if (kInc && champ_base) champ_base[(size_t)e * G + g.lane] = champ_l;
@@ -235,9 +256,25 @@
     double rpre = 0.0;
     const bool lane_reward = kLaneReward && SL != nullptr && mode == MODE_STEP;
     if (lane_reward && have && !reset_only) rpre = zelda_reward_lanes(&SL->zr, B.stats + (size_t)e * 8, s, g.lane);
-    if (g.lane == 0 && have) {
+    if (kLaneFin && lane_fin) {
+        if (have && !reset_only) {
+            const bool w = finalize_lanes<kLaneFin ? PROB : PCGRL_PROB_BINARY>(P, B, e, s, g.lane, reinterpret_cast<const int2*>(B.counters)[e], rpre);
+            want_reset = (g.lane == 0 && w) ? 1 : 0;
+        } else if (g.lane == 0 && have) want_reset = 1;
+    } else if (g.lane == 0 && have) {
         if (reset_only) want_reset = 1;
         else want_reset = finish_or_park<PROB>(P, B, e, s, need_solver, mode, parity, shard, !inline_reset, -1, lane_reward ? &rpre : nullptr) ? 1 : 0;
+    }
+    if (STEP1 && B.step_task_writes) {
+        const bool wr = g.lane == 0 && have && !reset_only && !want_reset;
+        if (P.rep == PCGRL_REP_NARROW) { while (__hip_atomic_load(&SL->refill_done[SL->par], __ATOMIC_ACQUIRE, __HIP_MEMORY_SCOPE_WORKGROUP) < SL->need) __builtin_amdgcn_s_sleep(2); }
+        if (wr) {
+            const int w = SL->wr[e - SL->e0], cells = P.width * P.height;
+            const int hc = P.rep == PCGRL_REP_NARROW ? (int)B.pos[2 * e + 1] * P.width + (int)B.pos[2 * e] : (w & 1023);
+            B.map[(size_t)e * cells + (w & 1023)] = (uint8_t)(w >> 10);
+            heat_increment<true>(B, (size_t)e * cells + hc);
+        }
+        TL(30);
     }
     if (inline_reset) {
         const uint64_t want = __ballot(want_reset != 0);
diff --git a/gym_pcgrl_amd/csrc/kernels_step.h b/gym_pcgrl_amd/csrc/kernels_step.h
--- a/gym_pcgrl_amd/csrc/kernels_step.h
+++ b/gym_pcgrl_amd/csrc/kernels_step.h
@@ -184,7 +184,9 @@
         if (Bg.row.actions_out) Bg.row.actions_out[row_a0] = row_act;
     }
     if (threadIdx.x < EPB) { s_loc.dirty[threadIdx.x] = 0; if (OBS) { s_loc.obs_skip[threadIdx.x] = 0; s_loc.late[threadIdx.x] = 0; } }
-    if (threadIdx.x < 8) s_n[threadIdx.x >> 2][threadIdx.x & 3] = 0;
+    const int tick0 = (!MULTI && B.step_first_static) ? TPB / 64 : 0;
+    const bool task_writes = !MULTI && B.step_task_writes;
+    if (threadIdx.x < 8) s_n[threadIdx.x >> 2][threadIdx.x & 3] = (threadIdx.x & 3) == 3 ? tick0 : 0;
     if (threadIdx.x == 0) { s_loc.e0 = 0; s_loc.need = NUPD; s_loc.refill_done[0] = 0; s_loc.refill_done[1] = 0; s_loc.n_late = 0; s_obs_ticket = 0; }
     constexpr int OBS_PER_TASK = 8;
     const bool obs_delta = OBS && REP == PCGRL_REP_WIDE && NPL == 3 && Bg.obs.delta;
@@ -222,7 +224,7 @@
             const int q = a / dim;
             t3[0] = q % W; t3[1] = q / W; t3[2] = a - q * dim;
         }
-        if (e < ne) u = update_env<REP, MaskT, true, true, true>(P, B, act_lds, e, &mid);
+        if (e < ne) u = update_env<REP, MaskT, true, true, true, !MULTI>(P, B, act_lds, e, &mid, 0, task_writes);
         TL(2);
         const bool first = u.rst || u.sure_done;
         const bool packed_full = PROB == PCGRL_PROB_ZELDA && B.zelda_inc;
@@ -230,6 +232,7 @@
         if (first) { dest = 0; v = u.rst ? (e | WL_RESET_ONLY) : e; }
         else if (u.chg) { dest = u.cheap ? 2 : 1; v = (u.cheap || packed_full) ? u.inc_item : ((u.touch && B.step_touch) ? (u.inc_item | (int)0x80000000) : e); }
         if (u.chg) s_loc.dirty[e] = 1;
+        if (!MULTI && task_writes && u.chg) s_loc.wr[e] = (uint16_t)u.wr;
         if (OBS && first && e < EPB) s_loc.obs_skip[e] = 1;
         const uint64_t m0 = __ballot(dest == 0), m1 = __ballot(dest == 1), m2 = __ballot(dest == 2);
         const uint64_t below = (1ull << lane64) - 1ull;
@@ -238,7 +241,7 @@
             b0 = m0 ? atomicAdd(&s_n[sp][0], __popcll(m0)) : 0;
             b1 = m1 ? atomicAdd(&s_n[sp][1], __popcll(m1)) : 0;
             b2 = m2 ? atomicAdd(&s_n[sp][2], __popcll(m2)) : 0;
-            if (wv == 0) { s_n[sp ^ 1][0] = 0; s_n[sp ^ 1][1] = 0; s_n[sp ^ 1][2] = 0; s_n[sp ^ 1][3] = 0; s_loc.refill_done[sp ^ 1] = 0; s_loc.par = sp; }
+            if (wv == 0) { s_n[sp ^ 1][0] = 0; s_n[sp ^ 1][1] = 0; s_n[sp ^ 1][2] = 0; s_n[sp ^ 1][3] = tick0; s_loc.refill_done[sp ^ 1] = 0; s_loc.par = sp; }
         }
         b0 = __builtin_amdgcn_readfirstlane(b0); b1 = __builtin_amdgcn_readfirstlane(b1); b2 = __builtin_amdgcn_readfirstlane(b2);
         if (dest == 0) s_items[0][b0 + __popcll(m0 & below)] = v;
@@ -257,10 +260,12 @@
         __builtin_amdgcn_s_barrier();
         int k_used = 0, cur0 = 0;
         if (lane64 == 0) s_loc.late_done[wv] = 0;
-        if (e < ne && !first) update_env_cursor<REP, MaskT>(P, B, e, mid, k_used, cur0);
+        if (e < ne && !first) update_env_cursor<REP, MaskT>(P, B, e, mid, k_used, cur0, !MULTI && task_writes);
         if (OBS && REP == PCGRL_REP_WIDE && NPL == 3 && obs_delta && e < ne && !first && u.chg) obs_write_delta_piece(obs_src, obs_view_from_lds(&s_loc.obs_v), e, act_lds[3 * e], act_lds[3 * e + 1]);
         if (e < EPB) s_loc.pend[e] = (has_fifo && e < ne && !first) ? k_used : 0;
-        asm volatile("s_waitcnt vmcnt(0) lgkmcnt(0)" ::: "memory");
+        TL(29);
+        if (!MULTI && task_writes) asm volatile("s_waitcnt lgkmcnt(0)" ::: "memory");
+        else asm volatile("s_waitcnt vmcnt(0) lgkmcnt(0)" ::: "memory");
         if (lane64 == 0) __hip_atomic_fetch_add(&s_loc.refill_done[sp], 1, __ATOMIC_RELEASE, __HIP_MEMORY_SCOPE_WORKGROUP);
     }
     int n0 = 0, n1 = 0, n2 = 0, w_full = 0, w_total = 0, w_lone = 0;
@@ -304,8 +309,8 @@
             }
         }
         if (!stats_left) { if (!OBS || !obs_left) break; continue; }
-        int wid = 0;
-        if (lane64 == 0) wid = atomicAdd(&s_n[sp][3], 1);
+        int wid = wv >= NUPD ? wv - NUPD : wv + (TPB / 64 - NUPD);
+        if (!(first_round && tick0) && lane64 == 0) wid = atomicAdd(&s_n[sp][3], 1);
         wid = __builtin_amdgcn_readfirstlane(wid);
         TL(18);
         if (wid >= w_total) { stats_left = false; if (!OBS || !obs_left) break; continue; }
@@ -318,7 +323,7 @@
             const int want = lone ? (prio & 3) : (inc ? ((prio >> 4) & 3) : ((prio_nfull == 0 || wid - w_lone < prio_nfull) ? ((prio >> 2) & 3) : 0));
             if (want != prio_now) { prio_now = want; step_set_prio(want); }
         }
-        stats_wave_task<PROB, G, MaskT, true>(P, B, g, lane64, gw, lone, inc, PROB == PCGRL_PROB_ZELDA && pair, zinc, have, raw, lane64, MODE_STEP, parity, 1, gen_map, mt, tiles, rowmask, &s_loc, OBS);
+        stats_wave_task<PROB, G, MaskT, true, !MULTI>(P, B, g, lane64, gw, lone, inc, PROB == PCGRL_PROB_ZELDA && pair, zinc, have, raw, lane64, MODE_STEP, parity, 1, gen_map, mt, tiles, rowmask, &s_loc, OBS);
         TL(7);
     }
     if (prio_now) { prio_now = 0; step_set_prio(0); }
@@ -333,6 +338,7 @@
         }
         asm volatile("s_waitcnt vmcnt(0) lgkmcnt(0)" ::: "memory");
         if (lane64 == 0) __hip_atomic_store(&s_loc.late_done[wv], 1, __ATOMIC_RELEASE, __HIP_MEMORY_SCOPE_WORKGROUP);
+        TL(31);
     }
     TL(8);
     if (MULTI && (reward_out || done_out || info_out)) {
diff --git a/gym_pcgrl_amd/csrc/kernels_update.h b/gym_pcgrl_amd/csrc/kernels_update.h
--- a/gym_pcgrl_amd/csrc/kernels_update.h
+++ b/gym_pcgrl_amd/csrc/kernels_update.h
@@ -9,12 +9,14 @@
     int bucket;
     int inc_item;
     int k, cur0;
+    int wr;
 };
 struct UpdateMid { int x, y, hx, hy, cur; bool chg, dead; };
-template <int REP, class MaskT, bool FIFO = false, bool SPLIT = false, bool AR_ONLY = false>
-__device__ __forceinline__ UpdateOut update_env(const PcgrlParams& P, const DevBufs& B, const int32_t* __restrict__ actions, int e, UpdateMid* mid = nullptr, const int ash = 0) {
+template <int REP, class MaskT, bool FIFO = false, bool SPLIT = false, bool AR_ONLY = false, bool DEFER = false>
+__device__ __forceinline__ UpdateOut update_env(const PcgrlParams& P, const DevBufs& B, const int32_t* __restrict__ actions, int e, UpdateMid* mid = nullptr, const int ash = 0,
+                                              const bool defer = false) {
     bool chg = false, rst = false, cheap = false, sure_done = false, touch_item = false;
-    int bucket = 0, inc_item = 0, k_used = 0, cur0 = 0;
+    int bucket = 0, inc_item = 0, k_used = 0, cur0 = 0, wr = 0;
     uint32_t fw[PCGRL_FIFO_N];
 #pragma unroll
     for (int i = 0; i < PCGRL_FIFO_N; i++) fw[i] = 0;
@@ -143,7 +145,8 @@
                 cheap = po == pn;
             }
             const bool dead_writes = FIFO && P.auto_reset && B.inline_reset && (c.y + 1 >= P.max_changes || iter >= P.max_iterations);
-            if (!dead_writes) *cell = (uint8_t)tile;
+            if (DEFER && defer) wr = (wy * W + wx) | (tile << 10);
+            else if (!dead_writes) *cell = (uint8_t)tile;
             const MaskT bit = (MaskT)1 << wx;
             if (NPL > 0) pl[0] = (tile & 1) ? (m0 | bit) : (m0 & ~bit);
             if (NPL > 1) {
@@ -227,7 +230,7 @@
             changes += 1;
             const bool dead_writes = FIFO && P.auto_reset && B.inline_reset && (changes >= P.max_changes || iter >= P.max_iterations);
             dead_heat = dead_writes;
-            if (!dead_writes && !(SPLIT && REP == PCGRL_REP_NARROW)) heat_increment<AR_ONLY>(B, ((size_t)e * H + hy) * W + hx);
+            if (!dead_writes && !(SPLIT && REP == PCGRL_REP_NARROW) && !(DEFER && defer)) heat_increment<AR_ONLY>(B, ((size_t)e * H + hy) * W + hx);
         }
         reinterpret_cast<int2*>(B.counters)[e] = make_int2(iter, changes);
         if (bad) atomicOr(B.status, PCGRL_STATUS_BAD_ACTION);
@@ -253,12 +256,13 @@
     }
     UpdateOut o;
     o.chg = chg; o.rst = rst; o.cheap = cheap; o.touch = touch_item; o.sure_done = sure_done; o.bucket = bucket; o.inc_item = inc_item;
-    o.k = k_used; o.cur0 = cur0;
+    o.k = k_used; o.cur0 = cur0; o.wr = wr;
     return o;
 }
 
 template <int REP, class MaskT>
-__device__ __forceinline__ void update_env_cursor(const PcgrlParams& P, const DevBufs& B, int e, const UpdateMid& mid, int& k_used, int& cur0) {
+__device__ __forceinline__ void update_env_cursor(const PcgrlParams& P, const DevBufs& B, int e, const UpdateMid& mid, int& k_used, int& cur0,
+                                                  const bool defer = false) {
     const int W = P.width, H = P.height;
     int x = mid.x, y = mid.y, cur = mid.cur;
     k_used = 0; cur0 = cur;
@@ -315,7 +319,7 @@
         x += 1;
         if (x >= W) { x = 0; y += 1; if (y >= H) y = 0; }
     }
-    if (mid.chg && !mid.dead) heat_increment<true>(B, ((size_t)e * H + y) * W + x);
+    if (mid.chg && !mid.dead && !defer) heat_increment<true>(B, ((size_t)e * H + y) * W + x);
     reinterpret_cast<uchar2*>(B.pos)[e] = make_uchar2((unsigned char)x, (unsigned char)y);
 }
 
diff --git a/gym_pcgrl_amd/csrc/pcgrl_abi.hip b/gym_pcgrl_amd/csrc/pcgrl_abi.hip
--- a/gym_pcgrl_amd/csrc/pcgrl_abi.hip
+++ b/gym_pcgrl_amd/csrc/pcgrl_abi.hip
@@ -305,6 +305,9 @@
     B.step_ipw = (i == 1 || i == 2) ? i : 4;
     B.step_touch = tun_or(T.no_touch, 0) ? 0 : 1;
     B.touch_resume = tun_or(T.touch_resume, 1) ? 1 : 0;
+    B.step_task_writes = tun_or(T.step_task_writes, 1) ? 1 : 0;
+    B.step_lane_fin = tun_or(T.step_lane_finalize, 1) ? 1 : 0;
+    B.step_first_static = tun_or(T.step_first_static, 1) ? 1 : 0;
     B.step_pair = tun_or(T.step_pair, 6);
     B.step_tight = B.step_touch ? tun_or(T.touch_tight, 1) : 0;
     h->no_inc = tun_or(T.no_inc, 0) != 0;
diff --git a/gym_pcgrl_amd/csrc/pcgrl_algos.h b/gym_pcgrl_amd/csrc/pcgrl_algos.h
--- a/gym_pcgrl_amd/csrc/pcgrl_algos.h
+++ b/gym_pcgrl_amd/csrc/pcgrl_algos.h
@@ -142,6 +142,40 @@
     return n[5] >= P.target_solution;
 }
 PCGRL_HD bool episode_over(const PcgrlParams& P, const int32_t* n, const int32_t* start) { return episode_over(P, n, start, P.prob); }
+struct ZeldaRewardTab { double w[8]; int lo[8]; int hi[8]; };
+PCGRL_HD void zelda_reward_tab(const PcgrlParams& P, ZeldaRewardTab* T) {
+    T->w[0] = P.rewards[0]; T->w[1] = P.rewards[1]; T->w[2] = P.rewards[2]; T->w[3] = P.rewards[4]; T->w[4] = P.rewards[3];
+    T->w[5] = P.rewards[5]; T->w[6] = P.rewards[6]; T->w[7] = 0.0;
+    T->lo[0] = 1; T->lo[1] = 1; T->lo[2] = 1; T->lo[3] = 2; T->lo[4] = 1; T->lo[5] = P.target_enemy_dist; T->lo[6] = PCGRL_IPOS; T->lo[7] = 0;
+    T->hi[0] = 1; T->hi[1] = 1; T->hi[2] = 1; T->hi[3] = P.max_enemies; T->hi[4] = 1; T->hi[5] = PCGRL_IPOS; T->hi[6] = PCGRL_IPOS; T->hi[7] = 0;
+}
+PCGRL_HD double zelda_reward_term(const ZeldaRewardTab* T, int k, int n, int o) {
+    const int kk = k & 7;
+    return k < 7 ? (double)range_reward_i(n, o, T->lo[kk], T->hi[kk]) * T->w[kk] : 0.0;
+}
+PCGRL_HD double binary_reward_term(const PcgrlParams& P, int k, int n, int o) {
+    const double t0 = (double)range_reward_i(n, o, 1, 1) * P.rewards[0], t1 = (double)(n - o) * P.rewards[1];
+    return k == 0 ? t0 : t1;
+}
+PCGRL_HD int lane_slot(const int32_t* s, int k) {
+    const int s0 = s[0], s1 = s[1], s2 = s[2], s3 = s[3], s4 = s[4], s5 = s[5], s6 = s[6], s7 = s[7];
+    int n = s7;
+    n = k == 6 ? s6 : n; n = k == 5 ? s5 : n; n = k == 4 ? s4 : n; n = k == 3 ? s3 : n;
+    n = k == 2 ? s2 : n; n = k == 1 ? s1 : n; n = k == 0 ? s0 : n;
+    return n;
+}
+PCGRL_HD int lane_info_value(int prob, int k, int n, const int32_t* s, int sv1, int iterations, int changes) {
+    if (k == 8) return iterations;
+    if (k == 9) return changes;
+    if (prob == PCGRL_PROB_BINARY && k == 2) return s[1] - sv1;
+    if (prob == PCGRL_PROB_BINARY && k == 3) return 0;
+    return n;
+}
+
+PCGRL_HD bool episode_over_sv1(const PcgrlParams& P, const int32_t* n, int sv1, int prob) {
+    if (prob == PCGRL_PROB_BINARY) return n[0] == 1 && n[1] - sv1 >= P.target_path;
+    return n[5] >= P.target_enemy_dist && n[6] >= P.target_path;
+}
 PCGRL_HD int num_stats(int prob) { return prob == PCGRL_PROB_BINARY ? 2 : (prob == PCGRL_PROB_ZELDA ? 7 : (prob == PCGRL_PROB_SOKOBAN ? 6 : 8)); }
 
 template <class WordT>
diff --git a/gym_pcgrl_amd/csrc/worklist.h b/gym_pcgrl_amd/csrc/worklist.h
--- a/gym_pcgrl_amd/csrc/worklist.h
+++ b/gym_pcgrl_amd/csrc/worklist.h
@@ -97,6 +97,7 @@
     int32_t big_team;
     int32_t touch_resume;
     int32_t step_touch;
+    int32_t step_task_writes, step_lane_fin, step_first_static;
     uint8_t* big_arena;
     uint8_t* pending; unsigned long long* async_stats;
     const uint8_t* async_slots; size_t async_slot_bytes; int32_t async_nslots; int32_t* async_run; int32_t* async_run_n;
@@ -105,7 +106,6 @@
 };
 #define PCGRL_FIFO_N 8
 
-struct ZeldaRewardTab { double w[8]; int lo[8]; int hi[8]; };
 struct ObsView {
     uint8_t* out;
     int oh, ow, depth, centered, pad, W, H;
@@ -114,6 +114,7 @@
     int e0;
     int par, need;
     int refill_done[2];
+    uint16_t wr[256];
     int pend[256];
     int late_done[4];
     uint8_t dirty[256];
diff --git a/include/pcgrl_hip.h b/include/pcgrl_hip.h
--- a/include/pcgrl_hip.h
+++ b/include/pcgrl_hip.h
@@ -93,6 +93,9 @@
     int32_t big_team;
     int32_t obs_at_end;
     int32_t touch_resume;
+    int32_t step_task_writes;
+    int32_t step_lane_finalize;
+    int32_t step_first_static;
     int32_t changes_grid;
     int32_t changes_chunk;
 } pcgrl_tuning;
```
